# ofekm5/relative-pose-estimation

Measured on AMD Instinct MI355X. Metric: image-pairs/s end-to-end (640x480 pairs), median rotation-angle error alongside, higher is better.
Workload: dtype u8/i32 (ORB, Hamming) + f64 (RANSAC, pose); 1 GPU; 1024 640x480 pairs per GPU, ORB(1000kp)+BF-Hamming crossCheck top-500+5pt-RANSAC(0.999,1px)+recoverPose (BASELINE configs[1]); pairs_per_gpu=1024, distinct_pairs=1024, global_pairs=1024, streams_per_gpu=1, pairs_per_launch=1024

## Files before the change

include/rpe_amd.h:

```cpp
#ifndef RPE_AMD_H
#define RPE_AMD_H

#include <stddef.h>
#include <stdint.h>

#ifdef __cplusplus
extern "C" {
#endif

#define RPE_ABI_VERSION 3
#define RPE_ORB_LEVELS 12

enum {
    RPE_PAIR_OK = 0,
    RPE_PAIR_NO_DESCRIPTORS = 1,
    RPE_PAIR_INSUFFICIENT_MATCHES = 2,
    RPE_PAIR_NO_ESSENTIAL = 3,
    RPE_PAIR_AMBIGUOUS_ESSENTIAL = 4
};

enum {
    RPE_OVF_ORB_CANDIDATES = 1 << 0,
    RPE_OVF_ORB_KEYPOINTS  = 1 << 1,
    RPE_OVF_SIFT_SEEDS     = 1 << 4,
// ... 48 lines not shown
    float x, y;
    float size;
    float angle;
    float response;
    int32_t octave;
} rpe_sift_keypoint;

void rpe_default_config(rpe_config *cfg);
int rpe_create(const rpe_config *cfg, rpe_handle **out);
void rpe_destroy(rpe_handle *h);
const char *rpe_last_error(const rpe_handle *h);
int rpe_device_count(void);
int rpe_keypoint_capacity(const rpe_handle *h);

int rpe_device_malloc(rpe_handle *h, size_t bytes, void **d_ptr);
int rpe_device_free(rpe_handle *h, void *d_ptr);
int rpe_memcpy_h2d(rpe_handle *h, void *d_dst, const void *h_src, size_t bytes);
int rpe_memcpy_d2h(rpe_handle *h, void *h_dst, const void *d_src, size_t bytes);
int rpe_synchronize(rpe_handle *h);
int rpe_host_alloc(rpe_handle *h, size_t bytes, void **h_ptr);
int rpe_host_free(rpe_handle *h, void *h_ptr);
int rpe_host_register(rpe_handle *h, void *h_ptr, size_t bytes);
int rpe_host_unregister(rpe_handle *h, void *h_ptr);

int rpe_estimate_batch(rpe_handle *h, const uint8_t *h_imgs1, const uint8_t *h_imgs2, int B,
                       const double K[9], double *R, double *t, int32_t *inliers,
                       int32_t *n_matches, int32_t *status);
int rpe_estimate_batch_device(rpe_handle *h, const uint8_t *d_imgs1, const uint8_t *d_imgs2, int B,
                              const double K[9], double *R, double *t, int32_t *inliers,
                              int32_t *n_matches, int32_t *status);
int rpe_enqueue_batch_device(rpe_handle *h, const uint8_t *d_imgs1, const uint8_t *d_imgs2, int B,
                             const double K[9]);
int rpe_fetch_results(rpe_handle *h, int B, double *R, double *t, int32_t *inliers,
                      int32_t *n_matches, int32_t *status);
int rpe_fetch_overflow(rpe_handle *h, int n_pairs, uint32_t *flags);
int rpe_estimate_stream(rpe_handle *h, const uint8_t *h_frames, int F, const double K[9],
                        double *R, double *t, int32_t *inliers, int32_t *n_matches, int32_t *status);
int rpe_enqueue_stream_device(rpe_handle *h, const uint8_t *d_frames, int F, const double K[9]);

int rpe_frames_reserve(rpe_handle *h, int n_slots);
int rpe_frames_capacity(const rpe_handle *h);
int rpe_frames_put_device(rpe_handle *h, const uint8_t *d_frames, int n, const int32_t *slots);
int rpe_frames_put(rpe_handle *h, const uint8_t *h_frames, int n, const int32_t *slots);
int rpe_frames_info(rpe_handle *h, int n, const int32_t *slots, int32_t *counts, uint32_t *flags);
int rpe_enqueue_pairs(rpe_handle *h, const int32_t *slot1, const int32_t *slot2, int P, const double K[9]);
int rpe_estimate_pairs(rpe_handle *h, const int32_t *slot1, const int32_t *slot2, int P, const double K[9],
                       double *R, double *t, int32_t *inliers, int32_t *n_matches, int32_t *status);

#define RPE_UNDISTORT_ITERS 5
typedef struct rpe_camera {
    double fx, fy, cx, cy;
    double dist[8];
} rpe_camera;

int rpe_frames_set_cameras(rpe_handle *h, int n, const int32_t *slots, const rpe_camera *cams);
int rpe_enqueue_pairs_cameras(rpe_handle *h, const int32_t *slot1, const int32_t *slot2, int P);
int rpe_estimate_pairs_cameras(rpe_handle *h, const int32_t *slot1, const int32_t *slot2, int P,
                               double *R, double *t, int32_t *inliers, int32_t *n_matches, int32_t *status);
int rpe_enqueue_batch_cameras_device(rpe_handle *h, const uint8_t *d_imgs1, const uint8_t *d_imgs2, int B,
                                     const rpe_camera *cam1, const rpe_camera *cam2);
int rpe_estimate_batch_cameras_device(rpe_handle *h, const uint8_t *d_imgs1, const uint8_t *d_imgs2, int B,
                                      const rpe_camera *cam1, const rpe_camera *cam2, double *R, double *t,
                                      int32_t *inliers, int32_t *n_matches, int32_t *status);
int rpe_estimate_batch_cameras(rpe_handle *h, const uint8_t *h_imgs1, const uint8_t *h_imgs2, int B,
                               const rpe_camera *cam1, const rpe_camera *cam2, double *R, double *t,
                               int32_t *inliers, int32_t *n_matches, int32_t *status);
int rpe_undistort_points(rpe_handle *h, const float *h_pts, int n, const rpe_camera *cam, double *h_out_xy);
int rpe_find_essential_cameras(rpe_handle *h, const float *h_pts1, const float *h_pts2, const int32_t *m, int B,
                               const rpe_camera *cam1, const rpe_camera *cam2, double *E, uint8_t *mask,
                               int32_t *found, int32_t *info);
int rpe_recover_pose_cameras(rpe_handle *h, const double *h_E, const float *h_pts1, const float *h_pts2,
                             const int32_t *m, int B, const rpe_camera *cam1, const rpe_camera *cam2,
                             double *R, double *t, int32_t *inliers);
int rpe_refine_pose_points_cameras(rpe_handle *h, const double *h_R0, const double *h_t0, const float *h_pts1,
                                   const float *h_pts2, const uint8_t *h_mask, const int32_t *m, int B,
                                   const rpe_camera *cam1, const rpe_camera *cam2, int max_iters, double *R, double *t,
                                   int32_t *inliers, int32_t *info, double *rms);

enum { RPE_ORDER_BGR = 0, RPE_ORDER_RGB = 1 };
int rpe_bgr_to_gray_device(rpe_handle *h, const uint8_t *d_bgr, size_t n_pixels, int order, uint8_t *d_gray);
int rpe_bgr_to_gray(rpe_handle *h, const uint8_t *h_bgr, size_t n_pixels, int order, uint8_t *h_gray);

int rpe_lsd_detect(const uint8_t *h_gray, int width, int height, float *h_lines, int capacity, int32_t *n_lines);

int rpe_fetch_matched_points(rpe_handle *h, int B, float *pts1, float *pts2);

int rpe_fetch_structure(rpe_handle *h, int B, uint8_t *ransac_mask, uint8_t *pose_mask, double *points);

enum {
    RPE_REFINE_OK = 0,
    RPE_REFINE_SKIPPED = 1,
    RPE_REFINE_REJECTED = 2
};

int rpe_refine_poses(rpe_handle *h, int B, int max_iters, double *R, double *t, int32_t *inliers,
                     int32_t *info, double *rms);

int rpe_fetch_match_indices(rpe_handle *h, int B, int32_t *qidx, int32_t *tidx);

enum { RPE_LINK_OK = 0, RPE_LINK_PAIR_FAILED = 1, RPE_LINK_TOO_FEW = 2 };
int rpe_scale_links(rpe_handle *h, int L, const int32_t *pair_a, const int32_t *pair_b, const int32_t *side,
                    int min_shared, double *stats, int32_t *n_shared, int32_t *code);

int rpe_guided_matches(rpe_handle *h, int B, const double *R, const double *t, double gate_px, int max_distance,
                       int32_t *qidx, int32_t *tidx, int32_t *dist, float *pts1, float *pts2, int32_t *n_matches);

int rpe_guided_matches_l2(rpe_handle *h, int B, const double *R, const double *t, double gate_px, double max_distance,
                          int32_t *qidx, int32_t *tidx, float *dist, float *pts1, float *pts2, int32_t *n_matches);

enum { RPE_HOMOGRAPHY_OK = 0, RPE_HOMOGRAPHY_SKIPPED = 1, RPE_HOMOGRAPHY_NONE = 2 };
int rpe_pair_homographies(rpe_handle *h, int B, int iters, double threshold_px,
                          double *H, double *R_rot, uint8_t *mask, int32_t *counts, int32_t *info);
int rpe_find_homography(rpe_handle *h, const float *h_pts1, const float *h_pts2, const int32_t *m, int B,
                        const double K[9], int iters, double threshold_px,
                        double *H, double *R_rot, uint8_t *mask, int32_t *counts, int32_t *info);

enum { RPE_LINKPOSE_OK = 0, RPE_LINKPOSE_PAIR_FAILED = 1, RPE_LINKPOSE_TOO_FEW = 2, RPE_LINKPOSE_NONE = 3 };
int rpe_link_poses(rpe_handle *h, int L, const int32_t *pair_a, const int32_t *pair_b, const int32_t *side,
                   int iters, double threshold_px, int min_shared, int refine_iters,
                   double *R, double *t, uint8_t *mask, int32_t *counts, int32_t *info, double *rms);

enum { RPE_BUNDLE_OK = 0, RPE_BUNDLE_PAIR_FAILED = 1, RPE_BUNDLE_TOO_FEW = 2, RPE_BUNDLE_SKIPPED = 3, RPE_BUNDLE_REJECTED = 4 };
int rpe_link_bundles(rpe_handle *h, int L, const int32_t *pair_a, const int32_t *pair_b, const int32_t *side,
                     const double *R0, const double *t0, double threshold_px, int min_shared, int max_iters,
                     double *R_a, double *t_a, double *R_b, double *t_b, double *points, uint8_t *views,
                     int32_t *counts, int32_t *info, double *rms);
int rpe_bundle_three_view(rpe_handle *h, int B, const int32_t *n, const double *obs_s, const double *obs_a,
                          const double *obs_c, const uint8_t *has_c, const double *X0, const double *Ra0, const double *ta0,
                          const double *Rc0, const double *tc0, double f_a, double f_c, int max_iters,
                          double *R_a, double *t_a, double *R_c, double *t_c, double *points, uint8_t *views,
                          int32_t *counts, int32_t *info, double *rms);

enum { RPE_TRACK_EDGES_USABLE = 0, RPE_TRACK_EDGES_RANSAC = 1, RPE_TRACK_EDGES_ALL = 2 };
int rpe_last_run_pairs(const rpe_handle *h);
int rpe_build_tracks(rpe_handle *h, const uint8_t *use_pair, int edge_rule, int min_len,
                     int32_t *counts, int32_t *track_start, int32_t *obs_frame, int32_t *obs_kp, float *obs_xy,
                     int32_t *match_track);
int rpe_tracks_from_matches(rpe_handle *h, int P, int n_frames, const int32_t *frame1, const int32_t *frame2, const int32_t *m,
                            const int32_t *qidx, const int32_t *tidx, const uint8_t *edge, const float *pts1, const float *pts2,
                            int min_len, int32_t *counts, int32_t *track_start, int32_t *obs_frame, int32_t *obs_kp,
                            float *obs_xy, int32_t *match_track);

enum { RPE_TRACKPT_OK = 0, RPE_TRACKPT_TOO_FEW = 1, RPE_TRACKPT_DEGENERATE = 2, RPE_TRACKPT_BEHIND = 3, RPE_TRACKPT_OUTLIERS = 4,
       RPE_TRACKPT_LOW_PARALLAX = 5 };
int rpe_triangulate_tracks(rpe_handle *h, int n_tracks, const int32_t *track_start, const int32_t *obs_frame, const float *obs_xy,
                           int n_frames, const double *R_abs, const double *T_abs, const int32_t *frame_group, const double *K,
                           const rpe_camera *cams, double threshold_px, int min_views, double max_cos, int max_iters,
                           double *points, int32_t *info, double *rms, double *min_cos, uint8_t *obs_flag, double *obs_err);

int rpe_orb_detect_and_compute(rpe_handle *h, const uint8_t *h_imgs, int n_images,
                               rpe_keypoint *kps, uint8_t *desc, int32_t *counts);
int rpe_orb_debug_fetch(rpe_handle *h, int index, int which, uint8_t *h_out);
int64_t rpe_orb_pyramid_pixels(const rpe_handle *h);
int rpe_orb_debug_retain(rpe_handle *h, int kind, int stl_runtime, void *elems, const int32_t *len, const int32_t *n_points,
                         int n_lists, int cap, int32_t *out_len);

int rpe_match_hamming(rpe_handle *h, const uint8_t *h_desc1, const int32_t *n1,
                      const uint8_t *h_desc2, const int32_t *n2, int B,
                      int32_t *qidx, int32_t *tidx, int32_t *dist, int32_t *n_matches);

int rpe_match_hamming_guided(rpe_handle *h, const uint8_t *h_desc1, const float *h_pts1, const int32_t *n1,
                             const uint8_t *h_desc2, const float *h_pts2, const int32_t *n2, int B,
                             const double K[9], const double *R, const double *t, double gate_px, int max_distance,
                             int32_t *qidx, int32_t *tidx, int32_t *dist, int32_t *n_matches);

int rpe_sift_detect_and_compute(rpe_handle *h, const uint8_t *h_imgs, int n_images,
                                rpe_sift_keypoint *kps, float *desc, int32_t *counts);
int64_t rpe_sift_debug_gauss(rpe_handle *h, int index, float *out);

int rpe_match_l2(rpe_handle *h, const float *h_desc1, const int32_t *n1, const float *h_desc2,
                 const int32_t *n2, int B, int32_t *qidx, int32_t *tidx, float *dist, int32_t *n_matches);

int rpe_match_l2_guided(rpe_handle *h, const float *h_desc1, const float *h_pts1, const int32_t *n1,
                        const float *h_desc2, const float *h_pts2, const int32_t *n2, int B,
                        const double K[9], const double *R, const double *t, double gate_px, double max_distance,
                        int32_t *qidx, int32_t *tidx, float *dist, int32_t *n_matches);

int rpe_find_essential(rpe_handle *h, const float *h_pts1, const float *h_pts2, const int32_t *m, int B,
                       const double K[9], double *E, uint8_t *mask, int32_t *found, int32_t *info);

int rpe_recover_pose(rpe_handle *h, const double *h_E, const float *h_pts1, const float *h_pts2,
                     const int32_t *m, int B, const double K[9],
                     double *R, double *t, int32_t *inliers);

int rpe_refine_pose_points(rpe_handle *h, const double *h_R0, const double *h_t0, const float *h_pts1,
                           const float *h_pts2, const uint8_t *h_mask, const int32_t *m, int B, const double K[9],
                           int max_iters, double *R, double *t, int32_t *inliers, int32_t *info, double *rms);

enum {
    RPE_STAGE_PYRAMID = 0, RPE_STAGE_FAST, RPE_STAGE_NMS, RPE_STAGE_SELECT, RPE_STAGE_HARRIS,
    RPE_STAGE_KEYPOINTS, RPE_STAGE_ANGLE, RPE_STAGE_BLUR, RPE_STAGE_DESCRIBE, RPE_STAGE_MATCH,
    RPE_STAGE_RANSAC, RPE_STAGE_POSE, RPE_STAGE_COUNT
};
int rpe_set_profiling(rpe_handle *h, int enable);
int rpe_get_stage_ms(rpe_handle *h, float *ms );
const char *rpe_stage_name(int stage);

#define RPE_COMM_ID_BYTES 128
#define RPE_POSE_RECORD_BYTES 128
typedef struct rpe_comm rpe_comm;
int rpe_comm_unique_id(uint8_t id[RPE_COMM_ID_BYTES]);
int rpe_comm_create(rpe_handle *h, int rank, int world, const uint8_t id[RPE_COMM_ID_BYTES], rpe_comm **out);
int rpe_comm_prepare(rpe_handle *h, int rank, int world, rpe_comm **out);
int rpe_comm_connect(rpe_comm *c, const uint8_t id[RPE_COMM_ID_BYTES]);
int rpe_comm_destroy(rpe_comm *c);
const char *rpe_comm_last_error(void);
int rpe_gather_poses(rpe_handle *h, rpe_comm *c, int n_local, int per_rank, int first_pair, void *h_records);
int rpe_comm_allreduce_max(rpe_comm *c, double *value);
int rpe_comm_barrier(rpe_comm *c);

int rpe_calibrate_valu(rpe_handle *h, int kind, int waves_per_simd, double *wave_insts_per_s);
const char *rpe_calibrate_valu_name(int kind);
int rpe_calibrate_hbm(rpe_handle *h, double *bytes_per_s);

#ifdef __cplusplus
}
#endif
#endif
```

relative_pose_estimation_amd/_capi.py:

```python
import ctypes as C
import os

import numpy as np

_HERE = os.path.dirname(os.path.abspath(__file__))
LIB_PATH = os.environ.get("RPE_LIB", os.path.join(_HERE, "librpe_amd.so"))

ABI_VERSION = 3
ORB_LEVELS = 12
PAIR_OK, PAIR_NO_DESCRIPTORS, PAIR_INSUFFICIENT_MATCHES, PAIR_NO_ESSENTIAL, PAIR_AMBIGUOUS_ESSENTIAL = 0, 1, 2, 3, 4
FEATURE_ORB, FEATURE_SIFT = 0, 1
NORM_HAMMING, NORM_L2 = 0, 1
MATCH_CROSSCHECK, MATCH_RATIO = 0, 1
STL_LIBSTDCXX, STL_MSVC = 0, 1
OVF_ORB_CANDIDATES, OVF_ORB_KEYPOINTS = 1 << 0, 1 << 1
OVF_SIFT_SEEDS, OVF_SIFT_RAW, OVF_SIFT_PREFILTER, OVF_SIFT_CAP, OVF_SIFT_KEYPOINTS = 1 << 4, 1 << 5, 1 << 6, 1 << 7, 1 << 8
SIFT_UNCAPPED_CAPACITY = 16320
MAX_MATCHES_LIMIT = 8064
CALIB_KINDS = 18
STAGE_COUNT = 12
ORDER_BGR, ORDER_RGB = 0, 1
REFINE_OK, REFINE_SKIPPED, REFINE_REJECTED = 0, 1, 2
LINK_OK, LINK_PAIR_FAILED, LINK_TOO_FEW = 0, 1, 2
HOMOGRAPHY_OK, HOMOGRAPHY_SKIPPED, HOMOGRAPHY_NONE = 0, 1, 2
LINKPOSE_OK, LINKPOSE_PAIR_FAILED, LINKPOSE_TOO_FEW, LINKPOSE_NONE = 0, 1, 2, 3
BUNDLE_OK, BUNDLE_PAIR_FAILED, BUNDLE_TOO_FEW, BUNDLE_SKIPPED, BUNDLE_REJECTED = 0, 1, 2, 3, 4
TRACK_EDGES_USABLE, TRACK_EDGES_RANSAC, TRACK_EDGES_ALL = 0, 1, 2
TRACK_COUNTS = ("n_tracks", "n_obs", "n_edges", "dropped_conflict", "dropped_short", "n_frames_seen")
TRACKPT_OK, TRACKPT_TOO_FEW, TRACKPT_DEGENERATE, TRACKPT_BEHIND, TRACKPT_OUTLIERS, TRACKPT_LOW_PARALLAX = 0, 1, 2, 3, 4, 5
TRACKPT_NAMES = ("OK", "TOO_FEW", "DEGENERATE", "BEHIND", "OUTLIERS", "LOW_PARALLAX")
UNDISTORT_ITERS = 5

_SIGNATURES = {
    "rpe_default_config": "v:p", "rpe_create": "i:pp", "rpe_destroy": "v:p", "rpe_last_error": "s:p", "rpe_device_count": "i:",
    "rpe_keypoint_capacity": "i:p", "rpe_device_malloc": "i:pzp", "rpe_device_free": "i:pp", "rpe_memcpy_h2d": "i:pppz",
    "rpe_memcpy_d2h": "i:pppz", "rpe_synchronize": "i:p", "rpe_host_alloc": "i:pzp", "rpe_host_free": "i:pp",
    "rpe_host_register": "i:ppz", "rpe_host_unregister": "i:pp",
    "rpe_estimate_batch": "i:pppipppppp", "rpe_estimate_batch_device": "i:pppipppppp", "rpe_enqueue_batch_device": "i:pppip",
    "rpe_fetch_results": "i:pippppp", "rpe_fetch_overflow": "i:pip", "rpe_estimate_stream": "i:ppipppppp",
    "rpe_enqueue_stream_device": "i:ppip",
    "rpe_frames_reserve": "i:pi", "rpe_frames_capacity": "i:p", "rpe_frames_put_device": "i:ppip", "rpe_frames_put": "i:ppip",
    "rpe_frames_info": "i:pippp", "rpe_enqueue_pairs": "i:pppip", "rpe_estimate_pairs": "i:pppipppppp",
    "rpe_frames_set_cameras": "i:pipp", "rpe_enqueue_pairs_cameras": "i:pppi", "rpe_estimate_pairs_cameras": "i:pppippppp",
    "rpe_enqueue_batch_cameras_device": "i:pppipp", "rpe_estimate_batch_cameras_device": "i:pppippppppp",
    "rpe_estimate_batch_cameras": "i:pppippppppp", "rpe_undistort_points": "i:ppipp",
    "rpe_find_essential_cameras": "i:ppppipppppp", "rpe_recover_pose_cameras": "i:pppppippppp",
    "rpe_refine_pose_points_cameras": "i:pppppppippippppp",
    "rpe_bgr_to_gray_device": "i:ppzip", "rpe_bgr_to_gray": "i:ppzip", "rpe_lsd_detect": "i:piipip",
    "rpe_fetch_matched_points": "i:pipp", "rpe_fetch_structure": "i:pippp", "rpe_refine_poses": "i:piippppp",
    "rpe_fetch_match_indices": "i:pipp", "rpe_scale_links": "i:pipppippp", "rpe_link_poses": "i:pipppidiipppppp",
    "rpe_link_bundles": "i:pipppppdiippppppppp", "rpe_bundle_three_view": "i:pippppppppppddippppppppp",
    "rpe_last_run_pairs": "i:p", "rpe_build_tracks": "i:ppiipppppp", "rpe_tracks_from_matches": "i:piippppppppipppppp",
    "rpe_triangulate_tracks": "i:pipppipppppdidipppppp",
    "rpe_guided_matches": "i:pippdipppppp",
    "rpe_guided_matches_l2": "i:pippddpppppp",
    "rpe_pair_homographies": "i:piidppppp", "rpe_find_homography": "i:ppppipidppppp",
    "rpe_orb_detect_and_compute": "i:ppippp", "rpe_orb_debug_fetch": "i:piip", "rpe_orb_pyramid_pixels": "l:p",
    "rpe_orb_debug_retain": "i:piipppiip",
    "rpe_match_hamming": "i:pppppipppp", "rpe_match_hamming_guided": "i:pppppppipppdipppp",
    "rpe_sift_detect_and_compute": "i:ppippp", "rpe_sift_debug_gauss": "l:pip", "rpe_match_l2": "i:pppppipppp",
    "rpe_match_l2_guided": "i:pppppppipppddpppp",
    "rpe_find_essential": "i:ppppippppp", "rpe_recover_pose": "i:pppppipppp", "rpe_refine_pose_points": "i:pppppppipippppp",
    "rpe_set_profiling": "i:pi", "rpe_get_stage_ms": "i:pp", "rpe_stage_name": "s:i",
    "rpe_comm_unique_id": "i:p", "rpe_comm_create": "i:piipp", "rpe_comm_prepare": "i:piip", "rpe_comm_connect": "i:pp",
    "rpe_comm_destroy": "i:p", "rpe_comm_last_error": "s:", "rpe_gather_poses": "i:ppiiip", "rpe_comm_allreduce_max": "i:pp",
    "rpe_comm_barrier": "i:p",
    "rpe_calibrate_valu": "i:piip", "rpe_calibrate_valu_name": "s:i", "rpe_calibrate_hbm": "i:pp",
}
_ARG = {"p": C.c_void_p, "i": C.c_int, "d": C.c_double, "z": C.c_size_t}
_RET = {"i": C.c_int, "l": C.c_int64, "s": C.c_char_p, "v": None}
SIGNATURES = {name: (_RET[sig[0]], [_ARG[c] for c in sig[2:]]) for name, sig in _SIGNATURES.items()}
EXPORTS = list(SIGNATURES)


class Config(C.Structure):
    _fields_ = [("abi_version", C.c_int32), ("device", C.c_int32), ("width", C.c_int32), ("height", C.c_int32),
                ("max_batch", C.c_int32), ("feature_method", C.c_int32), ("norm_type", C.c_int32),
                ("max_matches", C.c_int32), ("nfeatures", C.c_int32), ("fast_threshold", C.c_int32),
                ("ransac_max_iters", C.c_int32), ("ransac_prob", C.c_double), ("ransac_threshold", C.c_double),
                ("match_mode", C.c_int32), ("stl_runtime", C.c_int32), ("match_ratio", C.c_double)]


KP_DTYPE = np.dtype([("x", "<f4"), ("y", "<f4"), ("angle", "<f4"), ("response", "<f4"),
                     ("octave", "<i4"), ("lx", "<i4"), ("ly", "<i4")])

SIFT_KP_DTYPE = np.dtype([("x", "<f4"), ("y", "<f4"), ("size", "<f4"), ("angle", "<f4"), ("response", "<f4"),
                          ("octave", "<i4")])

CAMERA_DTYPE = np.dtype([("fx", "<f8"), ("fy", "<f8"), ("cx", "<f8"), ("cy", "<f8"), ("dist", "<f8", (8,))])

_lib = None


class RpeError(RuntimeError):
    pass


class Camera:

    def __init__(self, K, dist=None):
        K = np.asarray(K, np.float64)
        if K.shape != (3, 3):
            raise ValueError(f"Camera: K must be 3 x 3, got shape {K.shape}")
        d = np.zeros(0) if dist is None else np.asarray(dist, np.float64).reshape(-1)
        if d.size not in (0, 4, 5, 8):
            raise ValueError(f"Camera: dist must hold 4, 5 or 8 coefficients (cv2 order), got {d.size}")
        self.fx, self.fy, self.cx, self.cy = float(K[0, 0]), float(K[1, 1]), float(K[0, 2]), float(K[1, 2])
        self.dist = np.zeros(8)
        self.dist[:d.size] = d
        if not (np.isfinite([self.fx, self.fy, self.cx, self.cy]).all() and np.isfinite(self.dist).all()):
            raise ValueError("Camera: non-finite field")
        if not (self.fx > 0 and self.fy > 0):
            raise ValueError("Camera: fx and fy must be > 0")

    @property
    def K(self):
        return np.array([[self.fx, 0., self.cx], [0., self.fy, self.cy], [0., 0., 1.]])

    def record(self):
        r = np.zeros(1, CAMERA_DTYPE)
        r["fx"], r["fy"], r["cx"], r["cy"], r["dist"] = self.fx, self.fy, self.cx, self.cy, self.dist
        return r


def camera_records(cameras, n):
    if isinstance(cameras, np.ndarray) and cameras.dtype == CAMERA_DTYPE:
        rec = np.ascontiguousarray(cameras).reshape(-1)
    elif isinstance(cameras, Camera):
        rec = np.repeat(cameras.record(), n)
    else:
        cameras = list(cameras)
        if not all(isinstance(c, Camera) for c in cameras):
            raise ValueError("cameras: expected Camera objects")
        rec = np.concatenate([c.record() for c in cameras]) if cameras else np.zeros(0, CAMERA_DTYPE)
    if rec.size != n:
        raise ValueError(f"cameras: expected {n}, got {rec.size}")
    return np.ascontiguousarray(rec)


def load():
    global _lib
    if _lib is not None:
        return _lib
    if not os.path.exists(LIB_PATH):
        raise RpeError(f"{LIB_PATH} not found: build it with __graft_entry__.build() "
                       "(make -C relative_pose_estimation_amd/csrc); there is no CPU fallback")
    lib = C.CDLL(LIB_PATH)
    for name, (restype, argtypes) in SIGNATURES.items():
        fn = getattr(lib, name)
        fn.restype, fn.argtypes = restype, argtypes
    _lib = lib
    return lib


def _p(a):
    return a.ctypes.data_as(C.c_void_p)


def _opt(a):
    return None if a is None else _p(a)


def _f64(a):
    return np.ascontiguousarray(a, np.float64)


def _i32(a):
    return np.ascontiguousarray(a, np.int32).reshape(-1)


def _slot_pairs(slot1, slot2):
    s1, s2 = _i32(slot1), _i32(slot2)
    assert s1.size == s2.size
    return s1, s2


def lsd_detect(gray, capacity=8192):
    g = np.ascontiguousarray(gray, np.uint8)
    assert g.ndim == 2
    out = np.zeros((capacity, 4), np.float32)
    n = np.zeros(1, np.int32)
    rc = load().rpe_lsd_detect(_p(g), g.shape[1], g.shape[0], _p(out), capacity, _p(n))
    if rc != 0:
        raise RpeError(f"rpe_lsd_detect failed ({rc})")
    return out[:min(int(n[0]), capacity)].astype(np.float64)


class Engine:

    def __init__(self, width, height, max_batch=1, nfeatures=4000, max_matches=500, device=0,
                 feature_method=FEATURE_ORB, norm_type=NORM_HAMMING, fast_threshold=15,
                 ransac_max_iters=1000, ransac_prob=0.999, ransac_threshold=1.0,
                 match_mode=MATCH_CROSSCHECK, match_ratio=0.75, stl_runtime=STL_LIBSTDCXX):
        self.lib = load()
        cfg = Config()
        self.lib.rpe_default_config(C.byref(cfg))
        cfg.device = device; cfg.width = width; cfg.height = height; cfg.max_batch = max_batch
        cfg.feature_method = feature_method; cfg.norm_type = norm_type
        cfg.max_matches = max_matches; cfg.nfeatures = nfeatures; cfg.fast_threshold = fast_threshold
        cfg.ransac_max_iters = ransac_max_iters; cfg.ransac_prob = ransac_prob; cfg.ransac_threshold = ransac_threshold
        cfg.match_mode = match_mode; cfg.match_ratio = match_ratio; cfg.stl_runtime = stl_runtime
        self.cfg = cfg
        h = C.c_void_p()
        rc = self.lib.rpe_create(C.byref(cfg), C.byref(h))
        if rc != 0:
            raise RpeError(f"rpe_create failed ({rc}): {self.lib.rpe_last_error(None).decode()}")
        self.h = h
        self.width, self.height, self.max_batch = width, height, max_batch
        self.max_matches = max_matches
        self.kcap = self.lib.rpe_keypoint_capacity(h)
# ... 534 lines not shown
```

relative_pose_estimation_amd/csrc/orb_kernels.hip:

```cpp
#include "rpe_internal.h"
#include "rpe_devmath.h"
#include "retain_best_emul.h"
#include "fast_entry.h"

__device__ float4 c_pattern_f[256];

__constant__ uint2 c_discw[32 * 8];

__constant__ float c_gauss[7];

void rpe_orb_upload_constants(const signed char *disc, int n)
{
    uint2 wt[32 * 8];
    for (int i = 0; i < 32 * 8; ++i) wt[i] = make_uint2(0u, 0u);
    for (int i = 0; i < n; ++i) {
        const int u = disc[2 * i], v = disc[2 * i + 1];
        const int j = (u + 16) >> 2, b = (u + 16) & 3;
        wt[(v + 15) * 8 + j].x |= 1u << (8 * b);
        wt[(v + 15) * 8 + j].y |= (unsigned)(u + 16) << (8 * b);
    }
    hipMemcpyToSymbol(HIP_SYMBOL(c_discw), wt, sizeof(wt));
    {
        static const signed char pat[256 * 4] = {
#include "brief_pattern.inc"
        };
        std::vector<float> pf(1024);
        for (int i = 0; i < 1024; ++i) pf[i] = (float)pat[i];
        hipMemcpyToSymbol(HIP_SYMBOL(c_pattern_f), pf.data(), sizeof(float) * 1024);
    }
    {
        double v[7], sum = 0.;
        float g[7];
        for (int i = 0; i < 7; ++i) { const double x = (double)(i - 3); v[i] = exp(-0.125 * x * x); sum += v[i]; }
        for (int i = 0; i < 7; ++i) g[i] = (float)(v[i] / sum);
        hipMemcpyToSymbol(HIP_SYMBOL(c_gauss), g, sizeof(g));
    }
}

__device__ __forceinline__ int xcd_tile(int b, int n)
{
    const int per = (n + 7) >> 3;
    return (b & 7) * per + (b >> 3);
}

__device__ __forceinline__ bool xcd_image_block(int nb, int n_img, int &img, int &blk)
{
    const int b = blockIdx.x, x = b & 7, idx = b >> 3;
    img = x + 8 * (idx / nb);
    blk = idx - (idx / nb) * nb;
    return img < n_img;
}
static inline unsigned xcd_image_grid(int nb, int n_img) { return (unsigned)(8 * ((n_img + 7) / 8) * nb); }

constexpr int PYR_THREADS = 64;
constexpr int PYR_LDS_DW = PYR_ROWS * PYR_DW + 4;
constexpr int PYR_NQ = PYR_DW / 4;
constexpr int PYR_LROWS = PYR_THREADS / PYR_NQ;
constexpr int PYR_LLANES = PYR_LROWS * PYR_NQ;
constexpr int PYR_NLD = (PYR_ROWS + PYR_LROWS - 1) / PYR_LROWS;
constexpr int PYR_NLD_FULL = (PYR_TH + 1 + PYR_LROWS - 1) / PYR_LROWS;
constexpr int PYR_NCHUNK = PYR_ROWS * PYR_NQ;
static_assert(PYR_THREADS == PYR_TW / 4 && PYR_THREADS == 64 && PYR_TH == 16, "one wave per tile; a lane takes 4 columns x the tile's 16 rows");
static_assert(PYR_DW % 4 == 0, "window rows are whole 16-byte chunks");
static_assert(PYR_LROWS == 3 && PYR_LLANES == 63 && PYR_NLD == 8, "63 lanes x 8 rounds of 3 rows cover the 23 x 21 chunks");
static_assert(PYR_NCHUNK * 4 <= PYR_LDS_DW && (PYR_NLD - 1) * PYR_LLANES < PYR_NCHUNK, "only the last round is cut short by the window's end");
static_assert((PYR_ROWS + 1) * PYR_DW * 4 < (1 << PYR_YW_SHIFT), "a window byte offset fits the row field of the y table");
static_assert(PYR_LDS_DW * 4 == 7744, "LDS per tile window");
__global__ __launch_bounds__(PYR_THREADS) void pyr_resize_kernel(uint8_t *pyr, RpeDeviceLayout lay, const int *__restrict__ coef,
                                                                  const RpePyrTile *__restrict__ ptiles, int ntiles, int l)
{
    __shared__ __attribute__((aligned(16))) unsigned s_src[PYR_LDS_DW];
    const RpeLevel &S = lay.lv[l - 1];
    const RpeLevel &D = lay.lv[l];
    const int tid = threadIdx.x;
    const int ti = xcd_tile(blockIdx.x, ntiles);
    if (ti >= ntiles) return;
    const RpePyrTile pt = ptiles[ti];
    const int x0 = pt.x0, y0 = pt.y0, a0 = pt.a0, sy0 = pt.sy0, nsrc = pt.nsrc;
    const unsigned reuse = pt.reuse;
    const uint8_t *src = rpe_level_base(pyr, lay, blockIdx.y, l - 1);
    const int *cxp = coef + D.dcoef_off, *cyp = cxp + ((D.w + 127) & ~127) + y0;
    const int x4 = x0 + 4 * tid;
    const int4 cv = *(const int4 *)(cxp + x4);
    unsigned ys[PYR_TH];
#pragma unroll
    for (int r = 0; r < PYR_TH; ++r) ys[r] = (unsigned)cyp[r];
    {
        const int lr = tid / PYR_NQ, lc = tid - lr * PYR_NQ;
        const unsigned colb = (unsigned)min(a0 + 16 * lc, S.pitch - 16) + __umul24((unsigned)sy0, (unsigned)S.pitch);
        const unsigned off0 = colb + __umul24((unsigned)lr, (unsigned)S.pitch), offmax = colb + __umul24((unsigned)(nsrc - 1), (unsigned)S.pitch);
        const unsigned pitch3 = PYR_LROWS * S.pitch;
        uint4 stage[PYR_NLD];
#pragma unroll
        for (int q = 0; q < PYR_NLD; ++q)
            if (q < PYR_NLD_FULL || PYR_LROWS * q < nsrc) stage[q] = *(const uint4 *)(src + min(off0 + q * pitch3, offmax));
#pragma unroll
        for (int q = 0; q < PYR_NLD; ++q)
            if (q < PYR_NLD_FULL || PYR_LROWS * q < nsrc) asm volatile("" : "+v"(stage[q].x), "+v"(stage[q].y), "+v"(stage[q].z), "+v"(stage[q].w));
        if (tid < PYR_LLANES) {
#pragma unroll
            for (int q = 0; q < PYR_NLD; ++q)
                if ((q < PYR_NLD_FULL || PYR_LROWS * q < nsrc) && (PYR_LLANES * (q + 1) <= PYR_NCHUNK || tid < PYR_NCHUNK - PYR_LLANES * q))
                    ((uint4 *)s_src)[tid + PYR_LLANES * q] = stage[q];
        }
    }
    typedef unsigned short v2u16_t __attribute__((ext_vector_type(2)));
    unsigned selp[4];
    v2u16_t apk[4];
    int bcol;
    {
        const int cw[4] = {cv.x, cv.y, cv.z, cv.w};
        const int o0 = cw[0] & 0xFFFF;
        bcol = o0 - a0;
#pragma unroll
        for (int j = 0; j < 4; ++j) {
            const unsigned rel = (unsigned)min(max((cw[j] & 0xFFFF) - o0, 0), 4);
            selp[j] = 0x0c000c00u | rel | ((rel + 1u) << 16);
            const unsigned a1 = (unsigned)cw[j] >> 16;
            apk[j] = __builtin_bit_cast(v2u16_t, (256u - a1) | (a1 << 16));
        }
    }
    const unsigned vbase = ((unsigned)bcol & ~3u) - (unsigned)sy0 * (PYR_DW * 4);
    __syncthreads();
    if (x4 >= D.pitch) return;
    const unsigned sh = (unsigned)bcol & 3u;
    auto fetch = [&](unsigned lds_byte, unsigned (&t)[3]) {
        const unsigned *p = (const unsigned *)((const uint8_t *)s_src + lds_byte);
        t[0] = p[0]; t[1] = p[1]; t[2] = p[2];
    };
    auto hpass = [&](const unsigned (&t)[3], unsigned (&hh)[4]) {
        const unsigned lo = __builtin_amdgcn_alignbyte(t[1], t[0], sh), hi = __builtin_amdgcn_alignbyte(t[2], t[1], sh);
#pragma unroll
        for (int j = 0; j < 4; ++j) hh[j] = __builtin_amdgcn_udot2(__builtin_bit_cast(v2u16_t, __builtin_amdgcn_perm(hi, lo, selp[j])), apk[j], 0u, false);
    };
    const unsigned colmask = x4 + 3 < D.w ? 0xFFFFFFFFu : (x4 >= D.w ? 0u : (0xFFFFFFFFu >> (8 * (x4 + 4 - D.w))));
    const unsigned sel01 = (0x0c0c0602u & colmask) | (0x0c0c0c0cu & ~colmask), sel23 = (0x06020c0cu & colmask) | (0x0c0c0c0cu & ~colmask);
    uint8_t *drow = pyr + (long long)blockIdx.y * lay.stride + D.off + __umul24((unsigned)y0, (unsigned)D.pitch) + x0;
    const int nrows = min(PYR_TH, D.h - y0);
    unsigned vo = 4u * (unsigned)tid, half = 32768u;
    asm("" : "+v"(half));
    auto rowtop = [&](int r) { return (ys[r] & ((1u << PYR_YW_SHIFT) - 1u)) + vbase; };
    unsigned hs[2][4], nb[3];
    fetch(rowtop(0) + PYR_DW * 4, nb);
#pragma unroll
    for (int r = 0; r < PYR_TH; ++r) {
        if (r == 0 || !((reuse >> r) & 1u)) { unsigned tt[3]; fetch(rowtop(r), tt); hpass(tt, hs[r & 1]); }
        const unsigned cb[3] = {nb[0], nb[1], nb[2]};
        if (r + 1 < PYR_TH) fetch(rowtop(r + 1) + PYR_DW * 4, nb);
        hpass(cb, hs[(r + 1) & 1]);
        const unsigned (&ht)[4] = hs[r & 1], (&hb)[4] = hs[(r + 1) & 1];
        const unsigned b1u = ys[r] >> PYR_YW_SHIFT, b0u = 256u - b1u;
        unsigned sm[4];
#pragma unroll
        for (int j = 0; j < 4; ++j) {
            unsigned t = __umul24(b0u, ht[j]) + half;
            asm("" : "+v"(t));
            sm[j] = __umul24(b1u, hb[j]) + t;
        }
        asm("" : "+v"(vo));
        if (r < nrows) *(unsigned *)(drow + vo) = __builtin_amdgcn_perm(sm[1], sm[0], sel01) | __builtin_amdgcn_perm(sm[3], sm[2], sel23);
        drow += D.pitch;
    }
}

void rpe_launch_pyramid(rpe_handle *h, int n_img)
{
    for (int l = 1; l < RPE_NLEVELS; ++l) {
        const int nt = h->pyr_tile_cnt[l];
        hipLaunchKernelGGL(pyr_resize_kernel, dim3((nt + 7) / 8 * 8, n_img), dim3(PYR_THREADS), 0, h->stream, h->d_pyr, h->lay, h->d_coef,
                           (const RpePyrTile *)(h->d_pyr_tiles + h->pyr_tile_off[l]), nt, l);
    }
}

__device__ __forceinline__ int imax3(int a, int b, int c) { return max(a, max(b, c)); }
__device__ __forceinline__ int vmax3u(int a, int b, int c) { int d; asm("v_max3_u32 %0, %1, %2, %3" : "=v"(d) : "v"(a), "v"(b), "v"(c)); return d; }
__device__ __forceinline__ int vmin3u(int a, int b, int c) { int d; asm("v_min3_u32 %0, %1, %2, %3" : "=v"(d) : "v"(a), "v"(b), "v"(c)); return d; }
typedef unsigned short ushort2_t __attribute__((ext_vector_type(2)));
static constexpr int CIRC_DX[16] = {0, 1, 2, 3, 3, 3, 2, 1, 0, -1, -2, -3, -3, -3, -2, -1};
static constexpr int CIRC_DY[16] = {3, 3, 2, 1, 0, -1, -2, -3, -3, -3, -2, -1, 0, 1, 2, 3};

constexpr int FS_ROWS = FAST_TH + 2;
constexpr int FAST_PROWS = FAST_TH + 8;
constexpr int FAST_THREADS = 256;
constexpr int FAST_NRP = 14;
constexpr int FAST_LANES = FAST_NRP * 18;
constexpr int FAST_NCAND = FS_ROWS * 72;
static_assert(FAST_LANES <= FAST_THREADS, "a pass of FAST_NRP tile rows fits the workgroup");
static_assert(FAST_ENTRY_NRP == FAST_NRP && FAST_ENTRY_LANES == FAST_LANES && FAST_ENTRY_PITCH == 72 && FAST_ENTRY_NPASS == 5,
              "fast_entry.h describes this kernel's lane mapping");
static_assert(6 * FAST_NRP >= FAST_PROWS && 5 * FAST_NRP >= FS_ROWS, "6 load passes cover the pixel rows, 5 phase-1 passes the score rows");
static_assert(RPE_FAST_TILE_CAP == (64 / 2) * (FAST_TH / 2), "strict 3x3 maxima of a tile");
static_assert(RPE_FAST_TILE_CAP <= FAST_PROWS * 18, "the tile's keypoint list lives in the dead pixel tile");
static_assert((FAST_PROWS * 18 + FS_ROWS * 18) * 4 + FAST_NCAND * 2 + 8 == 19448, "LDS per workgroup");
__global__ __launch_bounds__(FAST_THREADS) void fast_nms_kernel(const uint8_t *__restrict__ pyr, unsigned *__restrict__ tile_list,
                                                        int *__restrict__ tile_cnt, RpeDeviceLayout lay,
                                                        const RpeTile *__restrict__ tiles, int ntiles)
{
    __shared__ __attribute__((aligned(16))) unsigned s_in[FAST_PROWS * 18];
    __shared__ __attribute__((aligned(16))) unsigned s_sc[FS_ROWS * 18];
    unsigned *s_out = s_in;
    __shared__ unsigned short s_cand[FAST_NCAND];
    __shared__ int s_ncand, s_nout;
    const int tid = threadIdx.x, lane = tid & 63;
    const int ti = xcd_tile(blockIdx.x, ntiles);
    if (ti >= ntiles) return;
    const RpeTile t = tiles[ti];
    const RpeLevel &L = lay.lv[t.level];
    const int w = L.w, hgt = L.h, pitch = L.pitch, thr = lay.fast_thr;
    const int x0 = t.tx, y0 = t.ty;
    const long long tslot = (long long)blockIdx.y * ntiles + ti;
    const bool live = w > 2 * RPE_EDGE && hgt > 2 * RPE_EDGE && x0 < w - RPE_EDGE && x0 + 64 > RPE_EDGE &&
                      y0 < hgt - RPE_EDGE && y0 + FAST_TH > RPE_EDGE;
    if (!live) {
        if (tid == 0) tile_cnt[tslot] = 0;
        return;
    }
    const uint8_t *src = rpe_level_base(pyr, lay, blockIdx.y, t.level);
    if (tid == 0) { s_ncand = 0; s_nout = 0; }
    {
        const int lc = tid % 18, lr = tid / 18;
        const int lx = min(x0 - 4 + 4 * lc, pitch - 4);
        unsigned stage[6];
#pragma unroll
        for (int q = 0; q < 6; ++q) {
            const int r = min(lr + FAST_NRP * q, FAST_PROWS - 1);
            const int y = min(y0 - 4 + r, hgt - 1);
            stage[q] = *(const unsigned *)(src + (__umul24((unsigned)y, (unsigned)pitch) + (unsigned)lx));
        }
#pragma unroll
        for (int q = 0; q < 6; ++q) asm volatile("" : "+v"(stage[q]));
#pragma unroll
        for (int q = 0; q < 6; ++q) { const int r = lr + FAST_NRP * q; if (tid < FAST_LANES && r < FAST_PROWS) s_in[r * 18 + lc] = stage[q]; }
    }
    {
        uint4 *z1 = (uint4 *)s_sc;
        const uint4 z = make_uint4(0, 0, 0, 0);
        for (int i = tid; i < FS_ROWS * 18 / 4; i += FAST_THREADS) z1[i] = z;
    }
    __syncthreads();
    const unsigned T0 = (unsigned)thr * 0x01000100u;
    const int c = tid % 18, r0 = tid / 18;
    unsigned dark_bits = 0, brt_bits = 0, ndark_bits = 0xFFFFFFFFu;
    if (tid < FAST_LANES) {
        const int cl = max(c - 1, 0), cr = min(c + 1, 17);
        const int pxb = x0 - 4 + 4 * c;
        const int xlo = max(x0 - 1, RPE_EDGE - 1), xhi = min(x0 + 64, w - RPE_EDGE);
        unsigned vmask = 0xFu;
        if (pxb < xlo) vmask &= 0xFu << min(xlo - pxb, 4);
        if (pxb + 3 > xhi) vmask &= 0xFu >> min(pxb + 3 - xhi, 4);
        vmask &= 0xFu;
        const unsigned vmask5 = ((vmask * 0x00204081u) & 0x01010101u) * 0x1Fu;
        const unsigned *pC = s_in + (r0 + 3) * 18 + c, *pL = s_in + (r0 + 3) * 18 + cl, *pR = s_in + (r0 + 3) * 18 + cr;
#pragma unroll
        for (int it = 0; it < 5; ++it) {
            const int ry = r0 + FAST_NRP * it;
            const int py = y0 - 1 + ry;
            if (vmask == 0 || ry >= FS_ROWS || py < RPE_EDGE - 1 || py >= hgt - RPE_EDGE + 1) continue;
            const int ro = FAST_NRP * 18 * it;
            const unsigned cdw = pC[ro], ldw = pL[ro], rdw = pR[ro];
            const unsigned upl = pL[ro - 36], upc = pC[ro - 36], upr = pR[ro - 36];
            const unsigned dnl = pL[ro + 36], dnc = pC[ro + 36], dnr = pR[ro + 36];
            const unsigned bot = pC[ro + 54], top = pC[ro - 54];
            const unsigned n = ~cdw;
            const ushort2_t ne = __builtin_bit_cast(ushort2_t, n << 8), no = __builtin_bit_cast(ushort2_t, n);
            const ushort2_t T8 = __builtin_bit_cast(ushort2_t, T0);
            const unsigned Yd = __builtin_amdgcn_perm(__builtin_bit_cast(unsigned, __builtin_elementwise_add_sat(no, T8)),
                                                      __builtin_bit_cast(unsigned, __builtin_elementwise_add_sat(ne, T8)), 0x07030501u);
            const unsigned Yb = __builtin_amdgcn_perm(__builtin_bit_cast(unsigned, __builtin_elementwise_sub_sat(no, T8)),
                                                      __builtin_bit_cast(unsigned, __builtin_elementwise_sub_sat(ne, T8)), 0x07030501u);
            unsigned r[8];
            r[0] = bot;
            r[1] = top;
            r[2] = __builtin_amdgcn_alignbyte(rdw, cdw, 3);
            r[3] = __builtin_amdgcn_alignbyte(cdw, ldw, 1);
            r[4] = __builtin_amdgcn_alignbyte(dnr, dnc, 2);
            r[5] = __builtin_amdgcn_alignbyte(upc, upl, 2);
            r[6] = __builtin_amdgcn_alignbyte(upr, upc, 2);
            r[7] = __builtin_amdgcn_alignbyte(dnc, dnl, 2);
            unsigned nd[8], br[8];
#pragma unroll
            for (int k = 0; k < 8; ++k) {
                nd[k] = __builtin_amdgcn_lerp(r[k], Yd, 0xFFFFFFFFu);
                br[k] = __builtin_amdgcn_lerp(r[k], Yb, 0u);
            }
            unsigned xnd = nd[0] & nd[1], xb = br[0] | br[1];
#pragma unroll
            for (int k = 2; k < 8; k += 2) {
                xnd = __builtin_amdgcn_bitop3_b32(nd[k], nd[k + 1], xnd, 0xEA);
                xb = __builtin_amdgcn_bitop3_b32(br[k], br[k + 1], xb, 0xA8);
            }
            const unsigned rowm = 0x01010101u << it;
            ndark_bits = (ndark_bits & ~rowm) | ((xnd >> (7 - it)) & rowm);
            brt_bits |= (xb >> (7 - it)) & rowm;
        }
        dark_bits = ~ndark_bits & vmask5;
        brt_bits &= vmask5;
    }
    {
        const unsigned both_bits = brt_bits & dark_bits, do_bits = dark_bits & ~brt_bits, bo_bits = brt_bits & ~dark_bits;
        const int n = __popc(dark_bits) | (__popc(bo_bits) << 16);
        const int inc = wave_inclusive_sum(n);
        const int total = __shfl(inc, 63);
        if (total) {
            int base = 0;
            if (lane == 63) base = atomicAdd(&s_ncand, total);
            const int pre = __shfl(base, 63) + inc - n;
            unsigned short *wF = s_cand + (pre & 0xFFFF), *wB = s_cand + (FAST_NCAND - 1 - (pre >> 16));
            const unsigned ebase = fast_entry_lane_base((unsigned)tid);
            auto append = [&](unsigned bits, unsigned sides, unsigned short *&w, int step) {
                unsigned e = fast_entry_lane(ebase, 0u, sides);
                asm("" : "+v"(e));
                while (bits) {
                    const unsigned bpos = (unsigned)__ffs((int)bits) - 1u;
                    bits &= bits - 1;
                    *w = (unsigned short)(e | bpos);
                    w += step;
                }
            };
            append(do_bits, FAST_ENTRY_DARK, wF, 1);
            append(both_bits, FAST_ENTRY_SIDES, wF, 1);
            append(bo_bits, FAST_ENTRY_BRIGHT, wB, -1);
        }
    }
    __syncthreads();
    const int ncand = s_ncand;
    const int nF = ncand & 0xFFFF, nB = ncand >> 16, nc = nF + nB, gap = FAST_NCAND - nc;
    const int wv = __builtin_amdgcn_readfirstlane(tid >> 6);
    const int slice = ((nc + FAST_THREADS - 1) / FAST_THREADS) * 64;
    const int jb = min(wv * slice, nc), je = min(jb + slice, nc);
    const int cb = jb < nF ? jb : jb + gap;
    int ncorner = 0;
    const uint8_t *sb = (const uint8_t *)s_in;
    for (int j0 = jb; j0 < je; j0 += 64) {
        const int j = j0 + lane;
        bool corner = false;
        int cc = 0;
        if (j < je) {
            cc = s_cand[j < nF ? j : j + gap];
            const unsigned off = fast_entry_offset((unsigned)cc);
            const uint8_t *p = sb + 3 * 72 + off;
            const int v = p[0];
            int r[16];
#pragma unroll
            for (int k = 0; k < 16; ++k) r[k] = p[CIRC_DY[k] * 72 + CIRC_DX[k]];
            int s = 0;
            if (cc & 0x4000) {
                int x3[16];
#pragma unroll
                for (int k = 0; k < 16; ++k) x3[k] = vmax3u(r[k], r[(k + 1) & 15], r[(k + 2) & 15]);
                int x9[16];
#pragma unroll
                for (int k = 0; k < 16; ++k) x9[k] = vmax3u(x3[k], x3[(k + 3) & 15], x3[(k + 6) & 15]);
                const int m = min(vmin3u(vmin3u(x9[0], x9[1], x9[2]), vmin3u(x9[3], x9[4], x9[5]), vmin3u(x9[6], x9[7], x9[8])),
                                  vmin3u(vmin3u(x9[9], x9[10], x9[11]), vmin3u(x9[12], x9[13], x9[14]), x9[15]));
                s = v - m;
            }
            if (cc & 0x8000) {
                int m3[16];
#pragma unroll
                for (int k = 0; k < 16; ++k) m3[k] = vmin3u(r[k], r[(k + 1) & 15], r[(k + 2) & 15]);
                int m9[16];
#pragma unroll
                for (int k = 0; k < 16; ++k) m9[k] = vmin3u(m3[k], m3[(k + 3) & 15], m3[(k + 6) & 15]);
                const int m = max(vmax3u(vmax3u(m9[0], m9[1], m9[2]), vmax3u(m9[3], m9[4], m9[5]), vmax3u(m9[6], m9[7], m9[8])),
                                  vmax3u(vmax3u(m9[9], m9[10], m9[11]), vmax3u(m9[12], m9[13], m9[14]), m9[15]));
                s = max(s, m - v);
            }
            if (s > thr) {
                ((uint8_t *)s_sc)[off] = (uint8_t)(s - 1);
                corner = true;
            }
        }
        const unsigned long long km = __ballot(corner);
        if (corner) s_cand[cb + ncorner + __popcll(km & ((1ull << lane) - 1ull))] = (unsigned short)fast_entry_to_compact((unsigned)cc);
        ncorner += __popcll(km);
    }
    __syncthreads();
    const uint8_t *sc = (const uint8_t *)s_sc;
    for (int i0 = 0; i0 < ncorner; i0 += 64) {
        const int i = i0 + lane;
        bool keep = false;
        unsigned ent = 0;
        if (i < ncorner) {
            const int cc = s_cand[cb + i];
            const int bx = (int)fast_entry_compact_bx((unsigned)cc), ry = (int)fast_entry_compact_ry((unsigned)cc);
            const int px = x0 - 4 + bx, py = y0 - 1 + ry;
            const bool inside = (unsigned)(bx - 4) < 64u & (unsigned)(ry - 1) < (unsigned)FAST_TH &
                                (unsigned)(px - RPE_EDGE) < (unsigned)(w - 2 * RPE_EDGE) & (unsigned)(py - RPE_EDGE) < (unsigned)(hgt - 2 * RPE_EDGE);
            const uint8_t *q = sc + ry * 72 + bx;
            const int v = q[0];
            const int nmax = imax3(imax3(q[-1], q[1], q[-73]), imax3(q[-72], q[-71], q[71]), max((int)q[72], (int)q[73]));
            if (inside & (v > nmax)) {
                keep = true;
                ent = ((unsigned)v << 24) | ((unsigned)py << 12) | (unsigned)px;
            }
        }
        const unsigned long long km = __ballot(keep);
        if (km) {
            int base = 0;
            if (lane == 0) base = atomicAdd(&s_nout, __popcll(km));
            base = __shfl(base, 0);
            if (keep) s_out[base + __popcll(km & ((1ull << lane) - 1ull))] = ent;
        }
    }
    __syncthreads();
    const int nout = s_nout;
    unsigned *dst = tile_list + tslot * RPE_FAST_TILE_CAP;
    for (int i = tid; i < nout; i += FAST_THREADS) dst[i] = s_out[i];
    if (tid == 0) tile_cnt[tslot] = nout;
}

void rpe_launch_fast(rpe_handle *h, int n_img)
{
    if (h->n_tiles_fast == 0) return;
    hipLaunchKernelGGL(fast_nms_kernel, dim3((h->n_tiles_fast + 7) / 8 * 8, n_img), dim3(FAST_THREADS), 0, h->stream,
                       h->d_pyr, h->d_tile_list, h->d_tile_cnt, h->lay, h->d_tiles_fast, h->n_tiles_fast);
}

__global__ __launch_bounds__(256) void raster_corners_kernel(const unsigned *__restrict__ tile_list, const int *__restrict__ tile_cnt,
                                                              unsigned *__restrict__ corner, int *__restrict__ corner_count,
                                                              unsigned *__restrict__ ovf, RpeDeviceLayout lay, int ntiles, int rows_cap, int key_cap)
{
    extern __shared__ unsigned s_dyn[];
    unsigned *s_rs = s_dyn;
    unsigned *s_fill = s_rs + rows_cap + 1;
    unsigned *s_key = s_fill + rows_cap;
    unsigned *s_toff = s_key + key_cap;
    __shared__ int s_wave[5];
    __shared__ int s_live;
    const int tid = threadIdx.x, l = blockIdx.x, img = blockIdx.y;
    const RpeLevel &L = lay.lv[l];
    if (tid == 64) s_live = 0x7FFFFFFF;
    const int nrows = L.h, nt = L.ntile, ccap = L.ccap;
    for (int i = tid; i <= nrows; i += 256) s_rs[i] = 0;
    for (int i = tid; i < nrows; i += 256) s_fill[i] = 0;
    const int *tc = tile_cnt + (long long)img * ntiles + L.tile0;
    const unsigned *tl = tile_list + ((long long)img * ntiles + L.tile0) * RPE_FAST_TILE_CAP;
    int nraw = 0;
    for (int t0 = 0; t0 < nt; t0 += 256) {
        const int t = t0 + tid;
        const int c = t < nt ? tc[t] : 0;
        int total;
        const int ex = block_excl_scan(c, s_wave, total);
        if (t < nt) s_toff[t] = (unsigned)(nraw + ex);
        nraw += total;
    }
    if (tid == 0) s_toff[nt] = (unsigned)nraw;
    __syncthreads();
    auto fetch = [&](int sidx) -> unsigned {
        int lo = 0, hi = nt;
        while (hi - lo > 1) { const int mid = (lo + hi) >> 1; if (s_toff[mid] <= (unsigned)sidx) lo = mid; else hi = mid; }
        return tl[(long long)lo * RPE_FAST_TILE_CAP + (sidx - (int)s_toff[lo])];
    };
    for (int base = 0; base < nraw; base += 1024) {
        unsigned e4[4];
#pragma unroll
        for (int u = 0; u < 4; ++u) { const int sidx = base + tid + 256 * u; e4[u] = sidx < nraw ? fetch(sidx) : 0u; }
#pragma unroll
        for (int u = 0; u < 4; ++u) if (e4[u] >> 24) atomicAdd(&s_rs[(e4[u] >> 12) & 0xFFFu], 1u);
    }
    __syncthreads();
    int kept = 0;
    for (int r0 = 0; r0 < nrows; r0 += 4096) {
        const int rb = r0 + tid * 16;
        unsigned c[16]; int sum = 0;
#pragma unroll
        for (int k = 0; k < 16; ++k) { c[k] = (rb + k < nrows) ? s_rs[rb + k] : 0u; sum += (int)c[k]; }
        int total;
        int ex = block_excl_scan(sum, s_wave, total) + kept;
        int first_out = 0x7FFFFFFF;
#pragma unroll
        for (int k = 0; k < 16; ++k) {
            if (rb + k < nrows) { s_rs[rb + k] = (unsigned)ex; if (ex >= ccap) first_out = min(first_out, ex); }
            ex += (int)c[k];
        }
        if (first_out != 0x7FFFFFFF) atomicMin(&s_live, first_out);
        kept += total;
    }
    if (tid == 0) s_rs[nrows] = (unsigned)kept;
    __syncthreads();
    for (int base = 0; base < nraw; base += 1024) {
        unsigned e4[4];
#pragma unroll
        for (int u = 0; u < 4; ++u) { const int sidx = base + tid + 256 * u; e4[u] = sidx < nraw ? fetch(sidx) : 0u; }
#pragma unroll
        for (int u = 0; u < 4; ++u) {
            const unsigned e = e4[u];
            if (e >> 24) {
                const unsigned y = (e >> 12) & 0xFFFu, rs = s_rs[y];
                if (rs < (unsigned)ccap) {
                    const unsigned slot = rs + atomicAdd(&s_fill[y], 1u);
                    if (slot < (unsigned)key_cap) s_key[slot] = e;
                }
            }
        }
    }
    __syncthreads();
    unsigned *out = corner + (long long)img * lay.corner_total + L.corner_off;
    const int nlive = min(min(s_live, kept), key_cap);
    for (int slot = tid; slot < nlive; slot += 256) {
        const unsigned key = s_key[slot];
        const unsigned y = (key >> 12) & 0xFFFu, x = key & 0xFFFu;
        const unsigned rs = s_rs[y], re = s_rs[y + 1];
        unsigned rank = 0;
        for (unsigned j = rs; j < re; ++j) rank += ((s_key[j] & 0xFFFu) < x) ? 1u : 0u;
        const unsigned pos = rs + rank;
        if (pos < (unsigned)ccap) out[pos] = key;
    }
    if (tid == 0) {
        corner_count[img * RPE_NLEVELS + l] = min(kept, ccap);
        if (kept > ccap) atomicOr(&ovf[img], (unsigned)RPE_OVF_ORB_CANDIDATES);
    }
}

#define RPE_RETAIN_FAST_WAVES 2
#define RPE_RETAIN_HARRIS_WAVES 1

template <int NW, class E, class GT, class GE>
__device__ __forceinline__ int retain_list(E *s_a, int n, int n_points, int stl, GT gt, GE ge, unsigned short *s_pos, int *s_ctl)
{
    if (stl == rb::RT_LIBSTDCXX)
        return rb::block_retain_best_gnu<NW>(s_a, n, n_points, gt, ge, s_pos, s_ctl);
    if (threadIdx.x == 0) s_ctl[0] = rb::retain_best(s_a, n, n_points, stl, gt, ge);
    __syncthreads();
    return s_ctl[0];
}

struct FastScoreGT { __device__ __forceinline__ bool operator()(unsigned a, unsigned b) const { return (a >> 24) > (b >> 24); } };
struct FastScoreGE { __device__ __forceinline__ bool operator()(unsigned a, unsigned b) const { return (a >> 24) >= (b >> 24); } };

__global__ __launch_bounds__(64 * RPE_RETAIN_FAST_WAVES) void retain_fast_kernel(const unsigned *__restrict__ corner, const int *__restrict__ corner_count,
                                                          unsigned *__restrict__ cand_xy, int *__restrict__ cand_count,
                                                          unsigned *__restrict__ ovf, RpeDeviceLayout lay, int lo, int cap, int n_img)
{
    extern __shared__ unsigned s_a[];
    __shared__ int s_ctl[3 * RPE_RETAIN_FAST_WAVES];
    const int tid = threadIdx.x, l = blockIdx.x;
    const RpeLevel &L = lay.lv[l];
#pragma unroll 1
    for (int img = blockIdx.y; img < n_img; img += gridDim.y) {
    __syncthreads();
    const int n0 = corner_count[img * RPE_NLEVELS + l];
    const int n_points = 2 * L.quota;
    const bool active = n0 > n_points;
    if (active ? !(n0 > lo && n0 <= cap) : lo != 0) continue;
    const unsigned *in = corner + (long long)img * lay.corner_total + L.corner_off;
    unsigned *out = cand_xy + (long long)img * lay.cand_total + L.cand_off;
    int n1 = n0;
    if (active) {
        for (int i = tid; i < n0; i += 64 * RPE_RETAIN_FAST_WAVES) s_a[i] = in[i];
        __syncthreads();
        n1 = retain_list<RPE_RETAIN_FAST_WAVES>(s_a, n0, n_points, lay.stl, FastScoreGT(), FastScoreGE(), (unsigned short *)(s_a + cap), s_ctl);
    }
    const int nw = min(n1, L.kcap2);
    for (int i = tid; i < nw; i += 64 * RPE_RETAIN_FAST_WAVES) {
        const unsigned e = active ? s_a[i] : in[i];
        out[i] = (((e >> 12) & 0xFFFu) << 16) | (e & 0xFFFu);
    }
    if (tid == 0) {
        cand_count[img * RPE_NLEVELS + l] = nw;
        if (n1 > L.kcap2) atomicOr(&ovf[img], (unsigned)RPE_OVF_ORB_CANDIDATES);
    }
    }
}

#define RPE_RETAIN_TIER 2048
constexpr int RETAIN_HARRIS_CAP_MAX = 4 * (RPE_ORB_MAX_FEATURES / 7 + 1) + 256;
static_assert(rpe_retain_lds(0, rpe_corner_cap(RPE_MAX_IMAGE_DIM, RPE_MAX_IMAGE_DIM)) <= RPE_LDS_DEFAULT_BYTES &&
              rpe_retain_lds(1, RETAIN_HARRIS_CAP_MAX) <= RPE_LDS_DEFAULT_BYTES, "the retain kernels need no raised limit");

constexpr int raster_key_cap(int ccap_max, int wmax) { return ccap_max + wmax / 2 + 64; }
constexpr size_t raster_lds_bytes(int rows_cap, int key_cap, int nt_max) { return sizeof(unsigned) * ((size_t)rows_cap + 1 + rows_cap + key_cap + nt_max + 1); }
constexpr size_t RASTER_LDS_MAX = raster_lds_bytes(RPE_MAX_IMAGE_DIM, raster_key_cap(rpe_corner_cap(RPE_MAX_IMAGE_DIM, RPE_MAX_IMAGE_DIM), RPE_MAX_IMAGE_DIM),
                                                   rpe_fast_tiles(RPE_MAX_IMAGE_DIM, RPE_MAX_IMAGE_DIM));
static_assert(RASTER_LDS_MAX <= RPE_CU_LDS_BYTES, "the largest image's rows, entries and tiles fit a CU's LDS");

void rpe_launch_raster_retain(rpe_handle *h, int n_img)
{
    int rows_cap = 0, ccap_max = 0, nt_max = 0, wmax = 0, nlev_big = 0;
    for (int l = 0; l < RPE_NLEVELS; ++l) {
        rows_cap = std::max(rows_cap, h->lay.lv[l].h); ccap_max = std::max(ccap_max, h->lay.lv[l].ccap);
        nt_max = std::max(nt_max, h->lay.lv[l].ntile); wmax = std::max(wmax, h->lay.lv[l].w);
        if (h->lay.lv[l].ccap > RPE_RETAIN_TIER) nlev_big = l + 1;
    }
    const int key_cap = raster_key_cap(ccap_max, wmax);
    const size_t lds = raster_lds_bytes(rows_cap, key_cap, nt_max);
    assert(lds <= RASTER_LDS_MAX);
    hipLaunchKernelGGL(raster_corners_kernel, dim3(RPE_NLEVELS, n_img), dim3(256), lds, h->stream,
                       (const unsigned *)h->d_tile_list, (const int *)h->d_tile_cnt,
                       h->d_corner, h->d_corner_count, h->d_ovf, h->lay, h->n_tiles_fast, rows_cap, key_cap);
    hipLaunchKernelGGL(retain_fast_kernel, dim3(RPE_NLEVELS, n_img), dim3(64 * RPE_RETAIN_FAST_WAVES), rpe_retain_lds(0, std::min(ccap_max, RPE_RETAIN_TIER)), h->stream,
                       (const unsigned *)h->d_corner, (const int *)h->d_corner_count, h->d_cand_xy, h->d_cand_count, h->d_ovf, h->lay,
                       0, std::min(ccap_max, RPE_RETAIN_TIER), n_img);
    if (nlev_big > 0)
        hipLaunchKernelGGL(retain_fast_kernel, dim3(nlev_big, std::min(n_img, 512)), dim3(64 * RPE_RETAIN_FAST_WAVES), rpe_retain_lds(0, ccap_max), h->stream,
                           (const unsigned *)h->d_corner, (const int *)h->d_corner_count, h->d_cand_xy, h->d_cand_count, h->d_ovf, h->lay,
                           RPE_RETAIN_TIER, ccap_max, n_img);
}

__global__ __launch_bounds__(256) void harris_kernel(const uint8_t *__restrict__ pyr, const unsigned *__restrict__ cand_xy,
                                                      const int *__restrict__ cand_count, float *__restrict__ cand_resp,
                                                      RpeDeviceLayout lay, int nb, int n_img)
{
    int img, blk;
    if (!xcd_image_block(nb, n_img, img, blk)) return;
    const int dsel = blk * 256 + threadIdx.x;
    int l = -1, ci = 0, acc = 0;
#pragma unroll
    for (int k = 0; k < RPE_NLEVELS; ++k) {
        const int n = cand_count[img * RPE_NLEVELS + k];
        if (l < 0 && dsel < acc + n) { l = k; ci = dsel - acc; }
        acc += n;
    }
    if (l < 0) return;
    const RpeLevel &L = lay.lv[l];
    const int c = L.cand_off + ci;
    unsigned xy = cand_xy[(long long)img * lay.cand_total + c];
    const int x0 = xy & 0xFFFF, y0 = xy >> 16, pitch = L.pitch;
    const int sh = x0 & 3;
    const uint8_t *p0 = rpe_level_base(pyr, lay, img, l) + (long long)(y0 - 4) * pitch + ((x0 - 4) & ~3);
    unsigned w[9][3];
#pragma unroll
    for (int r = 0; r < 9; ++r) {
        const unsigned *pr = (const unsigned *)(p0 + r * pitch);
        w[r][0] = pr[0]; w[r][1] = pr[1]; w[r][2] = pr[2];
    }
    int a = 0, b = 0, cc = 0;
    int rowm[9], row0[9], rowp[9];
    auto unpack = [&](int r, int (&out)[9]) {
        const unsigned q0 = __builtin_amdgcn_alignbyte(w[r][1], w[r][0], sh), q1 = __builtin_amdgcn_alignbyte(w[r][2], w[r][1], sh);
        const unsigned q2 = w[r][2] >> (8 * sh);
#pragma unroll
        for (int k = 0; k < 4; ++k) { out[k] = (int)((q0 >> (8 * k)) & 255u); out[4 + k] = (int)((q1 >> (8 * k)) & 255u); }
        out[8] = (int)(q2 & 255u);
    };
    unpack(0, rowm); unpack(1, row0);
#pragma unroll
    for (int r = 0; r < 7; ++r) {
        unpack(r + 2, rowp);
#pragma unroll
        for (int k = 1; k < 8; ++k) {
            int Ix = (row0[k + 1] - row0[k - 1]) * 2 + (rowm[k + 1] - rowm[k - 1]) + (rowp[k + 1] - rowp[k - 1]);
            int Iy = (rowp[k] - rowm[k]) * 2 + (rowp[k - 1] - rowm[k - 1]) + (rowp[k + 1] - rowm[k + 1]);
            a += Ix * Ix; b += Iy * Iy; cc += Ix * Iy;
        }
#pragma unroll
        for (int k = 0; k < 9; ++k) { rowm[k] = row0[k]; row0[k] = rowp[k]; }
    }
    const float scale = 1.f / ((1 << 2) * 7 * 255.f);
    const float scale_sq_sq = scale * scale * scale * scale;
    float fa = (float)a, fb = (float)b, fc = (float)cc;
    float t1 = fa * fb, t2 = fc * fc, t3 = t1 - t2;
    float s = fa + fb;
    float t4 = (0.04f * s) * s;
    cand_resp[(long long)img * lay.cand_total + c] = (t3 - t4) * scale_sq_sq;
}

void rpe_launch_harris(rpe_handle *h, int n_img)
{
    const int nb = (h->lay.cand_total + 255) / 256;
    hipLaunchKernelGGL(harris_kernel, dim3(xcd_image_grid(nb, n_img)), dim3(256), 0, h->stream,
                       h->d_pyr, h->d_cand_xy, h->d_cand_count, h->d_cand_resp, h->lay, nb, n_img);
}

struct HarrisGT { __device__ __forceinline__ bool operator()(unsigned long long a, unsigned long long b) const { return __uint_as_float((unsigned)(a >> 32)) > __uint_as_float((unsigned)(b >> 32)); } };
struct HarrisGE { __device__ __forceinline__ bool operator()(unsigned long long a, unsigned long long b) const { return __uint_as_float((unsigned)(a >> 32)) >= __uint_as_float((unsigned)(b >> 32)); } };

__global__ __launch_bounds__(64 * RPE_RETAIN_HARRIS_WAVES) void retain_harris_kernel(unsigned *__restrict__ cand_xy, float *__restrict__ cand_resp,
                                                            const int *__restrict__ cand_count, int *__restrict__ kp_lvl_count,
                                                            RpeDeviceLayout lay, int lo, int cap)
{
    extern __shared__ unsigned long long s_e[];
    __shared__ int s_ctl[3 * RPE_RETAIN_HARRIS_WAVES];
    const int tid = threadIdx.x, l = blockIdx.x, img = blockIdx.y;
    const RpeLevel &L = lay.lv[l];
    const int n1 = cand_count[img * RPE_NLEVELS + l];
    const int q = L.quota;
    const bool active = n1 > q;
    if (active ? !(n1 > lo && n1 <= cap) : lo != 0) return;
    if (!active) { if (tid == 0) kp_lvl_count[img * RPE_NLEVELS + l] = n1; return; }
    unsigned *xy = cand_xy + (long long)img * lay.cand_total + L.cand_off;
    float *resp = cand_resp + (long long)img * lay.cand_total + L.cand_off;
    for (int i = tid; i < n1; i += 64 * RPE_RETAIN_HARRIS_WAVES) s_e[i] = ((unsigned long long)__float_as_uint(resp[i]) << 32) | xy[i];
    __syncthreads();
    const int n2 = retain_list<RPE_RETAIN_HARRIS_WAVES>(s_e, n1, q, lay.stl, HarrisGT(), HarrisGE(), (unsigned short *)(s_e + cap), s_ctl);
    for (int i = tid; i < n2; i += 64 * RPE_RETAIN_HARRIS_WAVES) { const unsigned long long e = s_e[i]; xy[i] = (unsigned)e; resp[i] = __uint_as_float((unsigned)(e >> 32)); }
    if (tid == 0) kp_lvl_count[img * RPE_NLEVELS + l] = n2;
}

template <int NW, class E, class GT, class GE>
__global__ __launch_bounds__(64 * NW) void retain_debug_kernel(E *__restrict__ elems, const int *__restrict__ len,
                                                                          const int *__restrict__ n_points, int *__restrict__ out_len, int cap, int stl)
{
    extern __shared__ unsigned long long s_dbg[];
    __shared__ int s_ctl[3 * NW];
    E *s_l = (E *)s_dbg;
    E *list = elems + (long long)blockIdx.x * cap;
    const int tid = threadIdx.x, n = len[blockIdx.x];
    for (int i = tid; i < n; i += 64 * NW) s_l[i] = list[i];
    __syncthreads();
    const int n1 = retain_list<NW>(s_l, n, n_points[blockIdx.x], stl, GT(), GE(), (unsigned short *)(s_l + cap), s_ctl);
    for (int i = tid; i < n; i += 64 * NW) list[i] = s_l[i];
    if (tid == 0) out_len[blockIdx.x] = n1;
}

void rpe_launch_debug_retain(rpe_handle *h, int kind, int stl, void *d_elems, const int *d_len, const int *d_n_points, int *d_out_len, int n_lists, int cap)
{
    const size_t lds = rpe_retain_lds(kind, cap);
    if (kind == 0)
        hipLaunchKernelGGL((retain_debug_kernel<RPE_RETAIN_FAST_WAVES, unsigned, FastScoreGT, FastScoreGE>), dim3(n_lists), dim3(64 * RPE_RETAIN_FAST_WAVES), lds, h->stream,
                           (unsigned *)d_elems, d_len, d_n_points, d_out_len, cap, stl);
    else
        hipLaunchKernelGGL((retain_debug_kernel<RPE_RETAIN_HARRIS_WAVES, unsigned long long, HarrisGT, HarrisGE>), dim3(n_lists), dim3(64 * RPE_RETAIN_HARRIS_WAVES), lds, h->stream,
                           (unsigned long long *)d_elems, d_len, d_n_points, d_out_len, cap, stl);
}

__global__ __launch_bounds__(256) void compact_keypoints_kernel(const unsigned *__restrict__ cand_xy, const float *__restrict__ cand_resp,
                                                                 const int *__restrict__ kp_lvl_count,
                                                                 unsigned *__restrict__ kp_xy, float *__restrict__ kp_resp,
                                                                 float2 *__restrict__ kp_pt, int *__restrict__ kp_count,
                                                                 unsigned *__restrict__ ovf, RpeDeviceLayout lay)
{
    const int img = blockIdx.x, kcap = lay.kcap;
    int offset = 0;
#pragma unroll 1
    for (int l = 0; l < RPE_NLEVELS; ++l) {
        const RpeLevel &L = lay.lv[l];
        const int n = kp_lvl_count[img * RPE_NLEVELS + l];
        const unsigned *xy = cand_xy + (long long)img * lay.cand_total + L.cand_off;
        const float *resp = cand_resp + (long long)img * lay.cand_total + L.cand_off;
        for (int i = threadIdx.x; i < n; i += 256) {
            const int o = offset + i;
            if (o < kcap) {
                const unsigned p = xy[i];
                const int x = p & 0xFFFF, y = p >> 16;
                const long long g = (long long)img * kcap + o;
                kp_xy[g] = (unsigned)x | ((unsigned)y << 12) | ((unsigned)l << 24);
                kp_resp[g] = resp[i];
                kp_pt[g] = make_float2((float)x * L.scale, (float)y * L.scale);
            }
        }
        offset += n;
    }
    if (threadIdx.x == 0) {
        kp_count[img] = min(offset, kcap);
        if (offset > kcap) atomicOr(&ovf[img], (unsigned)RPE_OVF_ORB_KEYPOINTS);
    }
}

void rpe_launch_keypoints(rpe_handle *h, int n_img)
{
    int kcap2_max = 0, nlev_big = 0;
    for (int l = 0; l < RPE_NLEVELS; ++l) {
        kcap2_max = std::max(kcap2_max, h->lay.lv[l].kcap2);
        if (h->lay.lv[l].kcap2 > RPE_RETAIN_TIER / 2) nlev_big = l + 1;
    }
    const int tier = std::min(kcap2_max, RPE_RETAIN_TIER / 2);
    assert(kcap2_max <= RETAIN_HARRIS_CAP_MAX);
    hipLaunchKernelGGL(retain_harris_kernel, dim3(RPE_NLEVELS, n_img), dim3(64 * RPE_RETAIN_HARRIS_WAVES), rpe_retain_lds(1, tier), h->stream,
                       h->d_cand_xy, h->d_cand_resp, (const int *)h->d_cand_count, h->d_kp_lvl_count, h->lay, 0, tier);
    if (nlev_big > 0)
        hipLaunchKernelGGL(retain_harris_kernel, dim3(nlev_big, n_img), dim3(64 * RPE_RETAIN_HARRIS_WAVES), rpe_retain_lds(1, kcap2_max), h->stream,
                           h->d_cand_xy, h->d_cand_resp, (const int *)h->d_cand_count, h->d_kp_lvl_count, h->lay, RPE_RETAIN_TIER / 2, kcap2_max);
    hipLaunchKernelGGL(compact_keypoints_kernel, dim3(n_img), dim3(256), 0, h->stream,
                       (const unsigned *)h->d_cand_xy, (const float *)h->d_cand_resp, (const int *)h->d_kp_lvl_count,
                       h->d_kp_xy, h->d_kp_resp, h->d_kp_pt, h->d_kp_count, h->d_ovf, h->lay);
}

std::vector<RpeLdsCeiling> rpe_orb_lds_ceilings()
{
    return {{(const void *)raster_corners_kernel, "raster_corners_kernel", RASTER_LDS_MAX}};
}

#define KP_R 22
#define KP_ROWS 45
#define KP_RAW_DW 12
#define KP_HCOLS 40
#define KP_HSTRIDE 49
static_assert((KP_ROWS * KP_RAW_DW + 4 + KP_HCOLS * KP_HSTRIDE) * 4 == 10016, "LDS per keypoint");
__global__ __launch_bounds__(64) void orient_describe_kernel(const uint8_t *__restrict__ pyr, const unsigned *__restrict__ kp_xy,
                                                               const float2 *__restrict__ kp_pt, const int *__restrict__ kp_count,
                                                               float *__restrict__ kp_angle, uint8_t *__restrict__ desc,
                                                               RpeDeviceLayout lay, int nb, int n_img)
{
    __shared__ __attribute__((aligned(16))) unsigned raw[KP_ROWS * KP_RAW_DW + 4];
    __shared__ float hb[KP_HCOLS * KP_HSTRIDE];
    const int lane = threadIdx.x;
    int img, blk;
    if (!xcd_image_block(nb, n_img, img, blk)) return;
    const long long g = (long long)img * lay.kcap + blk;
    const int nkp = kp_count[img];
    const unsigned p = (unsigned)__builtin_amdgcn_readfirstlane((int)kp_xy[g]);
    if (blk >= nkp) return;
    const int x0 = p & 0xFFF, y0 = (p >> 12) & 0xFFF, l = p >> 24;
    const RpeLevel &L = lay.lv[l];
    const int pitch = L.pitch;
    const int xal = (x0 - KP_R) & ~3, off0 = (x0 - KP_R) - xal;
    uint2 wt[4];
    float4 pf[4];
    {
        const uint8_t *src = rpe_level_base(pyr, lay, img, l) + (long long)(y0 - KP_R) * pitch + xal;
        const int lc = lane % KP_RAW_DW, lr = lane / KP_RAW_DW;
        unsigned stage[9];
        if (lane < 60) {
            const unsigned vo = 4u * (unsigned)lc + (unsigned)lr * (unsigned)pitch, p5 = 5u * (unsigned)pitch;
#pragma unroll
            for (int q = 0; q < 9; ++q) stage[q] = *(const unsigned *)(src + (vo + (unsigned)q * p5));
        }
#pragma unroll
        for (int q = 0; q < 4; ++q) wt[q] = c_discw[lane + 64 * q];
#pragma unroll
        for (int bit = 0; bit < 4; ++bit) pf[bit] = c_pattern_f[lane * 4 + bit];
        if (lane < 60) {
#pragma unroll
            for (int q = 0; q < 9; ++q) raw[(lr + 5 * q) * KP_RAW_DW + lc] = stage[q];
        }
    }
    __syncthreads();
    int m10 = 0, m01 = 0;
    {
        {
            const int bo = off0 + KP_R - 16;
            const int sh = bo & 3;
            const unsigned *pw = raw + ((KP_R - 15) + (lane >> 3)) * KP_RAW_DW + ((bo >> 2) + (lane & 7));
            unsigned c[4], su = 0u;
#pragma unroll
            for (int q = 0; q < 4; ++q) {
                const unsigned px = __builtin_amdgcn_alignbyte(pw[8 * q * KP_RAW_DW + 1], pw[8 * q * KP_RAW_DW], sh);
                c[q] = __builtin_amdgcn_udot4(px, wt[q].x, q ? c[q - 1] : 0u, false);
                su = __builtin_amdgcn_udot4(px, wt[q].y, su, false);
            }
            m10 = (int)su - 16 * (int)c[3];
            m01 = __mul24((lane >> 3) + 9, (int)c[3]) - 8 * (int)(c[0] + c[1] + c[2]);
        }
        m10 = wave_sum(m10);
        m01 = wave_sum(m01);
        {
            const float g0 = c_gauss[0], g1 = c_gauss[1], g2 = c_gauss[2], g3 = c_gauss[3];
            const int rp = lane / 5, cg = lane - 5 * rp;
#pragma unroll
            for (int q = 0; q < 2; ++q) {
                if (lane < (q == 0 ? 60 : 55)) {
                    const int row = 2 * rp + (KP_ROWS / 2 + 1) * q;
                    const unsigned *pw = raw + row * KP_RAW_DW + 2 * cg;
                    unsigned qq[2][4];
#pragma unroll
                    for (int h = 0; h < 2; ++h) {
                        const unsigned *ph = pw + h * KP_RAW_DW;
                        const unsigned d0 = ph[0], d1 = ph[1], d2 = ph[2], d3 = ph[3], d4 = ph[4];
                        qq[h][0] = __builtin_amdgcn_alignbyte(d1, d0, off0); qq[h][1] = __builtin_amdgcn_alignbyte(d2, d1, off0);
                        qq[h][2] = __builtin_amdgcn_alignbyte(d3, d2, off0); qq[h][3] = __builtin_amdgcn_alignbyte(d4, d3, off0);
                    }
                    typedef float v2f_t __attribute__((ext_vector_type(2)));
                    v2f_t F[14];
#pragma unroll
                    for (int j = 0; j < 14; ++j)
                        F[j] = (v2f_t){(float)((qq[0][j >> 2] >> (8 * (j & 3))) & 255u), (float)((qq[1][j >> 2] >> (8 * (j & 3))) & 255u)};
                    float *dst = hb + (8 * cg) * KP_HSTRIDE + row;
                    const v2f_t G0 = {g0, g0}, G1 = {g1, g1}, G2 = {g2, g2}, G3 = {g3, g3};
#pragma unroll
                    for (int o = 0; o < 8; ++o) {
                        v2f_t sacc = G0 * F[o];
                        sacc = __builtin_elementwise_fma(G1, F[o + 1], sacc);
                        sacc = __builtin_elementwise_fma(G2, F[o + 2], sacc);
                        sacc = __builtin_elementwise_fma(G3, F[o + 3], sacc);
                        sacc = __builtin_elementwise_fma(G2, F[o + 4], sacc);
                        sacc = __builtin_elementwise_fma(G1, F[o + 5], sacc);
                        sacc = __builtin_elementwise_fma(G0, F[o + 6], sacc);
                        dst[o * KP_HSTRIDE] = sacc.x;
                        dst[o * KP_HSTRIDE + 1] = sacc.y;
                    }
                }
            }
        }
    }
    __syncthreads();
    float a, b;
    {
        const float angle = fast_atan2_deg((float)m01, (float)m10);
        if (lane == 0) kp_angle[g] = angle;
        const float ang = angle * (float)(3.141592653589793238462643383279502884 / 180.0);
        double sn, cs;
        det_sincos((double)ang, sn, cs);
        a = (float)cs; b = (float)sn;
    }
    const float2 pt = kp_pt[g];
    const float sc = L.inv_scale;
    const int cx = __float2int_rn(pt.x * sc), cy = __float2int_rn(pt.y * sc);
    const int dxo = cx - x0 + 19, dyo = cy - y0 + KP_R - 3;
    int o00 = __builtin_amdgcn_readfirstlane(dxo * KP_HSTRIDE + dyo);
    asm volatile("" : "+s"(o00));
    const float *hb0 = hb + o00;
    const float g3 = c_gauss[3], g4 = c_gauss[4], g5 = c_gauss[5], g6 = c_gauss[6];
    unsigned nib = 0;
#pragma unroll
    for (int bit = 0; bit < 4; ++bit) {
        const float p0 = pf[bit].x, p1 = pf[bit].y, p2 = pf[bit].z, p3 = pf[bit].w;
        float fx0 = p0 * a - p1 * b, fy0 = p0 * b + p1 * a;
        float fx1 = p2 * a - p3 * b, fy1 = p2 * b + p3 * a;
        float t01[2];
        const float rxs[2] = {__builtin_rintf(fx0), __builtin_rintf(fx1)}, rys[2] = {__builtin_rintf(fy0), __builtin_rintf(fy1)};
#pragma unroll
        for (int e = 0; e < 2; ++e) {
            const float *t = hb0 + (int)__builtin_fmaf(rxs[e], (float)KP_HSTRIDE, rys[e]);
            typedef float v2f_t __attribute__((ext_vector_type(2)));
            const v2f_t s45 = (v2f_t){t[4], t[5]} + (v2f_t){t[2], t[1]};
            float sacc = g3 * t[3];
            sacc = __builtin_fmaf(g4, s45.x, sacc);
            sacc = __builtin_fmaf(g5, s45.y, sacc);
            sacc = __builtin_fmaf(g6, t[6] + t[0], sacc);
            t01[e] = __builtin_rintf(sacc);
        }
        nib |= (unsigned)(t01[0] < t01[1]) << bit;
    }
    unsigned v = nib << (4 * (lane & 7));
    v |= (unsigned)__builtin_amdgcn_update_dpp(0, (int)v, 0xB1, 0xF, 0xF, false);
// ... 94 lines not shown
```

relative_pose_estimation_amd/csrc/rpe_api.hip:

```cpp
#include "rpe_internal.h"
#include <math.h>
#include <float.h>
#include <string.h>
#include <stdio.h>
#include <stdlib.h>
#include <algorithm>

void rpe_orb_upload_constants(const signed char *disc, int n);

std::string g_create_err;

static int check_batch(rpe_handle *h, int B)
{
    if (B > h->cfg.max_batch) { h->err = "batch exceeds max_batch"; return RPE_ERR_CAPACITY; }
    return RPE_OK;
}
static int check_stream(rpe_handle *h, int F)
{
    if (F > h->n_img_cap || F - 1 > h->cfg.max_batch) { h->err = "stream longer than the handle capacity (frames <= 2*max_batch, pairs <= max_batch)"; return RPE_ERR_CAPACITY; }
    return RPE_OK;
}
static int check_desc_counts(rpe_handle *h, const int32_t *n, int B)
{
    for (int i = 0; i < B; ++i) if (n[i] < 0 || n[i] > h->lay.kcap) { h->err = "descriptor count exceeds keypoint capacity"; return RPE_ERR_INVALID; }
// ... 31 lines not shown
    HIPCHK(h, hipStreamSynchronize(h->stream));
    return RPE_OK;
}

int rpe_bufset_fit(rpe_handle *h, RpeBufSet &s, std::initializer_list<RpeBufPiece> pieces)
{
    RpeBufLayout need;
    for (const RpeBufPiece &pc : pieces) need.place(pc.bytes);
    if (need.total() > s.bytes) {
        uint8_t *old = s.block;
        if (old) HIPCHK(h, hipStreamSynchronize(h->stream));
        s = {};
        for (const RpeBufPiece &pc : pieces) *pc.p = nullptr;
        h->dev_allocs.erase(std::remove(h->dev_allocs.begin(), h->dev_allocs.end(), (void *)old), h->dev_allocs.end());
        if (old) HIPCHK(h, hipFree(old));
        if (int rc = dmalloc(h, &s.block, need.total())) return rc;
        s.bytes = need.total();
    }
    RpeBufLayout at;
    for (const RpeBufPiece &pc : pieces) {
        const size_t off = at.place(pc.bytes);
        *pc.p = off == RPE_BUF_NONE ? nullptr : s.block + off;
    }
    return RPE_OK;
}

static int check_positive(rpe_handle *h, const char *who, const char *name, double v)
{
    return std::isfinite(v) && v > 0. ? RPE_OK : rpe_invalid(h, who, (std::string(name) + " must be finite and > 0").c_str());
}
static bool all_finite(const double *v, size_t n)
{
    bool fin = true;
    for (size_t i = 0; i < n; ++i) fin = fin && std::isfinite(v[i]);
    return fin;
}

static long long align_up(long long v, long long a) { return (v + a - 1) / a * a; }

extern "C" void rpe_default_config(rpe_config *c)
{
    memset(c, 0, sizeof(*c));
    c->abi_version = RPE_ABI_VERSION;
    c->device = 0;
    c->width = 640; c->height = 480;
    c->max_batch = 1;
    c->feature_method = RPE_FEATURE_ORB;
    c->norm_type = RPE_NORM_HAMMING;
    c->max_matches = 500;
    c->nfeatures = 4000;
    c->fast_threshold = 15;
    c->ransac_max_iters = 1000;
    c->ransac_prob = 0.999;
    c->ransac_threshold = 1.0;
    c->match_mode = RPE_MATCH_CROSSCHECK;
    c->match_ratio = 0.75;
    c->stl_runtime = RPE_STL_LIBSTDCXX;
}

extern "C" int rpe_device_count(void)
{
    int n = 0;
    if (hipGetDeviceCount(&n) != hipSuccess) return 0;
    return n;
}

extern "C" const char *rpe_last_error(const rpe_handle *h) { return h ? h->err.c_str() : g_create_err.c_str(); }
extern "C" int rpe_keypoint_capacity(const rpe_handle *h) { return h ? h->lay.kcap : 0; }

static void build_layout(rpe_handle *h)
{
    RpeDeviceLayout &L = h->lay;
    const int W = h->cfg.width, H = h->cfg.height;
    const int nf = (h->cfg.feature_method == RPE_FEATURE_SIFT && h->cfg.nfeatures == 0) ? RPE_SIFT_UNCAPPED_CAPACITY : h->cfg.nfeatures;
    const double sf = (double)1.1f;
    long long off = 0;
    int coef = 0, cand = 0;
    for (int l = 0; l < RPE_NLEVELS; ++l) {
        RpeLevel &v = L.lv[l];
        v.scale = (float)pow(sf, (double)l);
        v.inv_scale = 1.0f / v.scale;
        v.w = cv_round((double)((float)W * v.inv_scale));
        v.h = cv_round((double)((float)H * v.inv_scale));
        v.pitch = (int)align_up(v.w, 16);
        v.off = off;
        off = align_up(off + (long long)v.pitch * v.h, 256);
        v.coef_off = coef;
        coef += 2 * (v.w + v.h);
    }
    L.stride = off;
    float factor = (float)(1.0 / sf);
    float nd = nf * (1 - factor) / (1 - (float)pow((double)factor, (double)RPE_NLEVELS));
    int sum = 0;
    for (int l = 0; l < RPE_NLEVELS - 1; ++l) {
        L.lv[l].quota = cv_round((double)nd);
        sum += L.lv[l].quota;
        nd *= factor;
    }
    L.lv[RPE_NLEVELS - 1].quota = nf - sum > 0 ? nf - sum : 0;
    int corner = 0;
    for (int l = 0; l < RPE_NLEVELS; ++l) {
        L.lv[l].ccap = rpe_corner_cap(L.lv[l].w, L.lv[l].h);
        L.lv[l].corner_off = corner;
        corner += L.lv[l].ccap;
        L.lv[l].kcap2 = 4 * L.lv[l].quota + 256;
        L.lv[l].cand_off = cand;
        cand += L.lv[l].kcap2;
    }
    L.corner_total = corner;
    L.cand_total = cand;
    L.stl = h->cfg.stl_runtime;
    L.kcap = nf + 64;
    L.fast_thr = h->cfg.fast_threshold;
}

static void lin_coeffs(int src, int dst, int *ofs, int *a1)
{
    double inv_scale = (double)dst / (double)src;
    double scale = 1.0 / inv_scale;
    for (int d = 0; d < dst; ++d) {
        double f = scale * ((double)d + 0.5) - 0.5;
        int i = (int)floor(f);
        if (i >= 0 && src > 1) {
            if (i < src - 1) { ofs[d] = i; a1[d] = cv_round((f - (double)i) * 256.0); }
            else { ofs[d] = src - 1; a1[d] = 0; }
        } else { ofs[d] = 0; a1[d] = 0; }
    }
}

static inline uint32_t rng_next(uint64_t &st)
{
    st = (uint64_t)(uint32_t)st * 4164903690ULL + (uint32_t)(st >> 32);
    return (uint32_t)st;
}

static int build_tables(rpe_handle *h)
{
    const RpeDeviceLayout &L = h->lay;
    std::vector<RpeTile> full, fast;
    for (int l = 0; l < RPE_NLEVELS; ++l) {
        const RpeLevel &v = L.lv[l];
        for (int y = 0; y < v.h; y += 64)
            for (int x = 0; x < v.pitch; x += 64) full.push_back({(short)l, (short)x, (short)y, 0});
        h->lay.lv[l].tile0 = (int)fast.size();
        if (v.w > 2 * RPE_EDGE && v.h > 2 * RPE_EDGE)
            for (int y = RPE_EDGE; y < v.h - RPE_EDGE; y += FAST_TH)
                for (int x = FAST_TILE_X0; x < v.w - RPE_EDGE; x += 64) fast.push_back({(short)l, (short)x, (short)y, 0});
        h->lay.lv[l].ntile = (int)fast.size() - h->lay.lv[l].tile0;
        assert(h->lay.lv[l].ntile == rpe_fast_tiles(v.w, v.h));
    }
    for (const RpeTile &t : fast)
        if (t.tx < 4 || t.ty < 4) { h->err = "FAST tile origin below 4: the tile loads would start outside the level"; return RPE_ERR_INVALID; }
    h->n_tiles_full = (int)full.size(); h->n_tiles_fast = (int)fast.size();
    DM(h, h->d_tiles_full, full.size());
    DM(h, h->d_tiles_fast, fast.size() ? fast.size() : 1);
    HIPCHK(h, hipMemcpy(h->d_tiles_full, full.data(), full.size() * sizeof(RpeTile), hipMemcpyHostToDevice));
    if (!fast.empty()) HIPCHK(h, hipMemcpy(h->d_tiles_fast, fast.data(), fast.size() * sizeof(RpeTile), hipMemcpyHostToDevice));
    int ncoef = L.lv[RPE_NLEVELS - 1].coef_off + 2 * (L.lv[RPE_NLEVELS - 1].w + L.lv[RPE_NLEVELS - 1].h);
    std::vector<int> coef((size_t)ncoef, 0);
    for (int l = 1; l < RPE_NLEVELS; ++l) {
        const RpeLevel &S = L.lv[l - 1], &D = L.lv[l];
        int *xo = coef.data() + D.coef_off, *xa = xo + D.w, *yo = xa + D.w, *ya = yo + D.h;
        lin_coeffs(S.w, D.w, xo, xa);
        lin_coeffs(S.h, D.h, yo, ya);
    }
    {
        std::vector<RpePyrTile> pt;
        for (int l = 1; l < RPE_NLEVELS; ++l) {
            const RpeLevel &S = L.lv[l - 1], &D = L.lv[l];
            const int *xo = coef.data() + D.coef_off, *yo = xo + 2 * D.w;
            if ((long long)S.h * PYR_DW * 4 >= (1ll << PYR_YW_SHIFT)) { h->err = "pyramid level too tall for the packed row table"; return RPE_ERR_INVALID; }
            for (int x0 = 0; x0 < D.w; x0 += PYR_TW) {
                int a0 = ((int)(((long long)x0 * S.w) / D.w)) & ~15, xl = x0 + PYR_TW - 1 < D.w ? x0 + PYR_TW - 1 : D.w - 1;
                int hi = xo[xl] + 1 < S.w ? xo[xl] + 1 : S.w - 1;
                if (xo[x0] < a0 || hi - a0 >= PYR_DW * 4) { h->err = "pyramid footprint bound violated (x)"; return RPE_ERR_INVALID; }
            }
            h->pyr_tile_off[l] = (int)pt.size();
            for (int y0 = 0; y0 < D.h; y0 += PYR_TH) {
                const int s0 = (int)(((long long)y0 * S.h) / D.h), yl = y0 + PYR_TH - 1 < D.h ? y0 + PYR_TH - 1 : D.h - 1;
                const int hi = yo[yl] + 1 < S.h ? yo[yl] + 1 : S.h - 1;
                if (yo[y0] < s0 || hi - s0 >= PYR_ROWS || yo[yl] + 1 - s0 >= PYR_ROWS) { h->err = "pyramid footprint bound violated (y)"; return RPE_ERR_INVALID; }
                unsigned reuse = 0;
                for (int r = 1; y0 + r <= yl; ++r) reuse |= (unsigned)(yo[y0 + r] == yo[y0 + r - 1] + 1) << r;
                for (int x0 = 0; x0 < D.pitch; x0 += PYR_TW)
                    pt.push_back({(short)x0, (short)y0, (short)(((int)(((long long)x0 * S.w) / D.w)) & ~15), (short)s0,
                                  (unsigned short)(hi - s0 + 1), (unsigned short)reuse, 0});
            }
            h->pyr_tile_cnt[l] = (int)pt.size() - h->pyr_tile_off[l];
        }
        DM(h, h->d_pyr_tiles, pt.size() ? pt.size() : 1);
        if (!pt.empty()) HIPCHK(h, hipMemcpy(h->d_pyr_tiles, pt.data(), pt.size() * sizeof(RpePyrTile), hipMemcpyHostToDevice));
    }
    {
        int dtotal = 0;
        for (int l = 1; l < RPE_NLEVELS; ++l) {
            h->lay.lv[l].dcoef_off = dtotal;
            dtotal += ((L.lv[l].w + 127) & ~127) + ((L.lv[l].h + 63) & ~63);
        }
        h->lay.lv[0].dcoef_off = 0;
        std::vector<int> packed((size_t)dtotal + 4, 0);
        for (int l = 1; l < RPE_NLEVELS; ++l) {
            const RpeLevel &D = L.lv[l];
            const int *xo = coef.data() + D.coef_off, *xa = xo + D.w, *yo = xa + D.w, *ya = yo + D.h;
            const int xw = (D.w + 127) & ~127, yh = (D.h + 63) & ~63;
            int *px = packed.data() + D.dcoef_off, *py = px + xw;
            for (int x = 0; x < xw; ++x) { const int k = x < D.w ? x : D.w - 1; px[x] = xo[k] | (xa[k] << 16); }
            for (int y = 0; y < yh; ++y) { const int k = y < D.h ? y : D.h - 1; py[y] = (int)((unsigned)(yo[k] * (PYR_DW * 4)) | ((unsigned)ya[k] << PYR_YW_SHIFT)); }
        }
        DM(h, h->d_coef, packed.size());
        HIPCHK(h, hipMemcpy(h->d_coef, packed.data(), sizeof(int) * packed.size(), hipMemcpyHostToDevice));
    }
    {
        int umax[RPE_HALF_PATCH + 2];
        int v, v0, vmax = (int)floor(RPE_HALF_PATCH * sqrt(2.f) / 2 + 1);
        int vmin = (int)ceil(RPE_HALF_PATCH * sqrt(2.f) / 2);
        for (v = 0; v <= vmax; ++v) umax[v] = cv_round(sqrt((double)RPE_HALF_PATCH * RPE_HALF_PATCH - v * v));
        for (v = RPE_HALF_PATCH, v0 = 0; v >= vmin; --v) {
            while (umax[v0] == umax[v0 + 1]) ++v0;
            umax[v] = v0;
            ++v0;
        }
        std::vector<signed char> disc;
        for (int vv = -RPE_HALF_PATCH; vv <= RPE_HALF_PATCH; ++vv) {
            int d = umax[abs(vv)];
            for (int u = -d; u <= d; ++u) { disc.push_back((signed char)u); disc.push_back((signed char)vv); }
        }
        rpe_orb_upload_constants(disc.data(), (int)(disc.size() / 2));
    }
    const int mm = h->cfg.max_matches, iters = h->cfg.ransac_max_iters;
    {
        std::vector<unsigned short> sub((size_t)(mm + 1) * iters * 5, 0);
        for (int M = 6; M <= mm; ++M) {
            uint64_t st = 0xFFFFFFFFFFFFFFFFULL;
            unsigned short *s = sub.data() + (size_t)M * iters * 5;
            for (int it = 0; it < iters; ++it, s += 5)
                for (int i = 0; i < 5; ++i) {
                    int v, dup;
                    do {
                        v = (int)(rng_next(st) % (uint32_t)M);
                        dup = 0;
                        for (int k = 0; k < i; ++k) if (s[k] == v) dup = 1;
                    } while (dup);
                    s[i] = (unsigned short)v;
                }
        }
        DM(h, h->d_subsets, sub.size());
        HIPCHK(h, hipMemcpy(h->d_subsets, sub.data(), sub.size() * sizeof(unsigned short), hipMemcpyHostToDevice));
    }
    {
        size_t n = (size_t)(mm + 1) * (mm + 2) / 2;
        std::vector<double> den(n, 0.); std::vector<int> rnd(n, 0);
        double p = h->cfg.ransac_prob;
        p = p > 0. ? p : 0.; p = p < 1. ? p : 1.;
        double num0 = (1. - p) > DBL_MIN ? (1. - p) : DBL_MIN;
        h->nit_num = log(num0);
        for (int M = 1; M <= mm; ++M)
            for (int g = 0; g <= M; ++g) {
                size_t idx = (size_t)M * (M + 1) / 2 + g;
                double ep = (double)(M - g) / M;
                ep = ep > 0. ? ep : 0.; ep = ep < 1. ? ep : 1.;
                double denom = 1. - pow(1. - ep, 5);
                if (denom < DBL_MIN) { den[idx] = 0.; rnd[idx] = -1; continue; }
                denom = log(denom);
                den[idx] = denom;
                rnd[idx] = denom >= 0 ? 0 : cv_round(h->nit_num / denom);
            }
        DM(h, h->d_nit_denom, n); DM(h, h->d_nit_round, n);
        HIPCHK(h, hipMemcpy(h->d_nit_denom, den.data(), n * sizeof(double), hipMemcpyHostToDevice));
        HIPCHK(h, hipMemcpy(h->d_nit_round, rnd.data(), n * sizeof(int), hipMemcpyHostToDevice));
    }
    return RPE_OK;
}

struct ResultBlock {
    size_t off[RPE_RESULT_SECTIONS], bytes = 0;
    explicit ResultBlock(const rpe_handle *h)
    {
        for (int k = 0; k < RPE_RESULT_SECTIONS; ++k) { off[k] = bytes; bytes += (size_t)h->cfg.max_batch * kRpeResultElem[k]; }
    }
};
static_assert(9 * sizeof(double) + 3 * sizeof(double) + 3 * sizeof(int) == RPE_RESULT_BYTES, "result sections");

static void unpack_results(const rpe_handle *h, int B, double *R, double *t, int32_t *inliers, int32_t *n_matches, int32_t *status)
{
    const ResultBlock rb(h);
    void *dst[RPE_RESULT_SECTIONS] = {R, t, inliers, status, n_matches};
    for (int k = 0; k < RPE_RESULT_SECTIONS; ++k)
        if (dst[k]) memcpy(dst[k], h->h_resblk + rb.off[k], (size_t)B * kRpeResultElem[k]);
}

static int alloc_workspace(rpe_handle *h)
{
    const RpeDeviceLayout &L = h->lay;
    const size_t NI = (size_t)h->n_img_cap, B = (size_t)h->cfg.max_batch, mm = (size_t)h->cfg.max_matches;
    const size_t NIo = h->cfg.feature_method == RPE_FEATURE_SIFT ? 1 : NI;
    DM(h, h->d_pyr, NIo * L.stride); DM(h, h->d_bufA, L.stride);
    HIPCHK(h, hipMemset(h->d_bufA, 0, L.stride));
    HIPCHK(h, hipMemset(h->d_pyr, 0, NIo * L.stride));
    const size_t ntf = h->n_tiles_fast > 0 ? (size_t)h->n_tiles_fast : 1;
    DM(h, h->d_tile_cnt, NIo * ntf); DM(h, h->d_tile_list, NIo * ntf * RPE_FAST_TILE_CAP);
    HIPCHK(h, hipMemset(h->d_tile_cnt, 0, NIo * ntf * sizeof(int)));
    const size_t img = (size_t)h->cfg.width * h->cfg.height;
    DM(h, h->d_stage1, (B + 1) * img); DM(h, h->d_stage2, B * img);
    DM(h, h->d_cand_xy, NI * L.cand_total); DM(h, h->d_cand_resp, NI * L.cand_total);
    DM(h, h->d_cand_count, NI * RPE_NLEVELS);
    DM(h, h->d_corner, NIo * L.corner_total); DM(h, h->d_corner_count, NI * RPE_NLEVELS); DM(h, h->d_kp_lvl_count, NI * RPE_NLEVELS);
    DM(h, h->d_kp_xy, NI * L.kcap); DM(h, h->d_kp_resp, NI * L.kcap); DM(h, h->d_kp_angle, NI * L.kcap);
    DM(h, h->d_kp_pt, NI * L.kcap); DM(h, h->d_kp_count, NI);
    DM(h, h->d_ovf, NI);
    HIPCHK(h, hipMemset(h->d_ovf, 0, NI * sizeof(unsigned)));
    DM(h, h->d_desc, NI * L.kcap * h->desc_bytes);
    HIPCHK(h, hipMemset(h->d_desc, 0, NI * L.kcap * h->desc_bytes));
    HIPCHK(h, hipMemset(h->d_kp_pt, 0, NI * L.kcap * sizeof(float2)));
    HIPCHK(h, hipMemset(h->d_kp_count, 0, NI * sizeof(int)));
    DM(h, h->d_m_q, B * mm); DM(h, h->d_m_t, B * mm); DM(h, h->d_m_d, B * mm);
    DM(h, h->d_resblk, (size_t)B * RPE_RESULT_BYTES);
    const ResultBlock rb(h);
    h->d_R = (double *)(h->d_resblk + rb.off[0]); h->d_t = (double *)(h->d_resblk + rb.off[1]);
    h->d_inliers = (int *)(h->d_resblk + rb.off[2]); h->d_status = (int *)(h->d_resblk + rb.off[3]); h->d_m_n = (int *)(h->d_resblk + rb.off[4]);
    HIPCHK(h, hipHostMalloc((void **)&h->h_resblk, (size_t)B * RPE_RESULT_BYTES));
    DM(h, h->d_pts1, B * mm); DM(h, h->d_pts2, B * mm);
    if (h->cfg.norm_type == RPE_NORM_L2) { DM(h, h->d_m_best, B * L.kcap); DM(h, h->d_m_best2, B * L.kcap); DM(h, h->d_m_norm, 2 * NI * L.kcap); }
    else {
        size_t bs = std::min<size_t>(B, RPE_MATCH_SPLIT_PAIRS);
        for (int extra : {0, RPE_GUIDED_LDS_UINT4})
            if (rpe_hamming_plan(L.kcap, (int)B, extra).hbm) bs = B;
        DM(h, h->d_hm_best, bs * L.kcap); DM(h, h->d_hm_row, bs * L.kcap);
    }
    DM(h, h->d_n1, B * mm); DM(h, h->d_n2, B * mm);
    DM(h, h->d_rstate, B); DM(h, h->d_found, B);
    DM(h, h->d_models, B * RPE_RANSAC_MAXCHUNK * RPE_MAX_MODELS * 9);
    DM(h, h->d_hyp, B * (RPE_RANSAC_MAXCHUNK / 64) * 88 * 64);
    DM(h, h->d_nmodels, B * RPE_RANSAC_MAXCHUNK);
    DM(h, h->d_counts, B * RPE_RANSAC_MAXCHUNK * RPE_MAX_MODELS);
    DM(h, h->d_mask, B * mm);
    DM(h, h->d_E, B * 9);
    DM(h, h->d_K, 9);
    return RPE_OK;
}

static int raise_lds_limits(rpe_handle *h)
{
    for (auto list : {rpe_orb_lds_ceilings, rpe_match_lds_ceilings, rpe_geom_lds_ceilings, rpe_link_lds_ceilings})
        for (const RpeLdsCeiling &c : list()) {
            const hipError_t e = hipFuncSetAttribute(c.kernel, hipFuncAttributeMaxDynamicSharedMemorySize, (int)c.bytes);
            if (e != hipSuccess) {
                h->err = std::string("raising the dynamic LDS limit of ") + c.name + " to " + std::to_string(c.bytes) + " bytes failed: " + hipGetErrorString(e);
                return RPE_ERR_HIP;
            }
        }
    return RPE_OK;
}

extern "C" int rpe_create(const rpe_config *cfg, rpe_handle **out)
{
    if (!cfg || !out) { g_create_err = "null argument"; return RPE_ERR_INVALID; }
    *out = nullptr;
    if (cfg->abi_version != RPE_ABI_VERSION) { g_create_err = "ABI version mismatch"; return RPE_ERR_INVALID; }
    const bool is_sift = cfg->feature_method == RPE_FEATURE_SIFT;
    if (cfg->feature_method != RPE_FEATURE_ORB && !is_sift) { g_create_err = "unknown feature method"; return RPE_ERR_INVALID; }
    if (cfg->norm_type != RPE_NORM_HAMMING && cfg->norm_type != RPE_NORM_L2) { g_create_err = "unknown norm type"; return RPE_ERR_INVALID; }
    if (is_sift && cfg->norm_type == RPE_NORM_HAMMING) {
        g_create_err = "NORM_HAMMING needs 8-bit descriptors: SIFT descriptors are float (cv2 raises in match())"; return RPE_ERR_INVALID;
    }
    if (cfg->match_mode != RPE_MATCH_CROSSCHECK && cfg->match_mode != RPE_MATCH_RATIO) { g_create_err = "unknown match mode"; return RPE_ERR_INVALID; }
    if (cfg->norm_type == RPE_NORM_L2 && cfg->nfeatures > RPE_SIFT_UNCAPPED_CAPACITY) {
        g_create_err = "NORM_L2: nfeatures must be <= 16320"; return RPE_ERR_INVALID;
    }
    if (cfg->stl_runtime != RPE_STL_LIBSTDCXX && cfg->stl_runtime != RPE_STL_MSVC) { g_create_err = "unknown stl_runtime"; return RPE_ERR_INVALID; }
    if (cfg->match_mode == RPE_MATCH_RATIO && !(cfg->match_ratio > 0. && cfg->match_ratio <= 1.)) { g_create_err = "match_ratio must be in (0, 1]"; return RPE_ERR_INVALID; }
    if (is_sift && (cfg->nfeatures > RPE_SIFT_UNCAPPED_CAPACITY || cfg->nfeatures < 0 || cfg->width > 4000 || cfg->height > 4000)) {
        g_create_err = "SIFT: nfeatures must be 0 (no cap: cv2's SIFT_create()) or a cap <= 16320, and the image <= 4000 px"; return RPE_ERR_INVALID;
    }
    if (cfg->width < 96 || cfg->height < 96 || cfg->width > RPE_MAX_IMAGE_DIM || cfg->height > RPE_MAX_IMAGE_DIM || cfg->max_batch < 1 ||
        (!is_sift && (cfg->nfeatures < 1 || cfg->nfeatures > RPE_ORB_MAX_FEATURES)) || cfg->max_matches < 5 || cfg->max_matches > RPE_MAX_MATCHES_LIMIT ||
        cfg->ransac_max_iters < 1 || cfg->ransac_max_iters > 4096 || cfg->fast_threshold < 1 || cfg->fast_threshold > 254) {
        g_create_err = "configuration out of supported range"; return RPE_ERR_INVALID;
    }
    int ndev = 0;
    if (hipGetDeviceCount(&ndev) != hipSuccess || ndev <= 0) {
        g_create_err = "no HIP device available: the MI355X path has no CPU fallback"; return RPE_ERR_HIP;
    }
    if (cfg->device < 0 || cfg->device >= ndev) { g_create_err = "bad device ordinal"; return RPE_ERR_INVALID; }
    rpe_handle *h = new rpe_handle();
    h->cfg = *cfg;
    h->n_img_cap = 2 * cfg->max_batch;
    h->desc_bytes = is_sift ? 128 : 32;
    int rc = RPE_OK;
    do {
        if (hipSetDevice(cfg->device) != hipSuccess) { h->err = "hipSetDevice failed"; rc = RPE_ERR_HIP; break; }
        if ((rc = raise_lds_limits(h)) != RPE_OK) break;
        if (hipStreamCreate(&h->stream) != hipSuccess) { h->err = "hipStreamCreate failed"; rc = RPE_ERR_HIP; break; }
        build_layout(h);
        if ((rc = build_tables(h)) != RPE_OK) break;
        if ((rc = alloc_workspace(h)) != RPE_OK) break;
        if (is_sift && (rc = rpe_sift_create(h)) != RPE_OK) break;
        for (int i = 0; i <= RPE_STAGE_COUNT; ++i)
            if (hipEventCreate(&h->ev[i]) != hipSuccess) { h->err = "hipEventCreate failed"; rc = RPE_ERR_HIP; break; }
    } while (0);
    if (rc != RPE_OK) { g_create_err = h->err; rpe_destroy(h); return rc; }
    *out = h;
    return RPE_OK;
}

static void frames_free(rpe_handle::FrameStore &fs)
{
    void *ptrs[] = {fs.d_desc, fs.d_kp_pt, fs.d_norm, fs.d_count, fs.d_ovf, fs.d_cam};
    for (void *p : ptrs) if (p) hipFree(p);
    fs = rpe_handle::FrameStore();
}

extern "C" void rpe_destroy(rpe_handle *h)
{
    if (!h) return;
    hipSetDevice(h->cfg.device);
    if (h->stream) hipStreamSynchronize(h->stream);
    rpe_sift_destroy(h);
    for (auto &g : h->graphs) { hipGraphExecDestroy(g.exec); hipGraphDestroy(g.graph); }
    for (void *p : h->dev_allocs) hipFree(p);
    if (h->h_resblk) hipHostFree(h->h_resblk);
    frames_free(h->fs);
    if (h->h_pairtab) hipHostFree(h->h_pairtab);
    for (int i = 0; i < RPE_TAB_RING; ++i) if (h->ev_tab[i]) hipEventDestroy(h->ev_tab[i]);
    for (void *p : h->user_allocs) hipFree(p);
    for (int i = 0; i <= RPE_STAGE_COUNT; ++i) if (h->ev[i]) hipEventDestroy(h->ev[i]);
    for (int c = 0; c < 8; ++c) if (h->ev_up[c]) hipEventDestroy(h->ev_up[c]);
    if (h->copy_stream) hipStreamDestroy(h->copy_stream);
    if (h->stream) hipStreamDestroy(h->stream);
    delete h;
}

extern "C" int rpe_device_malloc(rpe_handle *h, size_t bytes, void **d_ptr)
{
    if (!h || !d_ptr) return rpe_invalid(h, "rpe_device_malloc");
    HIPCHK(h, hipSetDevice(h->cfg.device));
    HIPCHK(h, hipMalloc(d_ptr, bytes));
    h->user_allocs.push_back(*d_ptr);
    return RPE_OK;
}
extern "C" int rpe_device_free(rpe_handle *h, void *d_ptr)
{
    if (!h) return rpe_invalid(h, "rpe_device_free");
    for (size_t i = 0; i < h->user_allocs.size(); ++i)
        if (h->user_allocs[i] == d_ptr) { h->user_allocs.erase(h->user_allocs.begin() + i); HIPCHK(h, hipFree(d_ptr)); return RPE_OK; }
    h->err = "rpe_device_free: unknown pointer";
    return RPE_ERR_INVALID;
}
extern "C" int rpe_host_alloc(rpe_handle *h, size_t bytes, void **h_ptr)
{
    if (!h || !h_ptr) return rpe_invalid(h, "rpe_host_alloc");
    HIPCHK(h, hipSetDevice(h->cfg.device));
    HIPCHK(h, hipHostMalloc(h_ptr, bytes, hipHostMallocDefault));
    return RPE_OK;
}
extern "C" int rpe_host_free(rpe_handle *h, void *h_ptr)
{
    if (!h) return rpe_invalid(h, "rpe_host_free");
    HIPCHK(h, hipHostFree(h_ptr));
    return RPE_OK;
}
extern "C" int rpe_host_register(rpe_handle *h, void *h_ptr, size_t bytes)
{
    if (!h || !h_ptr) return rpe_invalid(h, "rpe_host_register");
    HIPCHK(h, hipSetDevice(h->cfg.device));
    HIPCHK(h, hipHostRegister(h_ptr, bytes, hipHostRegisterDefault));
    return RPE_OK;
}
extern "C" int rpe_host_unregister(rpe_handle *h, void *h_ptr)
{
    if (!h || !h_ptr) return rpe_invalid(h, "rpe_host_unregister");
    HIPCHK(h, hipHostUnregister(h_ptr));
    return RPE_OK;
}
extern "C" int rpe_memcpy_h2d(rpe_handle *h, void *d, const void *s, size_t n)
{
    if (!h) return rpe_invalid(h, "rpe_memcpy_h2d");
    HIPCHK(h, hipMemcpyAsync(d, s, n, hipMemcpyHostToDevice, h->stream));
    HIPCHK(h, hipStreamSynchronize(h->stream));
    return RPE_OK;
}
extern "C" int rpe_memcpy_d2h(rpe_handle *h, void *d, const void *s, size_t n)
{
    if (!h) return rpe_invalid(h, "rpe_memcpy_d2h");
    HIPCHK(h, hipMemcpyAsync(d, s, n, hipMemcpyDeviceToHost, h->stream));
    HIPCHK(h, hipStreamSynchronize(h->stream));
    return RPE_OK;
}
extern "C" int rpe_synchronize(rpe_handle *h)
{
    if (!h) return rpe_invalid(h, "rpe_synchronize");
    HIPCHK(h, hipStreamSynchronize(h->stream));
    return RPE_OK;
}


static int load_level0(rpe_handle *h, const uint8_t *d_a, const uint8_t *d_b, int na, int nb)
{
    const int W = h->cfg.width, H = h->cfg.height;
    const RpeLevel &v = h->lay.lv[0];
    const size_t img = (size_t)W * H;
    if (v.pitch == W) {
        if (na) HIPCHK(h, hipMemcpy2DAsync(h->d_pyr + v.off, h->lay.stride, d_a, img, img, na, hipMemcpyDeviceToDevice, h->stream));
        if (nb) HIPCHK(h, hipMemcpy2DAsync(h->d_pyr + (size_t)na * h->lay.stride + v.off, h->lay.stride, d_b, img, img, nb,
                                           hipMemcpyDeviceToDevice, h->stream));
        return RPE_OK;
    }
    for (int i = 0; i < na + nb; ++i) {
        const uint8_t *src = i < na ? d_a + (size_t)i * img : d_b + (size_t)(i - na) * img;
        uint8_t *dst = h->d_pyr + (size_t)i * h->lay.stride + v.off;
        HIPCHK(h, hipMemcpy2DAsync(dst, v.pitch, src, W, W, H, hipMemcpyDeviceToDevice, h->stream));
    }
    return RPE_OK;
}

static bool set_level0_source(rpe_handle *h, const uint8_t *d_a, const uint8_t *d_b, int na, int nb)
{
    const bool direct = h->lay.lv[0].pitch == h->cfg.width && (((uintptr_t)d_a | (uintptr_t)(nb ? d_b : d_a)) & 15) == 0;
    h->lay.in_a = direct ? d_a : nullptr; h->lay.in_b = direct ? d_b : nullptr;
    h->lay.in_na = na; h->lay.in_img = h->cfg.width * h->cfg.height;
    h->level0_slots = na + nb;
    return direct;
}

static int run_orb(rpe_handle *h, const uint8_t *d_a, const uint8_t *d_b, int na, int nb)
{
    const int n = na + nb;
    MARK(h, RPE_STAGE_PYRAMID);
    HIPCHK(h, hipMemsetAsync(h->d_ovf, 0, sizeof(unsigned) * (size_t)n, h->stream));
    if (!set_level0_source(h, d_a, d_b, na, nb)) {
        int rc = load_level0(h, d_a, d_b, na, nb);
        if (rc) return rc;
    }
    rpe_launch_pyramid(h, n);
    MARK(h, RPE_STAGE_FAST);      rpe_launch_fast(h, n);
    MARK(h, RPE_STAGE_NMS);
    MARK(h, RPE_STAGE_SELECT);    rpe_launch_raster_retain(h, n);
    MARK(h, RPE_STAGE_HARRIS);    rpe_launch_harris(h, n);
    MARK(h, RPE_STAGE_KEYPOINTS); rpe_launch_keypoints(h, n);
    MARK(h, RPE_STAGE_ANGLE);     rpe_launch_orient_describe(h, n);
    MARK(h, RPE_STAGE_BLUR);
    MARK(h, RPE_STAGE_DESCRIBE);
    MARK(h, RPE_STAGE_MATCH);
    HIPCHK(h, hipGetLastError());
    return RPE_OK;
}

static int set_K(rpe_handle *h, const double K[9])
{
    if (h->K_valid && memcmp(h->K_last, K, sizeof(double) * 9) == 0) return RPE_OK;
    memcpy(h->K_last, K, sizeof(double) * 9);
    h->K_valid = false;
    HIPCHK(h, hipMemcpyAsync(h->d_K, h->K_last, sizeof(double) * 9, hipMemcpyHostToDevice, h->stream));
    h->K_valid = true;
    return RPE_OK;
}

static void last_run_begin(rpe_handle *h, RpeLastRun::Kind kind, const RpeRun &run, const int32_t *slot1 = nullptr,
                           const int32_t *slot2 = nullptr, const unsigned *flags = nullptr)
{
    RpeLastRun &l = h->last;
    l.kind = kind; l.pairs = run.pairs; l.run = run;
    l.tab.clear(); l.ovf.clear();
    for (int p = 0; kind == RpeLastRun::LIST && p < run.pairs; ++p) { l.tab.push_back(slot1[p]); l.tab.push_back(slot2[p]); }
    for (int p = 0; kind == RpeLastRun::CHUNKED && p < run.pairs; ++p) l.ovf.push_back(flags[p] | flags[h->cfg.max_batch + p]);
    l.per_match = kind != RpeLastRun::CHUNKED;
    l.structure = 0;
    h->ev_first = kind == RpeLastRun::LIST ? RPE_STAGE_MATCH : 0;
}

static void last_run_end(rpe_handle *h, bool images_too = false)
{
    h->last.per_match = false;
    h->last.structure = 0;
    if (images_too) { h->last.kind = RpeLastRun::NONE; h->last.pairs = 0; }
}

static void last_run_store_changed(rpe_handle *h, bool resized)
{
    if (resized) h->last.tab.clear();
    if (h->last.run.cam.tab) last_run_end(h);
}

static RpeRun last_run_first(const rpe_handle *h, int B)
{
    RpeRun r = h->last.run;
    r.pairs = B;
    return r;
}

static int last_run_structure(rpe_handle *h, int B, bool always)
{
    const size_t cap = (size_t)h->cfg.max_batch * h->cfg.max_matches;
    DM_ONCE(h, h->d_pose_mask, cap);
    DM_ONCE(h, h->d_points, cap * 3);
    if (!always && h->last.structure >= B) return RPE_OK;
    rpe_launch_structure(h, last_run_first(h, B));
    HIPCHK(h, hipGetLastError());
    h->last.structure = std::max(h->last.structure, B);
    return RPE_OK;
}

enum : unsigned { NEED_UNCHUNKED = 1, NEED_PER_MATCH = 2, NEED_COUNT = 4, NEED_TABLE = 8 };
static int last_run_gate(rpe_handle *h, const char *who, int n, unsigned needs)
{
    const RpeLastRun &l = h->last;
    const char *why = nullptr;
    if ((needs & NEED_UNCHUNKED) && l.kind == RpeLastRun::CHUNKED)
        why = ": the last host batch ran in chunks: what a run leaves per match is kept for unchunked and device-resident batches (rpe_estimate_batch_device) only";
    else if ((needs & NEED_PER_MATCH) && !l.per_match) why = ": no batch or stream since the last stage-API call (it overwrote the per-match buffers)";
    else if ((needs & NEED_COUNT) && n > l.pairs) why = ": more pairs than the last batch had";
    else if ((needs & NEED_TABLE) && l.kind == RpeLastRun::LIST && l.tab.size() < (size_t)2 * n) why = ": the frame store was resized since the pair list";
    if (why) { h->err = std::string(who) + why; return RPE_ERR_INVALID; }
    return RPE_OK;
}

static int run_tail(rpe_handle *h, const RpeRun &r)
{
    if (h->cfg.norm_type == RPE_NORM_L2) rpe_launch_match_l2(h, r);
    else rpe_launch_match(h, r);
    MARK(h, RPE_STAGE_RANSAC);
    rpe_launch_ransac(h, r, false);
    MARK(h, RPE_STAGE_POSE);
    rpe_launch_pose(h, r, true);
    if (h->profiling) { hipEventRecord(h->ev[RPE_STAGE_COUNT], h->stream); h->ev_valid = true; }
    HIPCHK(h, hipGetLastError());
    return RPE_OK;
}

static int run_images(rpe_handle *h, const uint8_t *d_a, const uint8_t *d_b, int na, int nb, const RpeRun &r)
{
    last_run_begin(h, RpeLastRun::RULE, r);
    int rc;
    if (h->cfg.feature_method == RPE_FEATURE_SIFT) {
        rc = rpe_sift_run(h, d_a, d_b, na, nb);
        MARK(h, RPE_STAGE_MATCH);
    } else
        rc = run_orb(h, d_a, d_b, na, nb);
    if (rc == RPE_OK) rc = run_tail(h, r);
    if (rc != RPE_OK) last_run_end(h);
    return rc;
}

extern "C" int rpe_enqueue_batch_device(rpe_handle *h, const uint8_t *d_imgs1, const uint8_t *d_imgs2, int B, const double K[9])
{
    if (!h || !d_imgs1 || !d_imgs2 || !K || B < 1) return rpe_invalid(h, "rpe_enqueue_batch_device");
    if (int rc = check_batch(h, B)) return rc;
    HIPCHK(h, hipSetDevice(h->cfg.device));
    int rc = set_K(h, K);
    if (rc) return rc;
    static const bool no_graph = getenv("RPE_NO_GRAPH") != nullptr;
    if (B > RPE_GRAPH_MAX_PAIRS || h->profiling || h->cfg.feature_method != RPE_FEATURE_ORB || no_graph)
        return run_images(h, d_imgs1, d_imgs2, B, B, rpe_run_batch(h, B));
    for (auto &g : h->graphs)
        if (g.a == d_imgs1 && g.b == d_imgs2 && g.B == B) {
            last_run_begin(h, RpeLastRun::RULE, rpe_run_batch(h, B));
            set_level0_source(h, d_imgs1, d_imgs2, B, B);
            HIPCHK(h, hipGraphLaunch(g.exec, h->stream));
            return RPE_OK;
        }
    rpe_handle::GraphEntry e{d_imgs1, d_imgs2, B, nullptr, nullptr};
    if (hipStreamBeginCapture(h->stream, hipStreamCaptureModeThreadLocal) != hipSuccess) {
        (void)hipGetLastError();
        return run_images(h, d_imgs1, d_imgs2, B, B, rpe_run_batch(h, B));
    }
    rc = run_images(h, d_imgs1, d_imgs2, B, B, rpe_run_batch(h, B));
    const hipError_t ce = hipStreamEndCapture(h->stream, &e.graph);
    if (rc != RPE_OK || ce != hipSuccess || !e.graph || hipGraphInstantiate(&e.exec, e.graph, nullptr, nullptr, 0) != hipSuccess) {
        (void)hipGetLastError();
        if (e.graph) hipGraphDestroy(e.graph);
        return rc != RPE_OK ? rc : run_images(h, d_imgs1, d_imgs2, B, B, rpe_run_batch(h, B));
    }
    if (h->graphs.size() >= 4) {
        hipGraphExecDestroy(h->graphs.front().exec); hipGraphDestroy(h->graphs.front().graph);
        h->graphs.erase(h->graphs.begin());
    }
    h->graphs.push_back(e);
    HIPCHK(h, hipGraphLaunch(e.exec, h->stream));
    return RPE_OK;
}

extern "C" int rpe_enqueue_stream_device(rpe_handle *h, const uint8_t *d_frames, int F, const double K[9])
{
    if (!h || !d_frames || !K || F < 2) return rpe_invalid(h, "rpe_enqueue_stream_device");
    if (int rc = check_stream(h, F)) return rc;
    HIPCHK(h, hipSetDevice(h->cfg.device));
    int rc = set_K(h, K);
    if (rc) return rc;
    return run_images(h, d_frames, d_frames, F, 0, rpe_run_stream(h, F - 1));
}

extern "C" int rpe_estimate_stream(rpe_handle *h, const uint8_t *h_frames, int F, const double K[9],
// ... 787 lines not shown
    return RPE_OK;
}

static int frames_check_put(rpe_handle *h, const void *frames, int n, const int32_t *slots)
{
    if (!h || !frames || !slots || n < 1) { if (h) h->err = "rpe_frames_put: null argument or n < 1"; return RPE_ERR_INVALID; }
    if (n > h->n_img_cap) { h->err = "rpe_frames_put: more than 2*max_batch frames in one call"; return RPE_ERR_CAPACITY; }
    if (h->fs.cap == 0) { h->err = "rpe_frames_put: no frame store (rpe_frames_reserve)"; return RPE_ERR_INVALID; }
    std::vector<int32_t> s(slots, slots + n);
    std::sort(s.begin(), s.end());
    if (s.front() < 0 || s.back() >= h->fs.cap) { h->err = "rpe_frames_put: slot outside the store"; return RPE_ERR_INVALID; }
    for (int i = 1; i < n; ++i) if (s[i] == s[i - 1]) { h->err = "rpe_frames_put: a slot appears twice in one put"; return RPE_ERR_INVALID; }
    return RPE_OK;
}

static int frames_put_run(rpe_handle *h, const uint8_t *d_a, const uint8_t *d_b, int na, int nb, const int32_t *slots)
{
    const int n = na + nb;
    int rc = upload_table(h, slots, nullptr, n);
    if (rc) return rc;
    last_run_end(h, true);
    h->ev_valid = false;
    if (h->cfg.feature_method == RPE_FEATURE_SIFT) rc = rpe_sift_run(h, d_a, d_b, na, nb);
    else rc = run_orb(h, d_a, d_b, na, nb);
    if (rc) return rc;
    const bool l2 = frames_keep_norms(h);
    if (l2) rpe_launch_l2_norms(h, n);
    const int rows = h->lay.kcap * (h->desc_bytes >> 4);
    const int gx = rows >= 65536 ? 32 : rows >= 8192 ? 8 : 2;
    hipLaunchKernelGGL(frames_scatter_kernel, dim3(gx, n), dim3(256), 0, h->stream,
                       (const uint8_t *)h->d_desc, (const float2 *)h->d_kp_pt, l2 ? (const int2 *)h->d_m_norm : (const int2 *)nullptr,
                       (const int *)h->d_kp_count, (const unsigned *)h->d_ovf, (const int *)h->d_pairtab, h->lay.kcap, h->desc_bytes,
                       h->fs.d_desc, h->fs.d_kp_pt, h->fs.d_norm, h->fs.d_count, h->fs.d_ovf);
    HIPCHK(h, hipGetLastError());
    for (int i = 0; i < n; ++i) h->fs.filled[(size_t)slots[i]] = 1;
    return RPE_OK;
}

extern "C" int rpe_frames_put_device(rpe_handle *h, const uint8_t *d_frames, int n, const int32_t *slots)
{
    int rc = frames_check_put(h, d_frames, n, slots);
    if (rc) return rc;
    HIPCHK(h, hipSetDevice(h->cfg.device));
    return frames_put_run(h, d_frames, d_frames, n, 0, slots);
}

extern "C" int rpe_frames_put(rpe_handle *h, const uint8_t *h_frames, int n, const int32_t *slots)
{
    int rc = frames_check_put(h, h_frames, n, slots);
    if (rc) return rc;
    HIPCHK(h, hipSetDevice(h->cfg.device));
    int na, nb;
    if ((rc = stage_images(h, h_frames, n, na, nb)) != RPE_OK) return rc;
    return frames_put_run(h, h->d_stage1, h->d_stage2, na, nb, slots);
}

extern "C" int rpe_frames_info(rpe_handle *h, int n, const int32_t *slots, int32_t *counts, uint32_t *flags)
{
    if (!h || !slots || n < 1) { if (h) h->err = "rpe_frames_info: null argument or n < 1"; return RPE_ERR_INVALID; }
    if (h->fs.cap == 0) { h->err = "rpe_frames_info: no frame store (rpe_frames_reserve)"; return RPE_ERR_INVALID; }
    for (int i = 0; i < n; ++i) if (slots[i] < 0 || slots[i] >= h->fs.cap) { h->err = "rpe_frames_info: slot outside the store"; return RPE_ERR_INVALID; }
    HIPCHK(h, hipSetDevice(h->cfg.device));
    int lo = slots[0], hi = slots[0];
    for (int i = 1; i < n; ++i) { lo = std::min(lo, (int)slots[i]); hi = std::max(hi, (int)slots[i]); }
    const size_t span = (size_t)(hi - lo + 1);
    std::vector<int> cnt(span);
    std::vector<unsigned> ov(span);
    if (int rc = fetch(h, {{cnt.data(), h->fs.d_count + lo, sizeof(int) * span}, {ov.data(), h->fs.d_ovf + lo, sizeof(unsigned) * span}})) return rc;
    for (int i = 0; i < n; ++i) {
        const size_t s = (size_t)slots[i];
        const bool f = h->fs.filled[s] != 0;
        if (counts) counts[i] = f ? cnt[s - lo] : -1;
        if (flags) flags[i] = f ? ov[s - lo] : 0u;
    }
    return RPE_OK;
}

static int enqueue_pairs_run(rpe_handle *h, const int32_t *slot1, const int32_t *slot2, int P, const double *K, const char *who)
{
    const char *bad = nullptr;
    int rc = RPE_ERR_INVALID;
    if (P > h->cfg.max_batch) { bad = ": pair list exceeds max_batch"; rc = RPE_ERR_CAPACITY; }
    else if (h->fs.cap == 0) bad = ": no frame store (rpe_frames_reserve)";
    for (int p = 0; p < P && !bad; ++p) {
        if (slot1[p] < 0 || slot1[p] >= h->fs.cap || slot2[p] < 0 || slot2[p] >= h->fs.cap) bad = ": slot outside the store";
        else if (!h->fs.filled[(size_t)slot1[p]] || !h->fs.filled[(size_t)slot2[p]]) bad = ": a pair names an empty slot";
        else if (!K && (!h->fs.has_cam[(size_t)slot1[p]] || !h->fs.has_cam[(size_t)slot2[p]])) bad = ": a pair names a slot without a camera (rpe_frames_set_cameras)";
    }
    if (bad) { h->err = std::string(who) + bad; return rc; }
    HIPCHK(h, hipSetDevice(h->cfg.device));
    if (K && (rc = set_K(h, K)) != RPE_OK) return rc;
    if ((rc = upload_table(h, slot1, slot2, P)) != RPE_OK) return rc;
    const RpeRun r = rpe_run_list(h, P, K ? RpeCamSrc{nullptr, nullptr, 0} : RpeCamSrc{h->fs.d_cam, (const int2 *)h->d_pairtab, 0});
    last_run_begin(h, RpeLastRun::LIST, r, slot1, slot2);
    MARK(h, RPE_STAGE_MATCH);
    if ((rc = run_tail(h, r)) != RPE_OK) last_run_end(h);
    return rc;
}

extern "C" int rpe_enqueue_pairs(rpe_handle *h, const int32_t *slot1, const int32_t *slot2, int P, const double K[9])
{
    if (!h || !slot1 || !slot2 || !K || P < 1) { if (h) h->err = "rpe_enqueue_pairs: null argument or P < 1"; return RPE_ERR_INVALID; }
    return enqueue_pairs_run(h, slot1, slot2, P, K, "rpe_enqueue_pairs");
}

extern "C" int rpe_estimate_pairs(rpe_handle *h, const int32_t *slot1, const int32_t *slot2, int P, const double K[9],
                                  double *R, double *t, int32_t *inliers, int32_t *n_matches, int32_t *status)
{
    int rc = rpe_enqueue_pairs(h, slot1, slot2, P, K);
    if (rc) return rc;
    return rpe_fetch_results(h, P, R, t, inliers, n_matches, status);
}

extern "C" int rpe_orb_detect_and_compute(rpe_handle *h, const uint8_t *h_imgs, int n_images,
                                          rpe_keypoint *kps, uint8_t *desc, int32_t *counts)
{
    if (!h || !h_imgs || n_images < 1) return rpe_invalid(h, "rpe_orb_detect_and_compute");
    if (h->cfg.feature_method != RPE_FEATURE_ORB) { h->err = "handle was not created for ORB"; return RPE_ERR_INVALID; }
    if (n_images > h->n_img_cap) { h->err = "n_images exceeds 2*max_batch"; return RPE_ERR_CAPACITY; }
    HIPCHK(h, hipSetDevice(h->cfg.device));
    last_run_end(h);
    int na, nb;
    int rc = stage_images(h, h_imgs, n_images, na, nb);
    if (rc == RPE_OK) rc = run_orb(h, h->d_stage1, h->d_stage2, na, nb);
    if (rc) return rc;
    const int kcap = h->lay.kcap;
    std::vector<unsigned> xy((size_t)n_images * kcap);
    std::vector<float> resp((size_t)n_images * kcap), ang((size_t)n_images * kcap);
    std::vector<float2> pt((size_t)n_images * kcap);
    std::vector<int> cnt(n_images);
    rc = fetch(h, {{xy.data(), h->d_kp_xy, xy.size() * 4}, {resp.data(), h->d_kp_resp, resp.size() * 4}, {ang.data(), h->d_kp_angle, ang.size() * 4},
                   {pt.data(), h->d_kp_pt, pt.size() * 8}, {cnt.data(), h->d_kp_count, cnt.size() * 4}, {desc, h->d_desc, (size_t)n_images * kcap * 32}});
    if (rc) return rc;
    for (int i = 0; i < n_images; ++i) {
        if (counts) counts[i] = cnt[i];
        if (!kps) continue;
        for (int k = 0; k < cnt[i]; ++k) {
            size_t g = (size_t)i * kcap + k;
            rpe_keypoint &o = kps[g];
            o.x = pt[g].x; o.y = pt[g].y; o.angle = ang[g]; o.response = resp[g];
            o.octave = (int)(xy[g] >> 24); o.lx = (int)(xy[g] & 0xFFF); o.ly = (int)((xy[g] >> 12) & 0xFFF);
        }
    }
    return RPE_OK;
}

extern "C" int64_t rpe_orb_pyramid_pixels(const rpe_handle *h)
{
    if (!h) return 0;
    int64_t n = 0;
    for (int l = 0; l < RPE_NLEVELS; ++l) n += (int64_t)h->lay.lv[l].w * h->lay.lv[l].h;
    return n;
}

extern "C" int rpe_orb_debug_fetch(rpe_handle *h, int index, int which, uint8_t *h_out)
{
    if (!h || !h_out || index < 0 || index >= h->n_img_cap) return rpe_invalid(h, "rpe_orb_debug_fetch");
    if (h->cfg.feature_method != RPE_FEATURE_ORB) { h->err = "rpe_orb_debug_fetch: handle was not created for ORB"; return RPE_ERR_INVALID; }
    if (which != 0 && which != 2 && which != 3) { h->err = "rpe_orb_debug_fetch: which must be 0 (pyramid), 2 (NMS map) or 3 (blurred pyramid)"; return RPE_ERR_INVALID; }
    HIPCHK(h, hipSetDevice(h->cfg.device));
    std::vector<uint8_t> tmp((size_t)h->lay.stride, 0);
    if (which == 2) {
        const size_t nt = (size_t)h->n_tiles_fast;
        std::vector<int> cnt(nt ? nt : 1);
        std::vector<unsigned> lst((nt ? nt : 1) * RPE_FAST_TILE_CAP);
        if (nt) {
            HIPCHK(h, hipMemcpyAsync(cnt.data(), h->d_tile_cnt + (size_t)index * nt, nt * sizeof(int), hipMemcpyDeviceToHost, h->stream));
            HIPCHK(h, hipMemcpyAsync(lst.data(), h->d_tile_list + (size_t)index * nt * RPE_FAST_TILE_CAP, nt * RPE_FAST_TILE_CAP * sizeof(unsigned),
                                     hipMemcpyDeviceToHost, h->stream));
            HIPCHK(h, hipStreamSynchronize(h->stream));
        }
        for (int l = 0; l < RPE_NLEVELS; ++l) {
            const RpeLevel &v = h->lay.lv[l];
            for (int t = v.tile0; t < v.tile0 + v.ntile; ++t)
                for (int k = 0; k < cnt[t] && k < RPE_FAST_TILE_CAP; ++k) {
                    const unsigned e = lst[(size_t)t * RPE_FAST_TILE_CAP + k];
                    tmp[v.off + (size_t)((e >> 12) & 0xFFF) * v.pitch + (e & 0xFFF)] = (uint8_t)(e >> 24);
                }
        }
    } else {
        const uint8_t *src = h->d_pyr + (size_t)index * h->lay.stride;
        if (h->lay.in_a) {
            if (index >= h->level0_slots) { h->err = "rpe_orb_debug_fetch: image slot was not part of the last run"; return RPE_ERR_INVALID; }
            const size_t img = (size_t)h->lay.in_img;
            const uint8_t *in = index < h->lay.in_na ? h->lay.in_a + (size_t)index * img : h->lay.in_b + (size_t)(index - h->lay.in_na) * img;
            HIPCHK(h, hipMemcpyAsync(h->d_pyr + (size_t)index * h->lay.stride + h->lay.lv[0].off, in, img, hipMemcpyDeviceToDevice, h->stream));
        }
        if (which == 3) { rpe_launch_debug_blur(h, index); HIPCHK(h, hipGetLastError()); src = h->d_bufA; }
        HIPCHK(h, hipMemcpyAsync(tmp.data(), src, tmp.size(), hipMemcpyDeviceToHost, h->stream));
        HIPCHK(h, hipStreamSynchronize(h->stream));
    }
    uint8_t *o = h_out;
    for (int l = 0; l < RPE_NLEVELS; ++l) {
        const RpeLevel &v = h->lay.lv[l];
        for (int y = 0; y < v.h; ++y, o += v.w) memcpy(o, tmp.data() + v.off + (size_t)y * v.pitch, v.w);
    }
    return RPE_OK;
}

extern "C" int rpe_orb_debug_retain(rpe_handle *h, int kind, int stl_runtime, void *elems, const int32_t *len, const int32_t *n_points,
                                    int n_lists, int cap, int32_t *out_len)
{
    if (!h || !elems || !len || !n_points || !out_len || n_lists < 1 || cap < 1) return rpe_invalid(h, "rpe_orb_debug_retain");
    if (h->cfg.feature_method != RPE_FEATURE_ORB) return rpe_invalid(h, "rpe_orb_debug_retain", "handle was not created for ORB");
    if (kind != 0 && kind != 1) return rpe_invalid(h, "rpe_orb_debug_retain", "kind must be 0 (u32 FAST entries) or 1 (u64 Harris entries)");
    if (stl_runtime != RPE_STL_LIBSTDCXX && stl_runtime != RPE_STL_MSVC) return rpe_invalid(h, "rpe_orb_debug_retain", "unknown stl_runtime");
    if (cap > 8192 || rpe_retain_lds(kind, cap) > RPE_LDS_DEFAULT_BYTES) return rpe_invalid(h, "rpe_orb_debug_retain", "cap too large for one workgroup's LDS");
    for (int i = 0; i < n_lists; ++i)
        if (len[i] < 0 || len[i] > cap) return rpe_invalid(h, "rpe_orb_debug_retain", "a list is longer than the capacity the launch is sized for");
    HIPCHK(h, hipSetDevice(h->cfg.device));
    const size_t esz = kind ? 8 : 4, bytes = esz * (size_t)n_lists * cap, ibytes = sizeof(int) * (size_t)n_lists;
    void *d_elems = nullptr; int *d_int = nullptr;
    HIPCHK(h, hipMalloc(&d_elems, bytes));
    hipError_t e = hipMalloc((void **)&d_int, 3 * ibytes);
    if (e == hipSuccess) e = hipMemcpyAsync(d_elems, elems, bytes, hipMemcpyHostToDevice, h->stream);
    if (e == hipSuccess) e = hipMemcpyAsync(d_int, len, ibytes, hipMemcpyHostToDevice, h->stream);
    if (e == hipSuccess) e = hipMemcpyAsync(d_int + n_lists, n_points, ibytes, hipMemcpyHostToDevice, h->stream);
    if (e == hipSuccess) {
        rpe_launch_debug_retain(h, kind, stl_runtime, d_elems, d_int, d_int + n_lists, d_int + 2 * (size_t)n_lists, n_lists, cap);
        e = hipGetLastError();
    }
    if (e == hipSuccess) e = hipMemcpyAsync(elems, d_elems, bytes, hipMemcpyDeviceToHost, h->stream);
    if (e == hipSuccess) e = hipMemcpyAsync(out_len, d_int + 2 * (size_t)n_lists, ibytes, hipMemcpyDeviceToHost, h->stream);
    if (e == hipSuccess) e = hipStreamSynchronize(h->stream);
    hipFree(d_elems); hipFree(d_int);
    HIPCHK(h, e);
    return RPE_OK;
}

static int stage_match_run(rpe_handle *h, bool l2, const int32_t *n1, const int32_t *n2, int B, int32_t *qidx, int32_t *tidx,
                           void *dist, int32_t *n_matches)
{
    const size_t mm = h->cfg.max_matches;
    HIPCHK(h, hipMemcpyAsync(h->d_kp_count, n1, sizeof(int) * B, hipMemcpyHostToDevice, h->stream));
    HIPCHK(h, hipMemcpyAsync(h->d_kp_count + B, n2, sizeof(int) * B, hipMemcpyHostToDevice, h->stream));
    if (l2) rpe_launch_match_l2(h, rpe_run_batch(h, B));
    else rpe_launch_match(h, rpe_run_batch(h, B));
    HIPCHK(h, hipGetLastError());
    return fetch(h, {{qidx, h->d_m_q, sizeof(int) * mm * B}, {tidx, h->d_m_t, sizeof(int) * mm * B}, {dist, h->d_m_d, sizeof(int) * mm * B},
                     {n_matches, h->d_m_n, sizeof(int) * B}});
}

extern "C" int rpe_match_hamming(rpe_handle *h, const uint8_t *h_desc1, const int32_t *n1, const uint8_t *h_desc2,
                                 const int32_t *n2, int B, int32_t *qidx, int32_t *tidx, int32_t *dist, int32_t *n_matches)
{
    if (!h || !h_desc1 || !h_desc2 || !n1 || !n2 || B < 1) return rpe_invalid(h, "rpe_match_hamming");
    if (int rc = check_batch(h, B)) return rc;
    HIPCHK(h, hipSetDevice(h->cfg.device));
    last_run_end(h);
    const size_t per = (size_t)h->lay.kcap * 32;
    if (int rc = check_desc_counts(h, n1, B)) return rc;
    if (int rc = check_desc_counts(h, n2, B)) return rc;
    HIPCHK(h, hipMemcpyAsync(h->d_desc, h_desc1, per * B, hipMemcpyHostToDevice, h->stream));
    HIPCHK(h, hipMemcpyAsync(h->d_desc + per * B, h_desc2, per * B, hipMemcpyHostToDevice, h->stream));
    return stage_match_run(h, false, n1, n2, B, qidx, tidx, dist, n_matches);
}

static int upload_points(rpe_handle *h, const float *p1, const float *p2, const int32_t *m, int B)
{
    const size_t mm = h->cfg.max_matches;
    if (int rc = check_match_counts(h, m, B)) return rc;
    HIPCHK(h, hipMemcpyAsync(h->d_pts1, p1, sizeof(float2) * mm * B, hipMemcpyHostToDevice, h->stream));
    HIPCHK(h, hipMemcpyAsync(h->d_pts2, p2, sizeof(float2) * mm * B, hipMemcpyHostToDevice, h->stream));
    HIPCHK(h, hipMemcpyAsync(h->d_m_n, m, sizeof(int) * B, hipMemcpyHostToDevice, h->stream));
    return RPE_OK;
}

static int check_cameras(rpe_handle *h, const rpe_camera *c, int n, const char *who)
{
    for (int i = 0; i < n; ++i) {
        const double *f = &c[i].fx;
        bool fin = true;
        for (int k = 0; k < 12; ++k) fin = fin && std::isfinite(f[k]);
        if (!fin) { h->err = std::string(who) + ": a camera has a non-finite field"; return RPE_ERR_INVALID; }
        if (!(c[i].fx > 0.) || !(c[i].fy > 0.)) { h->err = std::string(who) + ": a camera has fx <= 0 or fy <= 0"; return RPE_ERR_INVALID; }
    }
    return RPE_OK;
}

static int upload_batch_cameras(rpe_handle *h, const rpe_camera *cam1, const rpe_camera *cam2, int B)
{
    const size_t cap = (size_t)2 * h->cfg.max_batch;
    if (!h->d_batch_cams) {
        DM(h, h->d_batch_cams, cap);
        h->h_batch_cams.resize(cap);
    }
    HIPCHK(h, hipStreamSynchronize(h->stream));
    memcpy(h->h_batch_cams.data(), cam1, sizeof(rpe_camera) * (size_t)B);
    memcpy(h->h_batch_cams.data() + B, cam2, sizeof(rpe_camera) * (size_t)B);
    HIPCHK(h, hipMemcpyAsync(h->d_batch_cams, h->h_batch_cams.data(), sizeof(rpe_camera) * 2 * (size_t)B, hipMemcpyHostToDevice, h->stream));
    return RPE_OK;
}

extern "C" int rpe_frames_set_cameras(rpe_handle *h, int n, const int32_t *slots, const rpe_camera *cams)
{
    if (!h || !slots || !cams || n < 1) { if (h) h->err = "rpe_frames_set_cameras: null argument or n < 1"; return RPE_ERR_INVALID; }
    if (h->fs.cap == 0) { h->err = "rpe_frames_set_cameras: no frame store (rpe_frames_reserve)"; return RPE_ERR_INVALID; }
    for (int i = 0; i < n; ++i) if (slots[i] < 0 || slots[i] >= h->fs.cap) { h->err = "rpe_frames_set_cameras: slot outside the store"; return RPE_ERR_INVALID; }
    int rc = check_cameras(h, cams, n, "rpe_frames_set_cameras");
    if (rc) return rc;
    HIPCHK(h, hipSetDevice(h->cfg.device));
    HIPCHK(h, hipStreamSynchronize(h->stream));
    last_run_store_changed(h, false);
    for (int i = 0; i < n; ++i) {
        const size_t s = (size_t)slots[i];
        h->fs.h_cam[s] = cams[i];
// ... 356 lines not shown
```

relative_pose_estimation_amd/csrc/rpe_internal.h:

```cpp
#pragma once
#include <hip/hip_runtime.h>
#include <assert.h>
#include <math.h>
#include <stdint.h>
#include <stdio.h>
#include <algorithm>
#include <initializer_list>
#include <string>
#include <vector>
#include "../../include/rpe_amd.h"
#include "buf_layout.h"

#define RPE_NLEVELS RPE_ORB_LEVELS
#define RPE_EDGE 31
#define RPE_HALF_PATCH 15
#define RPE_RANSAC_CHUNK 64
#define RPE_RANSAC_MAXCHUNK 512
#define RPE_MAX_MODELS 10
#define RPE_GRAPH_MAX_PAIRS 16
#define RPE_MATCH_SPLIT_PAIRS 64
#define RPE_GUIDED_LDS_UINT4 128
#define RPE_TAB_RING 4
#define RPE_MAX_MATCHES_LIMIT 8064
#define RPE_MAX_IMAGE_DIM 4095
#define RPE_ORB_MAX_FEATURES 8000
#define RPE_MAX_KCAP (RPE_SIFT_UNCAPPED_CAPACITY + 64)
#define RPE_CU_LDS_BYTES (160 * 1024)
#define RPE_LDS_DEFAULT_BYTES 65536
struct RpeLdsCeiling { const void *kernel; const char *name; size_t bytes; };
std::vector<RpeLdsCeiling> rpe_orb_lds_ceilings();
std::vector<RpeLdsCeiling> rpe_match_lds_ceilings();
std::vector<RpeLdsCeiling> rpe_geom_lds_ceilings();
std::vector<RpeLdsCeiling> rpe_link_lds_ceilings();
#define RPE_RESULT_SECTIONS 5
static const size_t kRpeResultElem[RPE_RESULT_SECTIONS] = {9 * sizeof(double), 3 * sizeof(double), sizeof(int), sizeof(int), sizeof(int)};
#define RPE_RESULT_BYTES 108
constexpr int FAST_TH = 64;
constexpr int FAST_TILE_X0 = RPE_EDGE & ~3;
static_assert(FAST_TILE_X0 >= 4 && RPE_EDGE >= 4, "the FAST tile loads do not clamp x0 - 4 and y0 - 4 at 0");
constexpr int RPE_FAST_TILE_CAP = 1024;
constexpr int rpe_fast_tiles(int w, int h)
{
    return w > 2 * RPE_EDGE && h > 2 * RPE_EDGE ? ((h - 2 * RPE_EDGE + FAST_TH - 1) / FAST_TH) * ((w - RPE_EDGE - FAST_TILE_X0 + 63) / 64) : 0;
}
constexpr int rpe_corner_cap(int w, int h)
{
    const long long c64 = (long long)w * h / 64;
    return (int)(c64 < 1024 ? 1024 : c64 > 8192 ? 8192 : c64);
}
constexpr int PYR_TW = 256, PYR_TH = 16;
constexpr int PYR_DW = 84, PYR_ROWS = 23;

struct RpeLevel {
    int w, h, pitch;
    int quota;
    int ccap;
    int corner_off;
    int kcap2;
    int cand_off;
    float scale;
    float inv_scale;
    long long off;
    int coef_off;
    int dcoef_off;
    int tile0, ntile;
};

struct RpeDeviceLayout {
    RpeLevel lv[RPE_NLEVELS];
    long long stride;
    int corner_total;
    int cand_total;
    int stl;
    int kcap;
    int fast_thr;
    const uint8_t *in_a, *in_b;
    int in_na, in_img;
};

__device__ __forceinline__ const uint8_t *rpe_level_base(const uint8_t *pyr, const RpeDeviceLayout &lay, int img, int l)
{
    if (l == 0 && lay.in_a)
        return img < lay.in_na ? lay.in_a + (long long)img * lay.in_img : lay.in_b + (long long)(img - lay.in_na) * lay.in_img;
    return pyr + (long long)img * lay.stride + lay.lv[l].off;
}

template <bool TAB>
__device__ __forceinline__ void rpe_pair_slots(const int2 *__restrict__ tab, int img2_base, int pair, int &img1, int &img2)
{
    if (TAB) { const int2 s = tab[pair]; img1 = s.x; img2 = s.y; }
    else { img1 = pair; img2 = img2_base + pair; }
}

struct RpeCamSrc { const rpe_camera *cams; const int2 *tab; int img2_base; };

__device__ __forceinline__ void rpe_pair_cameras(const RpeCamSrc &src, int pair, const rpe_camera *&c1, const rpe_camera *&c2)
{
    int i1 = pair, i2 = src.img2_base + pair;
    if (src.tab) { const int2 s = src.tab[pair]; i1 = s.x; i2 = s.y; }
    c1 = src.cams + i1; c2 = src.cams + i2;
}

template <bool CAM>
__device__ __forceinline__ double rpe_pair_focal(const double *__restrict__ K, const RpeCamSrc &src, int pair)
{
    if (CAM) {
        const rpe_camera *c1, *c2;
        rpe_pair_cameras(src, pair, c1, c2);
        return (((c1->fx + c1->fy) / 2) + ((c2->fx + c2->fy) / 2)) / 2;
    } else {
        const double fx = K[0], fy = K[4];
        return (fx + fy) / 2;
    }
}

__device__ __forceinline__ bool rpe_camera_has_lens(const rpe_camera *c)
{
    bool lens = false;
#pragma unroll
    for (int k = 0; k < 8; ++k) lens = lens || c->dist[k] != 0.;
    return lens;
}

__device__ __forceinline__ double2 rpe_camera_normalise(const rpe_camera *c, bool lens, float2 p)
{
    const double xd = ((double)p.x - c->cx) / c->fx, yd = ((double)p.y - c->cy) / c->fy;
    double x = xd, y = yd;
    if (lens) {
        const double k1 = c->dist[0], k2 = c->dist[1], p1 = c->dist[2], p2 = c->dist[3];
        const double k3 = c->dist[4], k4 = c->dist[5], k5 = c->dist[6], k6 = c->dist[7];
#pragma unroll
        for (int it = 0; it < RPE_UNDISTORT_ITERS; ++it) {
            const double r2 = x * x + y * y;
            const double icd = (1 + r2 * (k4 + r2 * (k5 + r2 * k6))) / (1 + r2 * (k1 + r2 * (k2 + r2 * k3)));
            const double dx = 2 * p1 * x * y + p2 * (r2 + 2 * x * x), dy = p1 * (r2 + 2 * y * y) + 2 * p2 * x * y;
            x = (xd - dx) * icd; y = (yd - dy) * icd;
        }
    }
    return make_double2(x, y);
}

template <bool CAM>
struct RpePairNormalise {
    const rpe_camera *c1, *c2;
    bool lens1, lens2;
    double fx, fy, cx, cy;
    __device__ __forceinline__ RpePairNormalise(const double *__restrict__ K, const RpeCamSrc &src, int pair)
    {
        if (CAM) {
            rpe_pair_cameras(src, pair, c1, c2);
            lens1 = rpe_camera_has_lens(c1); lens2 = rpe_camera_has_lens(c2);
        } else {
            fx = K[0]; fy = K[4]; cx = K[2]; cy = K[5];
        }
    }
    __device__ __forceinline__ void operator()(float2 a, float2 b, double2 &na, double2 &nb) const
    {
        if (CAM) {
            na = rpe_camera_normalise(c1, lens1, a);
            nb = rpe_camera_normalise(c2, lens2, b);
        } else {
            na = make_double2(((double)a.x - cx) / fx, ((double)a.y - cy) / fy);
            nb = make_double2(((double)b.x - cx) / fx, ((double)b.y - cy) / fy);
        }
    }
};

#define RPE_WAVE_SCAN(NAME, OP, IDENT)                                                                            \
    __device__ __forceinline__ int NAME(int v)                                                                    \
    {                                                                                                             \
        v = OP(v, __builtin_amdgcn_update_dpp(IDENT, v, 0x111, 0xF, 0xF, false));                  \
        v = OP(v, __builtin_amdgcn_update_dpp(IDENT, v, 0x112, 0xF, 0xF, false));                  \
        v = OP(v, __builtin_amdgcn_update_dpp(IDENT, v, 0x114, 0xF, 0xF, false));                  \
        v = OP(v, __builtin_amdgcn_update_dpp(IDENT, v, 0x118, 0xF, 0xF, false));                  \
        v = OP(v, __builtin_amdgcn_update_dpp(IDENT, v, 0x142, 0xA, 0xF, false));       \
        v = OP(v, __builtin_amdgcn_update_dpp(IDENT, v, 0x143, 0xC, 0xF, false));       \
        return v;                                                                                                 \
    }
#define RPE_OP_ADD(a, b) ((a) + (b))
#define RPE_OP_MAX(a, b) max((a), (b))
#define RPE_OP_MIN(a, b) min((a), (b))
RPE_WAVE_SCAN(wave_inclusive_sum, RPE_OP_ADD, 0)
RPE_WAVE_SCAN(wave_inclusive_max, RPE_OP_MAX, (int)0x80000000)
RPE_WAVE_SCAN(wave_inclusive_min, RPE_OP_MIN, 0x7FFFFFFF)
__device__ __forceinline__ int wave_sum(int v) { return __builtin_amdgcn_readlane(wave_inclusive_sum(v), 63); }
__device__ __forceinline__ int block_excl_scan(int v, int *s_wave , int &total)
{
    const int lane = threadIdx.x & 63, wv = threadIdx.x >> 6;
    const int inc = wave_inclusive_sum(v);
    if (lane == 63) s_wave[wv] = inc;
    __syncthreads();
    int base = 0;
#pragma unroll
    for (int k = 0; k < 4; ++k) { int s = s_wave[k]; if (k < wv) base += s; }
    total = s_wave[0] + s_wave[1] + s_wave[2] + s_wave[3];
    __syncthreads();
    return base + inc - v;
}
__device__ __forceinline__ void elect_best(int best_cnt, int best_key, int *s_best , int &win_cnt, int &win_key)
{
    const int wv = threadIdx.x >> 6;
    if ((threadIdx.x & 63) == 0) { s_best[wv * 2] = best_cnt; s_best[wv * 2 + 1] = best_key; }
    __syncthreads();
    win_cnt = -1; win_key = -1;
#pragma unroll
    for (int w = 0; w < 4; ++w) {
        const int c = s_best[w * 2], key = s_best[w * 2 + 1];
        if (key >= 0 && (c > win_cnt || (c == win_cnt && key < win_key))) { win_cnt = c; win_key = key; }
    }
}
__device__ __forceinline__ int block_count(int cnt, int *s_cnt )
{
    cnt = wave_sum(cnt);
    if ((threadIdx.x & 63) == 0) s_cnt[threadIdx.x >> 6] = cnt;
    __syncthreads();
    return (s_cnt[0] + s_cnt[1]) + (s_cnt[2] + s_cnt[3]);
}

__device__ __forceinline__ int tk_thread_index(int n)
{
    const long long i = (long long)blockIdx.x * 256 + threadIdx.x;
    return i < n ? (int)i : -1;
}

struct RpeTile { short level, tx, ty, pad; };
struct alignas(16) RpePyrTile { short x0, y0, a0, sy0; unsigned short nsrc, reuse; int pad; };
static_assert(sizeof(RpePyrTile) == 16 && PYR_TH <= 16, "one reuse bit per tile row");
constexpr int PYR_YW_SHIFT = 23;

struct RpeRansacState {
    int best_count;
    int best_iter;
    int best_model;
    int niters;
    int next_iter;
    int done;
    int found;
    int M;
    int iters_run;
    int pad_;
    double E[9];
};

struct RpeSiftState;

struct RpeFeatSrc { const uint8_t *desc; const int *count; const float2 *pt; const int2 *norm; const int2 *tab; int img2_base; };

struct RpeRun {
    int pairs;
    RpeFeatSrc feat;
    RpeCamSrc cam;
};

struct RpeLastRun {
    enum Kind { NONE, RULE, LIST, CHUNKED };
    Kind kind = NONE;
    int pairs = 0;
    RpeRun run{};
    std::vector<int> tab;
    std::vector<uint32_t> ovf;
    bool per_match = false;
    int structure = 0;
};

struct RpeTrackJob {
    int P, n_frames, rule, min_len;
    const int2 *frames;
    const int *m_n, *q, *t;
    const uint8_t *use_pair, *edge;
    const int *status;
    const uint8_t *rmask, *pmask;
    const float2 *pts1, *pts2;
};
#define RPE_TRACK_NODE_WORDS 11
static inline int rpe_track_scan_blocks(int N) { return (int)(((long long)N + 2047) / 2048); }

struct RpeTrackPointJob {
    int n_tracks, n_obs, min_views, max_iters, cam_stride;
    double threshold_px, max_cos;
    const int *track_start, *obs_frame, *group;
    const float2 *obs_xy;
    const double *R, *T;
    const rpe_camera *cams;
};

struct RpeLink { int a, b, side, pad; };
struct RpeLinkSrc {
    const RpeLink *links;
    const int *m_q, *m_t, *m_n, *status;
    const uint8_t *ransac_mask, *pose_mask;
    const double *points, *R, *t;
    const double2 *n1, *n2;
    int max_matches, kcap;
};

struct RpeBufSet { uint8_t *block = nullptr; size_t bytes = 0; };

struct rpe_handle {
    rpe_config cfg;
    RpeSiftState *sift = nullptr;
    int desc_bytes = 32;
    std::string err;
    hipStream_t stream = nullptr;
    hipStream_t copy_stream = nullptr;
    hipEvent_t ev_up[8] = {};
    struct GraphEntry { const uint8_t *a, *b; int B; hipGraph_t graph; hipGraphExec_t exec; };
    std::vector<GraphEntry> graphs;
    RpeLastRun last;
    std::vector<void *> dev_allocs;
    RpeDeviceLayout lay{};
    int n_img_cap = 0;
    RpeTile *d_tiles_fast = nullptr;  int n_tiles_fast = 0;
    int *d_coef = nullptr;
    RpePyrTile *d_pyr_tiles = nullptr;
    int pyr_tile_off[RPE_NLEVELS] = {}, pyr_tile_cnt[RPE_NLEVELS] = {};
    uint8_t *d_pyr = nullptr;
    unsigned *d_tile_list = nullptr;
    int *d_tile_cnt = nullptr;
    uint8_t *d_stage1 = nullptr, *d_stage2 = nullptr;
    unsigned *d_corner = nullptr;
    int *d_corner_count = nullptr;
    int *d_kp_lvl_count = nullptr;
    unsigned *d_cand_xy = nullptr;
    float *d_cand_resp = nullptr;
    int *d_cand_count = nullptr;
    unsigned *d_kp_xy = nullptr;
    float *d_kp_resp = nullptr, *d_kp_angle = nullptr;
    float2 *d_kp_pt = nullptr;
    int *d_kp_count = nullptr;
    unsigned *d_ovf = nullptr;
    int level0_slots = 0;
    uint8_t *d_desc = nullptr;
    RpeTile *d_tiles_full = nullptr;  int n_tiles_full = 0;
    uint8_t *d_bufA = nullptr;
    int *d_m_q = nullptr, *d_m_t = nullptr, *d_m_d = nullptr, *d_m_n = nullptr;
    unsigned long long *d_m_best = nullptr;
    int *d_m_norm = nullptr;
    unsigned *d_hm_best = nullptr, *d_hm_row = nullptr;
    unsigned long long *d_m_best2 = nullptr;
    float2 *d_pts1 = nullptr, *d_pts2 = nullptr;
    unsigned short *d_subsets = nullptr;
    double *d_nit_denom = nullptr;
    int *d_nit_round = nullptr;
    double nit_num = 0;
    RpeRansacState *d_rstate = nullptr;
    double2 *d_n1 = nullptr, *d_n2 = nullptr;
    int *d_found = nullptr;
    double *d_hyp = nullptr;
    double *d_models = nullptr;
    int *d_nmodels = nullptr;
    int *d_counts = nullptr;
    uint8_t *d_mask = nullptr;
    uint8_t *d_pose_mask = nullptr;
    double *d_points = nullptr;
    double *d_ref_R = nullptr, *d_ref_t = nullptr, *d_ref_rms = nullptr, *d_ref_R0 = nullptr, *d_ref_t0 = nullptr;
    int *d_ref_inl = nullptr, *d_ref_info = nullptr; RpeBufSet set_refine;
    RpeLink *d_links = nullptr;
    std::vector<RpeLink> link_tab;
    double *d_link_stats = nullptr;
    int *d_link_n = nullptr, *d_link_code = nullptr; RpeBufSet set_links;
    int *d_gm_q = nullptr, *d_gm_t = nullptr, *d_gm_d = nullptr, *d_gm_n = nullptr;
    float2 *d_gm_pts1 = nullptr, *d_gm_pts2 = nullptr;
    double *d_gm_R = nullptr, *d_gm_tr = nullptr, *d_gm_thr2 = nullptr;
    double4 *d_gm_rec = nullptr; RpeBufSet set_guided;
    double *d_hg_H = nullptr, *d_hg_R = nullptr;
    int *d_hg_counts = nullptr, *d_hg_info = nullptr;
    uint8_t *d_hg_mask = nullptr; RpeBufSet set_homography;
    double *d_lp_R = nullptr, *d_lp_t = nullptr, *d_lp_rms = nullptr, *d_lp_corr = nullptr;
    int *d_lp_counts = nullptr, *d_lp_info = nullptr;
    uint8_t *d_lp_mask = nullptr; RpeBufSet set_link_poses;
    uint8_t *d_ba_views = nullptr; RpeBufSet set_bundles;
    double *d_ba_obs = nullptr, *d_ba_points = nullptr, *d_ba_pose0 = nullptr, *d_ba_focal = nullptr, *d_ba_state = nullptr;
    double *d_ba_Rin = nullptr, *d_ba_tin = nullptr;
    int *d_ba_n = nullptr, *d_ba_pre = nullptr, *d_ba_counts = nullptr, *d_ba_info = nullptr;
    double *d_ba_Ra = nullptr, *d_ba_ta = nullptr, *d_ba_Rb = nullptr, *d_ba_tb = nullptr, *d_ba_rms = nullptr;
    uint8_t *d_tk_eflag = nullptr, *d_tk_edge = nullptr, *d_tk_use = nullptr;
    int *d_tk_mtrack = nullptr, *d_tk_q = nullptr, *d_tk_t = nullptr, *d_tk_m = nullptr, *d_tk_counts = nullptr;
    int *d_tk_tstart = nullptr, *d_tk_oframe = nullptr, *d_tk_okp = nullptr;
    float2 *d_tk_oxy = nullptr, *d_tk_pts1 = nullptr, *d_tk_pts2 = nullptr;
    int2 *d_tk_frames = nullptr, *d_tk_partial = nullptr;
    int *d_tk_node = nullptr, *d_tk_seen = nullptr; RpeBufSet set_tracks;
    std::vector<int> tk_frame_tab;
    int *d_tp_tstart = nullptr, *d_tp_oframe = nullptr, *d_tp_group = nullptr, *d_tp_info = nullptr;
    float2 *d_tp_oxy = nullptr;
    double2 *d_tp_obs = nullptr;
    double *d_tp_R = nullptr, *d_tp_T = nullptr, *d_tp_points = nullptr, *d_tp_rms = nullptr, *d_tp_mincos = nullptr, *d_tp_oerr = nullptr;
    uint8_t *d_tp_oflag = nullptr;
    rpe_camera *d_tp_cams = nullptr;
    rpe_camera tp_cam_k{}; RpeBufSet set_track_points;
    double *d_R = nullptr, *d_t = nullptr, *d_E = nullptr;
    int *d_inliers = nullptr, *d_status = nullptr;
    double K_last[9] = {0}; bool K_valid = false;
    uint8_t *d_resall = nullptr; unsigned *d_ovfall = nullptr;
    uint8_t *d_resblk = nullptr, *h_resblk = nullptr;
    double *d_K = nullptr;
    struct FrameStore {
        int cap = 0;
        uint8_t *d_desc = nullptr;
        float2 *d_kp_pt = nullptr;
        int2 *d_norm = nullptr;
        int *d_count = nullptr;
        unsigned *d_ovf = nullptr;
        std::vector<uint8_t> filled;
        rpe_camera *d_cam = nullptr;
        std::vector<rpe_camera> h_cam;
        std::vector<uint8_t> has_cam;
    } fs;
    int *h_pairtab = nullptr;
    int *d_pairtab = nullptr;
    hipEvent_t ev_tab[RPE_TAB_RING] = {};
    int tab_next = 0;
    rpe_camera *d_batch_cams = nullptr;
    std::vector<rpe_camera> h_batch_cams;
    unsigned *d_calib_sink = nullptr;
    bool profiling = false;
    hipEvent_t ev[RPE_STAGE_COUNT + 1] = {};
    bool ev_valid = false;
    int ev_first = 0;
    std::vector<void *> user_allocs;
};

template <typename T>
static int dmalloc(rpe_handle *h, T **p, size_t n)
{
    const hipError_t e = hipMalloc((void **)p, n * sizeof(T));
    if (e != hipSuccess) { *p = nullptr; h->err = std::string("hipMalloc failed: ") + hipGetErrorString(e); return RPE_ERR_HIP; }
    h->dev_allocs.push_back(*p);
    return RPE_OK;
}
#define DM(h, p, n) do { int r_ = dmalloc(h, &(p), (size_t)(n)); if (r_) return r_; } while (0)
#define DM_ONCE(h, p, n) do { if (!(p)) DM(h, p, n); } while (0)

struct RpeBufPiece { void **p; size_t bytes; };
template <typename T>
static inline RpeBufPiece buf_piece(T *&p, size_t n) { return {(void **)&p, n * sizeof(T)}; }
int rpe_bufset_fit(rpe_handle *h, RpeBufSet &s, std::initializer_list<RpeBufPiece> pieces);

extern std::string g_create_err;
#define HIPCHK(h, call)                                                                         \
    do {                                                                                        \
        hipError_t e_ = (call);                                                                 \
        if (e_ != hipSuccess) {                                                                 \
            char b_[512];                                                                       \
            snprintf(b_, sizeof(b_), "%s failed: %s (%s:%d)", #call, hipGetErrorString(e_), __FILE__, __LINE__); \
            if (h) (h)->err = b_; else g_create_err = b_;                                       \
            return RPE_ERR_HIP;                                                                 \
        }                                                                                       \
    } while (0)

static inline int cv_round(double v) { return (int)lrint(v); }

static inline int rpe_invalid(rpe_handle *h, const char *who, const char *what = "a null argument or a count out of range")
{
    if (h) h->err = std::string(who) + ": " + what;
    return RPE_ERR_INVALID;
}

static inline RpeRun rpe_run_rule(const rpe_handle *h, int pairs, int img2_base, RpeCamSrc cam)
{
    return {pairs, {h->d_desc, h->d_kp_count, h->d_kp_pt, (const int2 *)h->d_m_norm, nullptr, img2_base}, cam};
}
static inline RpeRun rpe_run_batch(const rpe_handle *h, int B, RpeCamSrc cam = {nullptr, nullptr, 0}) { return rpe_run_rule(h, B, B, cam); }
static inline RpeRun rpe_run_stream(const rpe_handle *h, int pairs, RpeCamSrc cam = {nullptr, nullptr, 0}) { return rpe_run_rule(h, pairs, 1, cam); }
static inline RpeRun rpe_run_list(const rpe_handle *h, int P, RpeCamSrc cam = {nullptr, nullptr, 0})
{
    return {P, {h->fs.d_desc, h->fs.d_count, h->fs.d_kp_pt, h->fs.d_norm, (const int2 *)h->d_pairtab, 0}, cam};
}

static inline int rpe_link_capacity(const rpe_handle *h) { return 4 * h->cfg.max_batch; }
static inline RpeLinkSrc rpe_link_src(const rpe_handle *h)
{
    return {h->d_links, h->d_m_q, h->d_m_t, h->d_m_n, h->d_status, h->d_mask, h->d_pose_mask, h->d_points, h->d_R, h->d_t,
            h->d_n1, h->d_n2, h->cfg.max_matches, h->lay.kcap};
}

void rpe_launch_pyramid(rpe_handle *h, int n_img);
void rpe_launch_fast(rpe_handle *h, int n_img);
void rpe_launch_raster_retain(rpe_handle *h, int n_img);
void rpe_launch_harris(rpe_handle *h, int n_img);
void rpe_launch_keypoints(rpe_handle *h, int n_img);
void rpe_launch_orient_describe(rpe_handle *h, int n_img);
void rpe_launch_debug_blur(rpe_handle *h, int img);
constexpr size_t rpe_retain_lds(int kind, int cap) { return (kind ? sizeof(unsigned long long) : sizeof(unsigned)) * (size_t)cap + sizeof(unsigned short) * ((size_t)cap + 4); }
void rpe_launch_debug_retain(rpe_handle *h, int kind, int stl, void *d_elems, const int *d_len, const int *d_n_points, int *d_out_len, int n_lists, int cap);
struct RpeHammingPlan {
    int region0;
    int sortP;
    int split;
    bool hbm;
    size_t lds_tile, lds_select;
};
RpeHammingPlan rpe_hamming_plan(int kcap, int B, int extra_uint4);
void rpe_launch_match(rpe_handle *h, const RpeRun &r);
void rpe_launch_match_l2(rpe_handle *h, const RpeRun &r);
void rpe_launch_l2_norms(rpe_handle *h, int n_img);
void rpe_launch_guided(rpe_handle *h, const RpeRun &r, const double *d_R, const double *d_t, const int *d_status, double gate_px, int max_distance);
void rpe_launch_guided_l2(rpe_handle *h, const RpeRun &r, const double *d_R, const double *d_t, const int *d_status, double gate_px, double max_distance);
int rpe_sift_create(rpe_handle *h);
void rpe_sift_destroy(rpe_handle *h);
int rpe_sift_run(rpe_handle *h, const uint8_t *d_a, const uint8_t *d_b, int na, int nb);
int rpe_sift_fetch(rpe_handle *h, int n_images, float *fin_host, int *counts);
int rpe_sift_fetch_gauss(rpe_handle *h, int index, float *out);
long long rpe_sift_gauss_floats(rpe_handle *h);
void rpe_launch_ransac(rpe_handle *h, const RpeRun &r, bool want_mask);
void rpe_launch_pose(rpe_handle *h, const RpeRun &r, bool set_status);
void rpe_launch_structure(rpe_handle *h, const RpeRun &r);
void rpe_launch_refine(rpe_handle *h, const RpeRun &r, int max_iters, bool from_batch);
void rpe_launch_scale_links(rpe_handle *h, int L, int min_shared);
void rpe_launch_link_poses(rpe_handle *h, const RpeRun &r, int L, int iters, double threshold_px, int min_shared, int refine_iters);
bool rpe_link_poses_in_lds(const rpe_handle *h);
void rpe_launch_bundle_gather(rpe_handle *h, const RpeRun &r, int L, double threshold_px);
void rpe_launch_bundle(rpe_handle *h, int n, int min_shared, int max_iters, bool links);
bool rpe_bundles_in_lds(const rpe_handle *h);
void rpe_launch_tracks(rpe_handle *h, const RpeTrackJob &job);
void rpe_launch_track_points(rpe_handle *h, const RpeTrackPointJob &job);
void rpe_launch_normalise(rpe_handle *h, const RpeRun &r);
void rpe_launch_homography(rpe_handle *h, const RpeRun &r, int iters, double threshold_px, bool from_batch);
void rpe_launch_undistort(rpe_handle *h, const float2 *d_pts, int n, const rpe_camera *d_cam, double2 *d_out);

#define MARK(h, stage) do { if ((h)->profiling) hipEventRecord((h)->ev[stage], (h)->stream); } while (0)
```

Measured before the change: 106,700 pairs/s.

## Split ORB pyramid levels into groups and overlap stages on a side stream

Partitions the ORB pyramid levels into two tile-balanced groups. The first group's FAST, raster/retain, Harris and retain-harris kernels run on a side stream while the main stream builds the remaining pyramid levels and runs the second group's stages. The two streams join before keypoint compaction. This aims to fill the GPU during the small, serial per-level kernels, at the cost of an extra stream, events and fork/join synchronisation. Batches small enough to be graph-captured keep the linear schedule.

Measured after the change: 112,500 pairs/s, median of 6. 5.5% higher.

```diff
diff --git a/include/rpe_amd.h b/include/rpe_amd.h
--- a/include/rpe_amd.h
+++ b/include/rpe_amd.h
@@ -224,6 +224,7 @@
                                rpe_keypoint *kps, uint8_t *desc, int32_t *counts);
 int rpe_orb_debug_fetch(rpe_handle *h, int index, int which, uint8_t *h_out);
 int64_t rpe_orb_pyramid_pixels(const rpe_handle *h);
+int rpe_orb_group_min_images(void);
 int rpe_orb_debug_retain(rpe_handle *h, int kind, int stl_runtime, void *elems, const int32_t *len, const int32_t *n_points,
                          int n_lists, int cap, int32_t *out_len);
 
diff --git a/relative_pose_estimation_amd/_capi.py b/relative_pose_estimation_amd/_capi.py
--- a/relative_pose_estimation_amd/_capi.py
+++ b/relative_pose_estimation_amd/_capi.py
@@ -56,6 +56,7 @@
     "rpe_guided_matches_l2": "i:pippddpppppp",
     "rpe_pair_homographies": "i:piidppppp", "rpe_find_homography": "i:ppppipidppppp",
     "rpe_orb_detect_and_compute": "i:ppippp", "rpe_orb_debug_fetch": "i:piip", "rpe_orb_pyramid_pixels": "l:p",
+    "rpe_orb_group_min_images": "i:",
     "rpe_orb_debug_retain": "i:piipppiip",
     "rpe_match_hamming": "i:pppppipppp", "rpe_match_hamming_guided": "i:pppppppipppdipppp",
     "rpe_sift_detect_and_compute": "i:ppippp", "rpe_sift_debug_gauss": "l:pip", "rpe_match_l2": "i:pppppipppp",
diff --git a/relative_pose_estimation_amd/csrc/orb_groups.h b/relative_pose_estimation_amd/csrc/orb_groups.h
--- /dev/null
+++ b/relative_pose_estimation_amd/csrc/orb_groups.h
@@ -0,0 +1,21 @@
+#pragma once
+
+#define RPE_ORB_GROUP_MAX 4
+
+struct RpeOrbGroup { int l0, l1, t0, nt; };
+
+static inline void rpe_orb_groups(const int *ntile, int nlevels, int G, RpeOrbGroup *out)
+{
+    long long total = 0;
+    for (int l = 0; l < nlevels; ++l) total += ntile[l];
+    long long before = 0;
+    int l = 0;
+    for (int g = 0; g < G; ++g) {
+        out[g].l0 = l; out[g].t0 = (int)before; out[g].nt = 0;
+        for (; l < nlevels && !(ntile[l] > 0 && (2 * before + ntile[l]) * G / (2 * total) > g); ++l) {
+            out[g].nt += ntile[l];
+            before += ntile[l];
+        }
+        out[g].l1 = l;
+    }
+}
diff --git a/relative_pose_estimation_amd/csrc/orb_kernels.hip b/relative_pose_estimation_amd/csrc/orb_kernels.hip
--- a/relative_pose_estimation_amd/csrc/orb_kernels.hip
+++ b/relative_pose_estimation_amd/csrc/orb_kernels.hip
@@ -163,9 +163,9 @@
     }
 }
 
-void rpe_launch_pyramid(rpe_handle *h, int n_img)
-{
-    for (int l = 1; l < RPE_NLEVELS; ++l) {
+void rpe_launch_pyramid(rpe_handle *h, int n_img, int l0, int l1)
+{
+    for (int l = std::max(l0, 1); l < l1; ++l) {
         const int nt = h->pyr_tile_cnt[l];
         hipLaunchKernelGGL(pyr_resize_kernel, dim3((nt + 7) / 8 * 8, n_img), dim3(PYR_THREADS), 0, h->stream, h->d_pyr, h->lay, h->d_coef,
                            (const RpePyrTile *)(h->d_pyr_tiles + h->pyr_tile_off[l]), nt, l);
@@ -194,7 +194,7 @@
 static_assert((FAST_PROWS * 18 + FS_ROWS * 18) * 4 + FAST_NCAND * 2 + 8 == 19448, "LDS per workgroup");
 __global__ __launch_bounds__(FAST_THREADS) void fast_nms_kernel(const uint8_t *__restrict__ pyr, unsigned *__restrict__ tile_list,
                                                         int *__restrict__ tile_cnt, RpeDeviceLayout lay,
-                                                        const RpeTile *__restrict__ tiles, int ntiles)
+                                                        const RpeTile *__restrict__ tiles, int ntiles, int t0, int nt)
 {
     __shared__ __attribute__((aligned(16))) unsigned s_in[FAST_PROWS * 18];
     __shared__ __attribute__((aligned(16))) unsigned s_sc[FS_ROWS * 18];
@@ -202,8 +202,9 @@
     __shared__ unsigned short s_cand[FAST_NCAND];
     __shared__ int s_ncand, s_nout;
     const int tid = threadIdx.x, lane = tid & 63;
-    const int ti = xcd_tile(blockIdx.x, ntiles);
-    if (ti >= ntiles) return;
+    const int tr = xcd_tile(blockIdx.x, nt);
+    if (tr >= nt) return;
+    const int ti = t0 + tr;
     const RpeTile t = tiles[ti];
     const RpeLevel &L = lay.lv[t.level];
     const int w = L.w, hgt = L.h, pitch = L.pitch, thr = lay.fast_thr;
@@ -410,16 +411,16 @@
     if (tid == 0) tile_cnt[tslot] = nout;
 }
 
-void rpe_launch_fast(rpe_handle *h, int n_img)
-{
-    if (h->n_tiles_fast == 0) return;
-    hipLaunchKernelGGL(fast_nms_kernel, dim3((h->n_tiles_fast + 7) / 8 * 8, n_img), dim3(FAST_THREADS), 0, h->stream,
-                       h->d_pyr, h->d_tile_list, h->d_tile_cnt, h->lay, h->d_tiles_fast, h->n_tiles_fast);
+void rpe_launch_fast(rpe_handle *h, int n_img, int t0, int nt, hipStream_t stream)
+{
+    if (nt == 0) return;
+    hipLaunchKernelGGL(fast_nms_kernel, dim3((nt + 7) / 8 * 8, n_img), dim3(FAST_THREADS), 0, stream,
+                       h->d_pyr, h->d_tile_list, h->d_tile_cnt, h->lay, h->d_tiles_fast, h->n_tiles_fast, t0, nt);
 }
 
 __global__ __launch_bounds__(256) void raster_corners_kernel(const unsigned *__restrict__ tile_list, const int *__restrict__ tile_cnt,
                                                               unsigned *__restrict__ corner, int *__restrict__ corner_count,
-                                                              unsigned *__restrict__ ovf, RpeDeviceLayout lay, int ntiles, int rows_cap, int key_cap)
+                                                              unsigned *__restrict__ ovf, RpeDeviceLayout lay, int ntiles, int rows_cap, int key_cap, int l0)
 {
     extern __shared__ unsigned s_dyn[];
     unsigned *s_rs = s_dyn;
@@ -428,7 +429,7 @@
     unsigned *s_toff = s_key + key_cap;
     __shared__ int s_wave[5];
     __shared__ int s_live;
-    const int tid = threadIdx.x, l = blockIdx.x, img = blockIdx.y;
+    const int tid = threadIdx.x, l = l0 + blockIdx.x, img = blockIdx.y;
     const RpeLevel &L = lay.lv[l];
     if (tid == 64) s_live = 0x7FFFFFFF;
     const int nrows = L.h, nt = L.ntile, ccap = L.ccap;
@@ -531,11 +532,11 @@
 
 __global__ __launch_bounds__(64 * RPE_RETAIN_FAST_WAVES) void retain_fast_kernel(const unsigned *__restrict__ corner, const int *__restrict__ corner_count,
                                                           unsigned *__restrict__ cand_xy, int *__restrict__ cand_count,
-                                                          unsigned *__restrict__ ovf, RpeDeviceLayout lay, int lo, int cap, int n_img)
+                                                          unsigned *__restrict__ ovf, RpeDeviceLayout lay, int lo, int cap, int n_img, int l0)
 {
     extern __shared__ unsigned s_a[];
     __shared__ int s_ctl[3 * RPE_RETAIN_FAST_WAVES];
-    const int tid = threadIdx.x, l = blockIdx.x;
+    const int tid = threadIdx.x, l = l0 + blockIdx.x;
     const RpeLevel &L = lay.lv[l];
 #pragma unroll 1
     for (int img = blockIdx.y; img < n_img; img += gridDim.y) {
@@ -575,8 +576,9 @@
                                                    rpe_fast_tiles(RPE_MAX_IMAGE_DIM, RPE_MAX_IMAGE_DIM));
 static_assert(RASTER_LDS_MAX <= RPE_CU_LDS_BYTES, "the largest image's rows, entries and tiles fit a CU's LDS");
 
-void rpe_launch_raster_retain(rpe_handle *h, int n_img)
-{
+void rpe_launch_raster_retain(rpe_handle *h, int n_img, int l0, int l1, hipStream_t stream)
+{
+    if (l1 <= l0) return;
     int rows_cap = 0, ccap_max = 0, nt_max = 0, wmax = 0, nlev_big = 0;
     for (int l = 0; l < RPE_NLEVELS; ++l) {
         rows_cap = std::max(rows_cap, h->lay.lv[l].h); ccap_max = std::max(ccap_max, h->lay.lv[l].ccap);
@@ -586,21 +588,21 @@
     const int key_cap = raster_key_cap(ccap_max, wmax);
     const size_t lds = raster_lds_bytes(rows_cap, key_cap, nt_max);
     assert(lds <= RASTER_LDS_MAX);
-    hipLaunchKernelGGL(raster_corners_kernel, dim3(RPE_NLEVELS, n_img), dim3(256), lds, h->stream,
+    hipLaunchKernelGGL(raster_corners_kernel, dim3(l1 - l0, n_img), dim3(256), lds, stream,
                        (const unsigned *)h->d_tile_list, (const int *)h->d_tile_cnt,
-                       h->d_corner, h->d_corner_count, h->d_ovf, h->lay, h->n_tiles_fast, rows_cap, key_cap);
-    hipLaunchKernelGGL(retain_fast_kernel, dim3(RPE_NLEVELS, n_img), dim3(64 * RPE_RETAIN_FAST_WAVES), rpe_retain_lds(0, std::min(ccap_max, RPE_RETAIN_TIER)), h->stream,
+                       h->d_corner, h->d_corner_count, h->d_ovf, h->lay, h->n_tiles_fast, rows_cap, key_cap, l0);
+    hipLaunchKernelGGL(retain_fast_kernel, dim3(l1 - l0, n_img), dim3(64 * RPE_RETAIN_FAST_WAVES), rpe_retain_lds(0, std::min(ccap_max, RPE_RETAIN_TIER)), stream,
                        (const unsigned *)h->d_corner, (const int *)h->d_corner_count, h->d_cand_xy, h->d_cand_count, h->d_ovf, h->lay,
-                       0, std::min(ccap_max, RPE_RETAIN_TIER), n_img);
-    if (nlev_big > 0)
-        hipLaunchKernelGGL(retain_fast_kernel, dim3(nlev_big, std::min(n_img, 512)), dim3(64 * RPE_RETAIN_FAST_WAVES), rpe_retain_lds(0, ccap_max), h->stream,
+                       0, std::min(ccap_max, RPE_RETAIN_TIER), n_img, l0);
+    if (std::min(nlev_big, l1) > l0)
+        hipLaunchKernelGGL(retain_fast_kernel, dim3(std::min(nlev_big, l1) - l0, std::min(n_img, 512)), dim3(64 * RPE_RETAIN_FAST_WAVES), rpe_retain_lds(0, ccap_max), stream,
                            (const unsigned *)h->d_corner, (const int *)h->d_corner_count, h->d_cand_xy, h->d_cand_count, h->d_ovf, h->lay,
-                           RPE_RETAIN_TIER, ccap_max, n_img);
+                           RPE_RETAIN_TIER, ccap_max, n_img, l0);
 }
 
 __global__ __launch_bounds__(256) void harris_kernel(const uint8_t *__restrict__ pyr, const unsigned *__restrict__ cand_xy,
                                                       const int *__restrict__ cand_count, float *__restrict__ cand_resp,
-                                                      RpeDeviceLayout lay, int nb, int n_img)
+                                                      RpeDeviceLayout lay, int nb, int n_img, int l0, int l1)
 {
     int img, blk;
     if (!xcd_image_block(nb, n_img, img, blk)) return;
@@ -608,6 +610,7 @@
     int l = -1, ci = 0, acc = 0;
 #pragma unroll
     for (int k = 0; k < RPE_NLEVELS; ++k) {
+        if (k < l0 || k >= l1) continue;
         const int n = cand_count[img * RPE_NLEVELS + k];
         if (l < 0 && dsel < acc + n) { l = k; ci = dsel - acc; }
         acc += n;
@@ -656,11 +659,12 @@
     cand_resp[(long long)img * lay.cand_total + c] = (t3 - t4) * scale_sq_sq;
 }
 
-void rpe_launch_harris(rpe_handle *h, int n_img)
-{
-    const int nb = (h->lay.cand_total + 255) / 256;
-    hipLaunchKernelGGL(harris_kernel, dim3(xcd_image_grid(nb, n_img)), dim3(256), 0, h->stream,
-                       h->d_pyr, h->d_cand_xy, h->d_cand_count, h->d_cand_resp, h->lay, nb, n_img);
+void rpe_launch_harris(rpe_handle *h, int n_img, int l0, int l1, hipStream_t stream)
+{
+    if (l1 <= l0) return;
+    const int nb = (h->lay.lv[l1 - 1].cand_off + h->lay.lv[l1 - 1].kcap2 - h->lay.lv[l0].cand_off + 255) / 256;
+    hipLaunchKernelGGL(harris_kernel, dim3(xcd_image_grid(nb, n_img)), dim3(256), 0, stream,
+                       h->d_pyr, h->d_cand_xy, h->d_cand_count, h->d_cand_resp, h->lay, nb, n_img, l0, l1);
 }
 
 struct HarrisGT { __device__ __forceinline__ bool operator()(unsigned long long a, unsigned long long b) const { return __uint_as_float((unsigned)(a >> 32)) > __uint_as_float((unsigned)(b >> 32)); } };
@@ -668,11 +672,11 @@
 
 __global__ __launch_bounds__(64 * RPE_RETAIN_HARRIS_WAVES) void retain_harris_kernel(unsigned *__restrict__ cand_xy, float *__restrict__ cand_resp,
                                                             const int *__restrict__ cand_count, int *__restrict__ kp_lvl_count,
-                                                            RpeDeviceLayout lay, int lo, int cap)
+                                                            RpeDeviceLayout lay, int lo, int cap, int l0)
 {
     extern __shared__ unsigned long long s_e[];
     __shared__ int s_ctl[3 * RPE_RETAIN_HARRIS_WAVES];
-    const int tid = threadIdx.x, l = blockIdx.x, img = blockIdx.y;
+    const int tid = threadIdx.x, l = l0 + blockIdx.x, img = blockIdx.y;
     const RpeLevel &L = lay.lv[l];
     const int n1 = cand_count[img * RPE_NLEVELS + l];
     const int q = L.quota;
@@ -748,8 +752,9 @@
     }
 }
 
-void rpe_launch_keypoints(rpe_handle *h, int n_img)
-{
+void rpe_launch_retain_harris(rpe_handle *h, int n_img, int l0, int l1, hipStream_t stream)
+{
+    if (l1 <= l0) return;
     int kcap2_max = 0, nlev_big = 0;
     for (int l = 0; l < RPE_NLEVELS; ++l) {
         kcap2_max = std::max(kcap2_max, h->lay.lv[l].kcap2);
@@ -757,11 +762,15 @@
     }
     const int tier = std::min(kcap2_max, RPE_RETAIN_TIER / 2);
     assert(kcap2_max <= RETAIN_HARRIS_CAP_MAX);
-    hipLaunchKernelGGL(retain_harris_kernel, dim3(RPE_NLEVELS, n_img), dim3(64 * RPE_RETAIN_HARRIS_WAVES), rpe_retain_lds(1, tier), h->stream,
-                       h->d_cand_xy, h->d_cand_resp, (const int *)h->d_cand_count, h->d_kp_lvl_count, h->lay, 0, tier);
-    if (nlev_big > 0)
-        hipLaunchKernelGGL(retain_harris_kernel, dim3(nlev_big, n_img), dim3(64 * RPE_RETAIN_HARRIS_WAVES), rpe_retain_lds(1, kcap2_max), h->stream,
-                           h->d_cand_xy, h->d_cand_resp, (const int *)h->d_cand_count, h->d_kp_lvl_count, h->lay, RPE_RETAIN_TIER / 2, kcap2_max);
+    hipLaunchKernelGGL(retain_harris_kernel, dim3(l1 - l0, n_img), dim3(64 * RPE_RETAIN_HARRIS_WAVES), rpe_retain_lds(1, tier), stream,
+                       h->d_cand_xy, h->d_cand_resp, (const int *)h->d_cand_count, h->d_kp_lvl_count, h->lay, 0, tier, l0);
+    if (std::min(nlev_big, l1) > l0)
+        hipLaunchKernelGGL(retain_harris_kernel, dim3(std::min(nlev_big, l1) - l0, n_img), dim3(64 * RPE_RETAIN_HARRIS_WAVES), rpe_retain_lds(1, kcap2_max), stream,
+                           h->d_cand_xy, h->d_cand_resp, (const int *)h->d_cand_count, h->d_kp_lvl_count, h->lay, RPE_RETAIN_TIER / 2, kcap2_max, l0);
+}
+
+void rpe_launch_keypoints(rpe_handle *h, int n_img)
+{
     hipLaunchKernelGGL(compact_keypoints_kernel, dim3(n_img), dim3(256), 0, h->stream,
                        (const unsigned *)h->d_cand_xy, (const float *)h->d_cand_resp, (const int *)h->d_kp_lvl_count,
                        h->d_kp_xy, h->d_kp_resp, h->d_kp_pt, h->d_kp_count, h->d_ovf, h->lay);
diff --git a/relative_pose_estimation_amd/csrc/rpe_api.hip b/relative_pose_estimation_amd/csrc/rpe_api.hip
--- a/relative_pose_estimation_amd/csrc/rpe_api.hip
+++ b/relative_pose_estimation_amd/csrc/rpe_api.hip
@@ -207,6 +207,11 @@
     for (const RpeTile &t : fast)
         if (t.tx < 4 || t.ty < 4) { h->err = "FAST tile origin below 4: the tile loads would start outside the level"; return RPE_ERR_INVALID; }
     h->n_tiles_full = (int)full.size(); h->n_tiles_fast = (int)fast.size();
+    {
+        int ntile[RPE_NLEVELS];
+        for (int l = 0; l < RPE_NLEVELS; ++l) ntile[l] = L.lv[l].ntile;
+        rpe_orb_groups(ntile, RPE_NLEVELS, RPE_ORB_GROUPS, h->orb_group);
+    }
     DM(h, h->d_tiles_full, full.size());
     DM(h, h->d_tiles_fast, fast.size() ? fast.size() : 1);
     HIPCHK(h, hipMemcpy(h->d_tiles_full, full.data(), full.size() * sizeof(RpeTile), hipMemcpyHostToDevice));
@@ -452,6 +457,11 @@
         if (is_sift && (rc = rpe_sift_create(h)) != RPE_OK) break;
         for (int i = 0; i <= RPE_STAGE_COUNT; ++i)
             if (hipEventCreate(&h->ev[i]) != hipSuccess) { h->err = "hipEventCreate failed"; rc = RPE_ERR_HIP; break; }
+        if (rc != RPE_OK || is_sift) break;
+        if (hipStreamCreateWithFlags(&h->side_stream, hipStreamNonBlocking) != hipSuccess) { h->err = "hipStreamCreateWithFlags failed"; rc = RPE_ERR_HIP; break; }
+        bool ev_ok = hipEventCreateWithFlags(&h->ev_join, hipEventDisableTiming) == hipSuccess;
+        for (int g = 0; g < RPE_ORB_GROUPS && ev_ok; ++g) ev_ok = hipEventCreateWithFlags(&h->ev_fork[g], hipEventDisableTiming) == hipSuccess;
+        if (!ev_ok) { h->err = "hipEventCreateWithFlags failed"; rc = RPE_ERR_HIP; break; }
     } while (0);
     if (rc != RPE_OK) { g_create_err = h->err; rpe_destroy(h); return rc; }
     *out = h;
@@ -470,6 +480,9 @@
     if (!h) return;
     hipSetDevice(h->cfg.device);
     if (h->stream) hipStreamSynchronize(h->stream);
+    if (h->side_stream) { hipStreamSynchronize(h->side_stream); hipStreamDestroy(h->side_stream); }
+    for (int g = 0; g < RPE_ORB_GROUPS; ++g) if (h->ev_fork[g]) hipEventDestroy(h->ev_fork[g]);
+    if (h->ev_join) hipEventDestroy(h->ev_join);
     rpe_sift_destroy(h);
     for (auto &g : h->graphs) { hipGraphExecDestroy(g.exec); hipGraphDestroy(g.graph); }
     for (void *p : h->dev_allocs) hipFree(p);
@@ -586,12 +599,40 @@
         int rc = load_level0(h, d_a, d_b, na, nb);
         if (rc) return rc;
     }
-    rpe_launch_pyramid(h, n);
-    MARK(h, RPE_STAGE_FAST);      rpe_launch_fast(h, n);
+    const bool grouped = n >= RPE_ORB_GROUP_MIN_IMAGES;
+    const int last = grouped ? RPE_ORB_GROUPS - 1 : 0;
+    const RpeOrbGroup all = {0, RPE_NLEVELS, 0, h->n_tiles_fast};
+    const int pyr_split = grouped ? std::max(h->orb_group[0].l1, 1) : RPE_NLEVELS;
+    hipError_t fe = hipSuccess;
+    bool forked = false;
+    rpe_launch_pyramid(h, n, 1, pyr_split);
+    if (!grouped) MARK(h, RPE_STAGE_FAST);
+    for (int g = 0; g < last; ++g) {
+        const RpeOrbGroup &G = h->orb_group[g];
+        if (g > 0) rpe_launch_fast(h, n, G.t0, G.nt, h->stream);
+        hipStream_t s = h->stream;
+        if (fe == hipSuccess) fe = hipEventRecord(h->ev_fork[g], h->stream);
+        if (fe == hipSuccess) fe = hipStreamWaitEvent(h->side_stream, h->ev_fork[g], 0);
+        if (fe == hipSuccess) { s = h->side_stream; forked = true; }
+        if (g == 0) rpe_launch_fast(h, n, G.t0, G.nt, s);
+        rpe_launch_raster_retain(h, n, G.l0, G.l1, s);
+        rpe_launch_harris(h, n, G.l0, G.l1, s);
+        rpe_launch_retain_harris(h, n, G.l0, G.l1, s);
+        if (g == 0) { rpe_launch_pyramid(h, n, pyr_split, RPE_NLEVELS); MARK(h, RPE_STAGE_FAST); }
+    }
+    const RpeOrbGroup &G = grouped ? h->orb_group[last] : all;
+    rpe_launch_fast(h, n, G.t0, G.nt, h->stream);
     MARK(h, RPE_STAGE_NMS);
-    MARK(h, RPE_STAGE_SELECT);    rpe_launch_raster_retain(h, n);
-    MARK(h, RPE_STAGE_HARRIS);    rpe_launch_harris(h, n);
-    MARK(h, RPE_STAGE_KEYPOINTS); rpe_launch_keypoints(h, n);
+    MARK(h, RPE_STAGE_SELECT);    rpe_launch_raster_retain(h, n, G.l0, G.l1, h->stream);
+    MARK(h, RPE_STAGE_HARRIS);    rpe_launch_harris(h, n, G.l0, G.l1, h->stream);
+    MARK(h, RPE_STAGE_KEYPOINTS); rpe_launch_retain_harris(h, n, G.l0, G.l1, h->stream);
+    if (forked) {
+        hipError_t je = hipEventRecord(h->ev_join, h->side_stream);
+        if (je == hipSuccess) je = hipStreamWaitEvent(h->stream, h->ev_join, 0);
+        if (je != hipSuccess) { hipStreamSynchronize(h->side_stream); if (fe == hipSuccess) fe = je; }
+    }
+    HIPCHK(h, fe);
+    rpe_launch_keypoints(h, n);
     MARK(h, RPE_STAGE_ANGLE);     rpe_launch_orient_describe(h, n);
     MARK(h, RPE_STAGE_BLUR);
     MARK(h, RPE_STAGE_DESCRIBE);
@@ -1685,6 +1726,8 @@
     for (int l = 0; l < RPE_NLEVELS; ++l) n += (int64_t)h->lay.lv[l].w * h->lay.lv[l].h;
     return n;
 }
+
+extern "C" int rpe_orb_group_min_images(void) { return RPE_ORB_GROUP_MIN_IMAGES; }
 
 extern "C" int rpe_orb_debug_fetch(rpe_handle *h, int index, int which, uint8_t *h_out)
 {
diff --git a/relative_pose_estimation_amd/csrc/rpe_internal.h b/relative_pose_estimation_amd/csrc/rpe_internal.h
--- a/relative_pose_estimation_amd/csrc/rpe_internal.h
+++ b/relative_pose_estimation_amd/csrc/rpe_internal.h
@@ -10,6 +10,7 @@
 #include <vector>
 #include "../../include/rpe_amd.h"
 #include "buf_layout.h"
+#include "orb_groups.h"
 
 #define RPE_NLEVELS RPE_ORB_LEVELS
 #define RPE_EDGE 31
@@ -18,6 +19,10 @@
 #define RPE_RANSAC_MAXCHUNK 512
 #define RPE_MAX_MODELS 10
 #define RPE_GRAPH_MAX_PAIRS 16
+#define RPE_ORB_GROUP_MIN_IMAGES 33
+#define RPE_ORB_GROUPS 2
+static_assert(RPE_ORB_GROUP_MIN_IMAGES > 2 * RPE_GRAPH_MAX_PAIRS, "a captured batch takes the linear schedule");
+static_assert(RPE_ORB_GROUPS >= 2 && RPE_ORB_GROUPS <= RPE_ORB_GROUP_MAX, "rpe_orb_groups cuts at most RPE_ORB_GROUP_MAX groups");
 #define RPE_MATCH_SPLIT_PAIRS 64
 #define RPE_GUIDED_LDS_UINT4 128
 #define RPE_TAB_RING 4
@@ -314,6 +319,9 @@
     int *d_coef = nullptr;
     RpePyrTile *d_pyr_tiles = nullptr;
     int pyr_tile_off[RPE_NLEVELS] = {}, pyr_tile_cnt[RPE_NLEVELS] = {};
+    RpeOrbGroup orb_group[RPE_ORB_GROUPS] = {};
+    hipStream_t side_stream = nullptr;
+    hipEvent_t ev_fork[RPE_ORB_GROUPS] = {}, ev_join = nullptr;
     uint8_t *d_pyr = nullptr;
     unsigned *d_tile_list = nullptr;
     int *d_tile_cnt = nullptr;
@@ -474,10 +482,11 @@
             h->d_n1, h->d_n2, h->cfg.max_matches, h->lay.kcap};
 }
 
-void rpe_launch_pyramid(rpe_handle *h, int n_img);
-void rpe_launch_fast(rpe_handle *h, int n_img);
-void rpe_launch_raster_retain(rpe_handle *h, int n_img);
-void rpe_launch_harris(rpe_handle *h, int n_img);
+void rpe_launch_pyramid(rpe_handle *h, int n_img, int l0, int l1);
+void rpe_launch_fast(rpe_handle *h, int n_img, int t0, int nt, hipStream_t stream);
+void rpe_launch_raster_retain(rpe_handle *h, int n_img, int l0, int l1, hipStream_t stream);
+void rpe_launch_harris(rpe_handle *h, int n_img, int l0, int l1, hipStream_t stream);
+void rpe_launch_retain_harris(rpe_handle *h, int n_img, int l0, int l1, hipStream_t stream);
 void rpe_launch_keypoints(rpe_handle *h, int n_img);
 void rpe_launch_orient_describe(rpe_handle *h, int n_img);
 void rpe_launch_debug_blur(rpe_handle *h, int img);
```
